# micahvista/VACmap

Measured on AMD Instinct MI355X. Metric: aligned Gbp/s (whole node) + reads/s, 15 kb ONT-shape reads vs hg38-size ref, 1/2/4/8 MI355X, higher is better.
Workload: dtype i16/i32 DP + f64 chains

## Files before the change

### include/vacmapx.h

```cpp
#ifndef VACMAPX_H
#define VACMAPX_H
#include <stdint.h>
#ifdef __cplusplus
extern "C" {
#endif

typedef enum vm_status {
    VM_OK = 0,
    VM_ERR_ARG = -1,
    VM_ERR_NO_DEVICE = -2,
    VM_ERR_NO_CTX = -3,
    VM_ERR_OOM = -4,
    VM_ERR_IO = -5,
    VM_ERR_HIP = -6,
    VM_ERR_UNSUPPORTED = -7,
    VM_READ_RAISED = -10,
    VM_READ_CAPACITY = -20,
    VM_READ_FASTPATH = -21,
    VM_READ_UNSUPPORTED = -22
} vm_status;

enum { VM_MODE_H = 0, VM_MODE_L = 1, VM_MODE_S = 2, VM_MODE_R = 3,
       VM_MODE_ASM = 4 };

// ... 45 lines not shown
int vm_index_blob_count(const vm_index*);
int vm_index_blob(const vm_index*, int i, void** dev_ptr, int64_t* bytes);
int vm_index_meta_size(const vm_index*, int64_t* bytes);
int vm_index_meta_get(const vm_index*, void* buf, int64_t bytes);
int vm_index_from_meta(vm_ctx*, const void* buf, int64_t bytes, vm_index** out);

int vm_sketch_batch(vm_ctx*, int k, int w, int64_t n, const char* seqs, const int64_t* offsets,
                    uint64_t** hash, int32_t** pos, int8_t** strand, int64_t** off);
int vm_map_batch(vm_ctx*, const vm_index*, int check_num, int mid_occ, int64_t n, const char* seqs,
                 const int64_t* offsets, int64_t** anchors, int64_t** anchor_off);
int vm_map(vm_ctx*, const vm_index*, const char* seq, int64_t len, int check_num, int mid_occ, int64_t** anchors, int64_t* n);

typedef struct vm_chains_out {
    int32_t* need_reverse;
    int32_t* mapq;
    double* score;
    int32_t* fast_used;
    int64_t* read_path_off;
    int64_t* path_off;
    int64_t* path_anchors;
    double* S; int64_t* P; int64_t* S_arg; int64_t* gmax; int64_t* opcount;
} vm_chains_out;
int vm_chain_global_batch(vm_ctx*, const vm_params*, int kmersize, int64_t n, const int64_t* anchors,
                          const int64_t* anchor_off, const int64_t* readlens, int want_raw, vm_chains_out* out);
void vm_chains_out_free(vm_chains_out*);

typedef struct vm_local_out {
    int32_t* status;
    int32_t* variant;
    double* score;
    int64_t* chain_off;
    int64_t* chain;
    int64_t* raw_off;
    int64_t* raw;
} vm_local_out;
int vm_local_chain_batch(vm_ctx*, const vm_index*, const vm_params*, int64_t n, const char* seqs, const int64_t* offsets,
                         const int64_t* read_path_off, const int64_t* path_off, const int64_t* path_anchors, vm_local_out* out);
void vm_local_out_free(vm_local_out*);

typedef struct vm_linked_out {
    int64_t gmax, n_hot, n_cold, opcount; double cold_max;
    double* S; int64_t* P; int64_t* S_arg_hot;
    int32_t carry_status, saved; int64_t n_carry; double* carry_S; int64_t* carry_P; int64_t* carry_rows; double carry_g_max_scores; int64_t carry_prereadloc;
} vm_linked_out;
int vm_chain_linked(vm_ctx*, int which, int kmersize, double skipcost, int maxdiff, int maxgap, int64_t n, const int64_t* rows, int64_t n_pre,
                    const double* pre_S, const int64_t* pre_P, double g_max_scores, int64_t g_max_index, int64_t prereadloc, vm_linked_out* out);
void vm_linked_out_free(vm_linked_out*);

typedef struct vm_score { int32_t match, mismatch, o1, e1, o2, e2; } vm_score;
int vm_k_cigar_batch(vm_ctx*, const vm_score*, int eqx, int64_t n, const char* t, const int64_t* t_off, const char* q,
                     const int64_t* q_off, char** cigars, int64_t** cigar_off, int32_t** scores);
int vm_k_cigar_batch_banded(vm_ctx*, const vm_score*, int eqx, int64_t n, const char* t, const int64_t* t_off, const char* q,
                            const int64_t* q_off, char** cigars, int64_t** cigar_off, int32_t** band_flag, int64_t* stats);
int vm_k_extend_batch(vm_ctx*, int match, int mismatch, int o, int e, int bw, int zdrop, int64_t n, const char* t,
                      const int64_t* t_off, const char* q, const int64_t* q_off, int32_t** t_e, int32_t** q_e, int32_t** score);
typedef struct vm_cigar_out { char* cigar; int32_t q_e, t_e, score; } vm_cigar_out;
int vm_k_cigar(vm_ctx*, const char* t, int64_t tl, const char* q, int64_t ql, const vm_score* sc, int bw, int zdrop,
               int eqx, vm_cigar_out* out);
int vm_edit_distance_batch(vm_ctx*, int64_t n, const char* q, const int64_t* q_off, const char* t, const int64_t* t_off,
                           int64_t** dist);
int64_t vm_edit_distance(vm_ctx*, const char* q, int64_t ql, const char* t, int64_t tl);
int vm_edit_distance_bound_batch(vm_ctx*, int tier, int64_t n, const char* q, const int64_t* q_off, const char* t, const int64_t* t_off,
                                 int64_t** bound);

typedef struct vm_record {
    int32_t read_idx;
    int32_t contig;
    int32_t strand;
    int32_t mapq;
    int64_t q_st, q_en;
    int64_t r_st, r_en;
    int64_t cigar_off, cigar_len;
} vm_record;

typedef struct vm_batch_stats {
    int64_t n_reads, read_bases, n_minimizers, n_hits, n_anchors, n_local_hits, n_local_anchors;
    int64_t n_segments, n_ed_problems, ed_cells, n_ext_problems, ext_cells, n_dp_problems, dp_cells;
    int64_t n_records, cigar_bytes, aligned_bases, n_unmapped, n_failed;
    int64_t dp_string_bytes;
    double ms_total;
    double ms_stage[16];
    double ms_gapfill_fill;
    double ms_gapfill_trace;
    int64_t n_gapfill_launches;
    int64_t n_ed_full;
    int64_t n_ed_tier2;
    int64_t n_ed_tier1;
    int64_t n_dp_redo;
    int64_t dp_redo_tb_bytes;
    double ms_local_seed;
    double ms_cluster;
    int64_t n_host_syncs;
    int64_t n_local_general;
    int64_t n_ext_retries;
    int64_t n_batch_retries;
    int64_t n_dp_redo_wide;
    int64_t n_dp_redo_full;
} vm_batch_stats;

int vm_align_batch(vm_ctx*, const vm_index*, const vm_params*, int64_t n_reads, const char* seqs, const int64_t* offsets,
                   vm_record** recs, int64_t* n_recs, char** cigar_blob, int32_t* status_per_read, vm_batch_stats* stats);
typedef struct vm_reads vm_reads;
int vm_reads_upload(vm_ctx*, int64_t n_reads, const char* seqs, const int64_t* offsets, vm_reads** out);
int vm_reads_reupload(vm_ctx*, vm_reads*, int64_t n_reads, const char* seqs, const int64_t* offsets);
void vm_reads_free(vm_reads*);
int vm_align_resident(vm_ctx*, const vm_index*, const vm_params*, const vm_reads*, vm_record** recs, int64_t* n_recs,
                      char** cigar_blob, int32_t* status_per_read, vm_batch_stats* stats);

int vm_align_asm(vm_ctx*, const vm_index*, const vm_params* p, const char* contig, int64_t len, int64_t split_len, int64_t batch_anchors, int64_t window,
                 vm_record** recs, int64_t* n_recs, char** cigar_blob, int32_t* status);

int vm_align_trace(vm_ctx*, const vm_index*, const vm_params*, int64_t n_reads, const char* seqs, const int64_t* offsets, int stage,
                   int64_t** rows, int64_t** row_off);

typedef struct vm_sam_opts {
    int32_t md, shortcs, cigar2cg, markunbalancetra, hardclip, fakecigar;
    const char* rg_id;
    int32_t asm_mode;
} vm_sam_opts;
int vm_sam_emit(const vm_index*, const vm_sam_opts*, int64_t n_reads, const char* names, const int64_t* name_off, const char* seqs, const int64_t* seq_off,
                const char* quals, const int64_t* qual_off, const char* comments, const int64_t* com_off, const vm_record* recs, int64_t n_recs,
                const char* cigar_blob, const int32_t* status, int nthreads, char** text, int64_t** text_off, int64_t* n_lines, int64_t* n_skipped);
int vm_sam_emit_device(vm_ctx*, const vm_index*, const vm_sam_opts*, int64_t n_reads, const char* names, const int64_t* name_off, const char* seqs,
                       const int64_t* seq_off, const char* quals, const int64_t* qual_off, const vm_record* recs, int64_t n_recs, const char* cigar_blob,
                       const int32_t* status, char** text, int64_t** text_off, int64_t* n_lines, int64_t* n_skipped);
int vm_sam_emit_device_times(vm_ctx*, double* seconds3);
int64_t vm_blob_gather(const char* blob, const int64_t* off, const int64_t* idx, int64_t n, char* out, int64_t* out_off);
int64_t vm_blob_write_parts_mmap(int fd, int64_t file_off, const char* const* blobs, const int64_t* const* offs, const int32_t* part, const int64_t* idx, int64_t n, int nthreads);
int64_t vm_blob_gather_parts(const char* const* blobs, const int64_t* const* offs, const int32_t* part, const int64_t* idx, int64_t n, char* out);
void* vm_pinned_alloc(int64_t bytes, int device);
void vm_pinned_free(void* p);
int64_t vm_blob_write_parts(int fd, const char* const* blobs, const int64_t* const* offs, const int32_t* part, const int64_t* idx, int64_t n);
typedef struct vm_fastx vm_fastx;
int vm_fastx_open(const char* path, vm_fastx** out);
int vm_fastx_open_range(const char* path, int64_t begin, int64_t end, vm_fastx** out);
void vm_fastx_close(vm_fastx*);
int64_t vm_fastx_read(vm_fastx*, int64_t max_reads, int64_t max_bases, char** names, int64_t** name_off, char** seqs, int64_t** seq_off, char** quals,
                      int64_t** qual_off, char** comments, int64_t** com_off);

typedef struct vm_bam_writer vm_bam_writer;
int vm_bam_writer_create(vm_ctx*, const char* sam_header, int64_t len, vm_bam_writer** out);
void vm_bam_writer_free(vm_bam_writer*);
int vm_bam_header(vm_bam_writer*, char** out, int64_t* n);
int vm_bam_encode(vm_bam_writer*, const char* sam, int64_t len, char** out, int64_t* n);
int vm_bam_compress_parts(vm_bam_writer*, const char* const* blobs, const int64_t* const* offs, const int32_t* part, const int64_t* idx, int64_t n,
                          char** out, int64_t* n_out);
int vm_bgzf_compress(vm_ctx*, const void* in, int64_t n, char** out, int64_t* n_out);

int vm_bgzf_decompress(vm_ctx*, const void* in, int64_t n, char** out, int64_t* n_out);
typedef struct vm_bam_reader vm_bam_reader;
// ... 27 lines not shown
```

### vacmap_amd/csrc/k_dp.hip

```cpp
#include "vmx_device.h"
#include "vmx_kernels.h"

__device__ __forceinline__ int vmx_tcode(uint8_t c) { return c < 4 ? (int)c : 6; }


__global__ void k_encode(const char* __restrict__ in, uint8_t* __restrict__ out, int64_t n) {
    int64_t i = (int64_t)blockIdx.x * blockDim.x + threadIdx.x;
    int64_t stride = (int64_t)gridDim.x * blockDim.x;
    for (; i < n; i += stride) out[i] = vmx_code((uint8_t)in[i]);
}

#define VMX_EXT_RING 512
__global__ void __launch_bounds__(64) k_extend(const uint8_t* __restrict__ tcodes, const int64_t* __restrict__ t_off,
                                               const uint8_t* __restrict__ qcodes, const int64_t* __restrict__ q_off, int n_prob,
                                               int match, int mismatch, int o, int e, int bw_in, int zdrop,
                                               int32_t* __restrict__ out_te, int32_t* __restrict__ out_qe, int32_t* __restrict__ out_sc, const int32_t* __restrict__ n_ptr) {
    if (n_ptr) n_prob = *n_ptr;
    __shared__ int sH[3][VMX_EXT_RING];
    __shared__ int sE[2][VMX_EXT_RING];
    __shared__ int sF[2][VMX_EXT_RING];
    const int lane = vmx_lane();
    const int RM = VMX_EXT_RING - 1;
    for (int p = blockIdx.x; p < n_prob; p += gridDim.x) {
        const uint8_t* T = tcodes + t_off[p];
// ... 390 lines not shown
                int dloX = 0, dloY = 0;
                const int gX = nsX > 0 ? vmx_ad_geom_nd(tlX0, qlX0, VMX_ADW_DPN * ns, &dloX) : 0, gY = nsY > 0 ? vmx_ad_geom_nd(tlY0, qlY0, VMX_ADW_DPN * ns, &dloY) : 0;
                const int tlX = gX > 0 ? tlX0 : 0, qlX = gX > 0 ? qlX0 : 0, tlY = gY > 0 ? tlY0 : 0, qlY = gY > 0 ? qlY0 : 0;
                int scX = 0, scY = 0;
#define VMX_ADW_RUN(NSV) vmx_gapfill_fill_ad<NSV, 64>(tcodes + prX.t_off, qcodes + prX.q_off, tlX, qlX, dloX, vmx_tb_ptr(tb_pool, redo_pool, prX.tb_off), tcodes + prY.t_off, qcodes + prY.q_off, \
                                                      tlY, qlY, dloY, vmx_tb_ptr(tb_pool, redo_pool, prY.tb_off), match, mismatch, o1, e1, o2, e2, lane, scX, scY)
                if (ns == 2) VMX_ADW_RUN(2); else if (ns == 3) VMX_ADW_RUN(3); else VMX_ADW_RUN(4);
#undef VMX_ADW_RUN
                keepX = gX > 0 && vmx_ad_proven(scX, tlX0, qlX0, gX, match, o1, e1, o2, e2);
                keepY = gY > 0 && vmx_ad_proven(scY, tlY0, qlY0, gY, match, o1, e1, o2, e2);
            }
            if (lane == 0) {
                if (keepX) out_score[pX] = VMX_PK_FLAG;
                if (keepY) out_score[pY] = VMX_PK_FLAG;
                const int kept = (int)keepX + (int)keepY, full = 1 + (int)(pY >= 0) - kept;
                if (kept) atomicAdd(redo_cnt + 6, kept);
                if (full) atomicAdd(redo_cnt + 7, full);
            }
            if (!keepX || (pY >= 0 && !keepY)) __syncthreads();
            if (!keepX) vmx_gapfill_fill_one<SCORE>(tcodes, qcodes, probs, pX, match, mismatch, o1, e1, o2, e2, tb_pool, bnd_pool, out_score, lane, VMX_PK_FLAG, redo_pool);
            if (pY >= 0 && !keepY) vmx_gapfill_fill_one<SCORE>(tcodes, qcodes, probs, pY, match, mismatch, o1, e1, o2, e2, tb_pool, bnd_pool, out_score, lane, VMX_PK_FLAG, redo_pool);
        }
    }
    while (true) {
        int q0;
        if (order) { int v = 0; if (lane == 0) v = atomicAdd(counter, 4); q0 = vmx_bcast0(v); }
        else { q0 = static_next; static_next += 4 * (int)gridDim.x; }
        if (q0 >= n_prob) break;
        const int qg = q0 + (lane >> 4);
        const int pg = qg < n_prob ? (order ? order[qg] : qg) : -1;
        bool x4 = false, skip = false;
        {
            vmx_dp_prob pr; pr.tl = 0; pr.ql = 0; pr.t_off = 0; pr.q_off = 0; pr.tb_off = 0; pr.bnd_off = 0;
            if (pg >= 0) pr = probs[pg];
            skip = redo_pass && pg >= 0 && VMX_REDO_PK(pr.tl, pr.ql);
            x4 = pg >= 0 && !skip && pr.tl > 0 && pr.ql > 0 && VMX_DP16X4_OK(pr.tl, pr.ql);
            if (!SCORE && x4 && (lane & 15) == 0) out_score[pg] = 0;
            if (__any(x4))
                vmx_gapfill_fill16x4<SCORE>(tcodes + pr.t_off, qcodes + pr.q_off, x4 ? pr.tl : 0, x4 ? pr.ql : 0, match, mismatch, o1, e1, o2, e2, vmx_tb_ptr(tb_pool, redo_pool, pr.tb_off),
                                            bnd_pool + pr.bnd_off, &out_score[pg < 0 ? 0 : pg], lane);
        }
        for (int gk = 0; gk < 4; ++gk) {
            const int p = vmx_readlane(pg, 16 * gk);
            if (p < 0 || vmx_readlane((int)(x4 || skip), 16 * gk)) continue;
            vmx_gapfill_fill_one<SCORE>(tcodes, qcodes, probs, p, match, mismatch, o1, e1, o2, e2, tb_pool, bnd_pool, out_score, lane, 0, redo_pool);
        }
    }
}

__device__ __forceinline__ void vmx_gapfill_ad_pass(const uint8_t* __restrict__ tcodes, const uint8_t* __restrict__ qcodes, vmx_dp_prob* __restrict__ probs, int n_prob,
                                                   int match, int mismatch, int o1, int e1, int o2, int e2, uint8_t* __restrict__ tb_pool, int32_t* __restrict__ bnd_pool,
                                                   int32_t* __restrict__ out_score, const int32_t* __restrict__ order, const int32_t* __restrict__ range, int32_t* __restrict__ counter,
                                                   int32_t* __restrict__ redo_list, int32_t* __restrict__ redo_cnt, int ad_pct, unsigned long long* __restrict__ redo_bytes,
                                                   unsigned long long redo_cap, int tb_by_ns) {
    const int lane = vmx_lane();
    const int pct = ad_pct & 0xffff, pct_min = (ad_pct >> 16) & 0xffff;
    const bool ad_ok = vmx_ad_scores_ok(match, mismatch, o1, e1, o2, e2);
    const int n_head = range[0] < n_prob ? range[0] : n_prob;
    bool head = n_head > 0;
    while (true) {
        int pX = -1, pY = -1;
        if (head) {
            int q; { int v = 0; if (lane == 0) v = atomicAdd(counter + 1, 1); q = vmx_bcast0(v); }
            if (q >= n_head) { head = false; continue; }
            if (lane < 16) pX = order[q];
        } else {
            int q0; { int v = 0; if (lane == 0) v = atomicAdd(counter, 8); q0 = n_head + vmx_bcast0(v); }
            if (q0 >= n_prob) break;
            const int qX = q0 + 2 * (lane >> 4), qY = qX + 1;
            if (qX < n_prob) pX = order[qX];
            if (qY < n_prob) pY = order[qY];
        }
        vmx_dp_prob prX, prY;
        prX.tl = 0; prX.ql = 0; prX.t_off = 0; prX.q_off = 0; prX.tb_off = 0; prY = prX;
        if (pX >= 0) prX = probs[pX];
        if (pY >= 0) prY = probs[pY];
        const bool x4X = pX >= 0 && prX.tl > 0 && prX.ql > 0 && VMX_DP16X4_OK(prX.tl, prX.ql), x4Y = pY >= 0 && prY.tl > 0 && prY.ql > 0 && VMX_DP16X4_OK(prY.tl, prY.ql);
        const int nsX = x4X && ad_ok ? vmx_ad_ns(prX.tl, prX.ql, match, o1, e1, o2, e2, pct, pct_min) : 0, nsY = x4Y && ad_ok ? vmx_ad_ns(prY.tl, prY.ql, match, o1, e1, o2, e2, pct, pct_min) : 0;
        const int ns = vmx_uniform_i32(vmx_wave_max_i32(nsX > nsY ? nsX : nsY));
        bool keepX = false, keepY = false, triedX = false, triedY = false;
        if (ns > 0) {
            int dloX = 0, dloY = 0;
            const bool fitX = !tb_by_ns || VMX_AD_W(nsX) == VMX_AD_W(ns), fitY = !tb_by_ns || VMX_AD_W(nsY) == VMX_AD_W(ns);
            const int gX = (nsX > 0 && fitX) ? vmx_ad_geom(prX.tl, prX.ql, ns, &dloX) : 0, gY = (nsY > 0 && fitY) ? vmx_ad_geom(prY.tl, prY.ql, ns, &dloY) : 0;
            const int tlX = gX > 0 ? prX.tl : 0, qlX = gX > 0 ? prX.ql : 0, tlY = gY > 0 ? prY.tl : 0, qlY = gY > 0 ? prY.ql : 0;
            int scX = 0, scY = 0;
#define VMX_AD_RUN(NSV) vmx_gapfill_fill_ad<NSV>(tcodes + prX.t_off, qcodes + prX.q_off, tlX, qlX, dloX, tb_pool + prX.tb_off, tcodes + prY.t_off, qcodes + prY.q_off, tlY, qlY, dloY, \
                                                 tb_pool + prY.tb_off, match, mismatch, o1, e1, o2, e2, lane, scX, scY)
            if (ns == 1) VMX_AD_RUN(1); else if (ns == 2) VMX_AD_RUN(2); else if (ns == 3) VMX_AD_RUN(3); else VMX_AD_RUN(4);
#undef VMX_AD_RUN
            triedX = gX > 0; triedY = gY > 0;
            keepX = gX > 0 && vmx_ad_proven(scX, prX.tl, prX.ql, gX, match, o1, e1, o2, e2);
            keepY = gY > 0 && vmx_ad_proven(scY, prY.tl, prY.ql, gY, match, o1, e1, o2, e2);
        }
        if ((lane & 15) == 0) {
            if (x4X) {
                out_score[pX] = keepX ? VMX_AD_FLAG + ns : 0;
                if (!keepX) {
                    if (triedX) atomicAdd(redo_cnt + 3, 1);
                    const unsigned long long need = (unsigned long long)VMX_REDO_TB_BYTES(prX.tl, prX.ql), at = atomicAdd(redo_bytes, need);
                    if (at + need > redo_cap) { probs[pX].tl = 0; probs[pX].ql = 0; probs[pX].tb_off = 0; }
                    else { probs[pX].tb_off = -(int64_t)at - 1; redo_list[atomicAdd(redo_cnt, 1)] = pX; }
                }
            }
            if (x4Y) {
                out_score[pY] = keepY ? VMX_AD_FLAG + ns : 0;
                if (!keepY) {
                    if (triedY) atomicAdd(redo_cnt + 3, 1);
                    const unsigned long long need = (unsigned long long)VMX_REDO_TB_BYTES(prY.tl, prY.ql), at = atomicAdd(redo_bytes, need);
                    if (at + need > redo_cap) { probs[pY].tl = 0; probs[pY].ql = 0; probs[pY].tb_off = 0; }
                    else { probs[pY].tb_off = -(int64_t)at - 1; redo_list[atomicAdd(redo_cnt, 1)] = pY; }
                }
            }
        }
        for (int gk = 0; gk < 8; ++gk) {
            const int p = vmx_readlane((gk & 1) ? pY : pX, 16 * (gk >> 1));
            if (p < 0 || vmx_readlane((int)((gk & 1) ? x4Y : x4X), 16 * (gk >> 1))) continue;
            vmx_gapfill_fill_one<false>(tcodes, qcodes, probs, p, match, mismatch, o1, e1, o2, e2, tb_pool, bnd_pool, out_score, lane);
        }
    }
}

__global__ void __launch_bounds__(64) k_gapfill_fill(const uint8_t* __restrict__ tcodes, const uint8_t* __restrict__ qcodes,
                                                     const vmx_dp_prob* __restrict__ probs, int n_prob, int match, int mismatch,
                                                     int o1, int e1, int o2, int e2, uint8_t* __restrict__ tb_pool,
                                                     int32_t* __restrict__ bnd_pool, int32_t* __restrict__ out_score,
                                                     const int32_t* __restrict__ order, int32_t* __restrict__ counter) {
    vmx_gapfill_fill_body<true>(tcodes, qcodes, probs, n_prob, match, mismatch, o1, e1, o2, e2, tb_pool, bnd_pool, out_score, order, counter);
}
__global__ void __launch_bounds__(64, 4) k_gapfill_fill_ns(const uint8_t* __restrict__ tcodes, const uint8_t* __restrict__ qcodes,
                                                        vmx_dp_prob* __restrict__ probs, int n_prob, int match, int mismatch,
                                                        int o1, int e1, int o2, int e2, uint8_t* __restrict__ tb_pool,
                                                        int32_t* __restrict__ bnd_pool, int32_t* __restrict__ out_score,
                                                        const int32_t* __restrict__ order, const int32_t* __restrict__ range, int32_t* __restrict__ counter,
                                                        int32_t* __restrict__ redo_list, int32_t* __restrict__ redo_cnt, int ad_pct,
                                                        unsigned long long* __restrict__ redo_bytes, const int32_t* __restrict__ n_ptr,
                                                        unsigned long long redo_cap, int tb_by_ns) {
    if (n_ptr) n_prob = *n_ptr;
    vmx_gapfill_ad_pass(tcodes, qcodes, probs, n_prob, match, mismatch, o1, e1, o2, e2, tb_pool, bnd_pool, out_score, order, range, counter, redo_list, redo_cnt, ad_pct, redo_bytes, redo_cap, tb_by_ns);
}
__global__ void __launch_bounds__(64) k_gapfill_redo(const uint8_t* __restrict__ tcodes, const uint8_t* __restrict__ qcodes, const vmx_dp_prob* __restrict__ probs,
                                                     int match, int mismatch, int o1, int e1, int o2, int e2, uint8_t* __restrict__ tb_pool,
                                                     int32_t* __restrict__ bnd_pool, int32_t* __restrict__ out_score, int32_t* __restrict__ redo_list,
                                                     int32_t* __restrict__ redo_cnt, uint8_t* __restrict__ redo_pool) {
    vmx_gapfill_fill_body<false, true>(tcodes, qcodes, probs, 0, match, mismatch, o1, e1, o2, e2, tb_pool, bnd_pool, out_score, nullptr, nullptr, redo_list, redo_cnt, redo_pool);
}

__global__ void k_gapfill_trace(const uint8_t* __restrict__ tcodes, const uint8_t* __restrict__ qcodes,
                                const vmx_dp_prob* __restrict__ probs, int n_prob, int eqx, const uint8_t* __restrict__ tb_pool,
                                uint32_t* __restrict__ run_pool, char* __restrict__ cig_pool, int32_t* __restrict__ cig_len,
                                const int32_t* __restrict__ band_flag, const uint8_t* __restrict__ redo_pool, int spread, int32_t* __restrict__ cig_q,
                                const int32_t* __restrict__ n_ptr) {
    VMX_SETPRIO(3);
    if (n_ptr) n_prob = *n_ptr;
    const int gt = (int)(blockIdx.x * blockDim.x + threadIdx.x);
    if (spread > 1 && gt % spread) return;
    int p = spread > 1 ? gt / spread : gt;
    if (p >= n_prob) return;
    const vmx_dp_prob pr = probs[p];
    const uint8_t* T = tcodes + pr.t_off;
    const uint8_t* Q = qcodes + pr.q_off;
    const int tl = pr.tl, ql = pr.ql;
    const uint8_t* tb = vmx_tb_ptr(tb_pool, redo_pool, pr.tb_off);
    uint32_t* runs = run_pool + pr.run_off;
    char* cig = cig_pool + pr.cig_off;
    bool x4 = tl > 0 && ql > 0 && VMX_DP16X4_OK(tl, ql);
    bool pk = !x4 && tl > 0 && ql > 0 && VMX_DP16_OK(tl, ql);
    const int flag = (x4 && band_flag != nullptr) ? band_flag[p] : 0;
    const int ns = flag > VMX_AD_FLAG ? flag - VMX_AD_FLAG : 0;
    if (flag == VMX_PK_FLAG) { x4 = false; pk = true; }
    int dlo = 0;
    if (ns) vmx_ad_geom(tl, ql, ns, &dlo);
    const int AW = ns ? VMX_AD_W(ns) : 4;
    const int W = x4 ? VMX_X4_W(ql) : ql + (pk ? 127 : 63);
    int nruns = 0; int cur_op = -1; uint32_t cur_len = 0;
#define VMX_EMIT(op)                                                                   \
    do {                                                                               \
        if ((op) == cur_op) ++cur_len;                                                 \
        else { if (cur_op >= 0) runs[nruns++] = (cur_len << 8) | (uint32_t)cur_op; cur_op = (op); cur_len = 1; } \
    } while (0)
    int i = tl, j = ql, state = 0;
    while (i > 0 && j > 0) {
        int b;
        if (ns && state == 0) {
            const int x = (j - i) - dlo, l = x / (2 * ns), k = (x - 2 * ns * l) >> 1;
            const uint8_t* cell = tb + VMX_AD_TB_OFF_W(0, l, AW) + k;
            const int s0 = i + j - 1;
            int m = i < j ? i : j; if (m > 8) m = 8;
            uint8_t bb[8], ta[8], qa[8];
#pragma unroll
            for (int u = 0; u < 8; ++u) if (u < m) { bb[u] = cell[VMX_AD_TB_OFF_W(s0 - 2 * u, 0, AW)]; if (eqx) { ta[u] = T[i - 1 - u]; qa[u] = Q[j - 1 - u]; } }
            int u = 0;
// ... 49 lines not shown
```

### vacmap_amd/csrc/vmx_align.hip

```cpp
#include "vmx_host.h"
#include "vmx_stage.h"
#include "vmx_select.h"
#include "vmx_ext_state.h"
#include "vmx_round.h"
#include <algorithm>
#include <cstdio>
#include <cstdlib>
#include <cstddef>
#include <cstring>
#include <string>

using namespace vmx;

__global__ void k_orient(const uint8_t* codes, const int64_t* roff, const double* gscore, int n_reads, uint8_t* ocodes);
__global__ void k_scan_i64(const int64_t* in, int64_t* out, int64_t n, int pow2_round);
__global__ void k_ext_phase(vmx_ext_args A, int phase);
__global__ void k_ed_anchor_bound(vmx_ext_args A, const int32_t* probread, const uint8_t* qpool, const int64_t* qoff, const uint8_t* tpool, const int64_t* toff,
                                  int64_t* ub_out);
__global__ void k_desc_lens(const vmx_pair_desc* desc, const int32_t* n_prob, int64_t* tl, int64_t* ql);
__global__ void k_gather(const vmx_pair_desc* desc, const int32_t* n_prob, const int32_t* prob_read, const uint8_t* ocodes, const int64_t* roff,
                         const uint8_t* ref, const int64_t* t_off, const int64_t* q_off, uint8_t* tpool, uint8_t* qpool, int64_t pool_cap, vmx_ext_read* er);
__global__ void k_prob_owner(const vmx_ext_read* er, int n_reads, int use_dp, int32_t* prob_read);
__global__ void k_dp_sizes(const vmx_pair_desc* desc, const int32_t* n_prob, int64_t* tb_sz, int64_t* bnd_sz, int64_t* run_sz, int64_t* cig_sz);
__global__ void k_dp_table(const vmx_pair_desc* desc, const int32_t* n_prob, const int64_t* t_off, const int64_t* q_off, const int64_t* tb_off,
// ... 90 lines not shown
    const bool rows_kernel = vmx_chain_rows_on() && rmode != 2;
    for (int64_t r = 0; r < n; ++r) {
        int64_t m = h_aoff[r + 1] - h_aoff[r]; const int64_t L = h_roff[r + 1] - h_roff[r];
        if (m <= 2) continue;
        if (prm->mode == VM_MODE_ASM && L >= 500000) { asm_long.push_back(r); continue; }
        if ((double)m / (double)L > 5.0) continue;
        int bk = NB; for (int q = 0; q < NB; ++q) if (m <= caps[q] && caps[q] <= gc_lds_max) { bk = q; break; }
        if (rows_kernel) bk = NB;
        lists[bk].push_back((int32_t)r);
    }
    {
        std::vector<int32_t> rl; int64_t rl_off[NB + 2];
        for (int q = 0; q <= NB; ++q) {
            std::stable_sort(lists[q].begin(), lists[q].end(), [&](int32_t a, int32_t b) { return h_aoff[a + 1] - h_aoff[a] > h_aoff[b + 1] - h_aoff[b]; });
            rl_off[q] = (int64_t)rl.size(); rl.insert(rl.end(), lists[q].begin(), lists[q].end());
        }
        VMX_TRY(vmx_push(c, B.rl, rl.data(), rl.size()));
        VMX_HIP(hipMemsetAsync(B.gmax.p, 0xff, 8 * (size_t)n, c->stream));
        { static const int64_t kUnsupported = -4; for (int64_t r : asm_long) VMX_HIP(hipMemcpyAsync(B.gmax.as<int64_t>() + r, &kUnsupported, 8, hipMemcpyHostToDevice, c->stream)); }
#ifndef VMX_EMU
        VMX_HIP(hipFuncSetAttribute((const void*)k_chain_global, hipFuncAttributeMaxDynamicSharedMemorySize, (int)((size_t)caps[NB - 1] * VMX_GC_BYTES_PER_ANCHOR + 64)));
#endif
        vmx_fork fk(c);
        for (int q = NB; q >= 0; --q) {
            int cnt = (int)lists[q].size(); if (!cnt) continue;
            int cap = q < NB ? caps[q] : 0; size_t shmem = (size_t)cap * VMX_GC_BYTES_PER_ANCHOR + 64;
            if (rows_kernel) {
                hipLaunchKernelGGL((vmx_chain_rows_win3() ? k_chain_global_rows_w3 : k_chain_global_rows), dim3((unsigned)((cnt + 3) / 4)), dim3(64), 0, fk.next(), B.sorted.as<vmx_anchor>(), B.aoff.as<int64_t>(),
                                   B.rl.as<int32_t>() + rl_off[q], cnt, c->tables, B.gap.as<double>(), prm->global_skipcost, prm->global_maxdiff, 1000, B.S.as<double>(),
                                   B.P.as<int32_t>(), B.SA.as<int32_t>(), B.cov.as<uint8_t>(), B.gmax.as<int64_t>(), B.opc.as<int64_t>(), rmode, B.fp.as<double>(), B.pp.as<double>(),
                                   vmx_chain_dbg());
                continue;
            }
            hipLaunchKernelGGL(k_chain_global, dim3((unsigned)cnt), dim3(64), shmem, fk.next(), B.sorted.as<vmx_anchor>(), B.aoff.as<int64_t>(),
                               B.rl.as<int32_t>() + rl_off[q], cnt, cap, c->tables, B.gap.as<double>(), prm->global_skipcost, prm->global_maxdiff, 1000, B.S.as<double>(),
                               B.P.as<int32_t>(), B.SA.as<int32_t>(), B.cov.as<uint8_t>(), B.gmax.as<int64_t>(), B.opc.as<int64_t>(), rmode, B.fp.as<double>(), B.pp.as<double>());
        }
        fk.join();
        vmx_chain_dbg_report(c->stream);
        VMX_TRY(B.si.reserve(4 * (size_t)(tot + 1))); VMX_TRY(B.tg.reserve(8 * (size_t)(tot + 1))); VMX_TRY(B.cntp.reserve(4 * (size_t)(total_bases + 50 * n + 64)));
        hipLaunchKernelGGL(k_chain_global_fast, dim3((unsigned)n), dim3(64), 0, c->stream, B.sorted.as<vmx_anchor>(), B.aoff.as<int64_t>(), (int)n, d_roff, c->tables,
                           B.gap.as<double>(), prm->global_skipcost, prm->global_maxdiff, 1000, B.S.as<double>(), B.P.as<int32_t>(), B.SA.as<int32_t>(), B.cov.as<uint8_t>(),
                           B.si.as<int32_t>(), B.tg.as<int64_t>(), B.cntp.as<int32_t>(), B.gmax.as<int64_t>(), d_ran, rmode, B.fp.as<double>(), B.pp.as<double>());
    }
    VMX_TRY(B.scr.reserve((size_t)stt + 64)); VMX_TRY(vmx_push(c, B.soff, soff.data(), (size_t)n + 1));
    VMX_TRY(B.res.reserve(16 * (size_t)(n + 2) + 64));
    double* d_gscore; int32_t* d_mapq; int32_t* d_np; vmx_res_ptrs(B, n, &d_gscore, &d_mapq, &d_np);
    VMX_TRY(B.plen.reserve(4 * (size_t)(tot + 1))); VMX_TRY(B.prow.reserve(sizeof(vmx_anchor) * (size_t)(tot + 1)));
    return vmx_launch_chain_select(c, n, h_aoff.data(), B.sellist, B.sorted.as<vmx_anchor>(), B.aoff.as<int64_t>(), B.lens.as<int64_t>(), B.S.as<double>(), B.P.as<int32_t>(), B.SA.as<int32_t>(),
                                   B.gmax.as<int64_t>(), B.flip.as<int32_t>(), prm->mode, B.scr.as<char>(), B.soff.as<int64_t>(), d_mapq, d_gscore, d_np, B.plen.as<int32_t>(), B.prow.as<vmx_anchor>());
}

void vmx_gapfill_chunk(vm_ctx* c, vmx_batch_bufs& B, const vm_score& sc, int ad_pct, int eqx, int p0, int64_t pn, const int32_t* n_ptr, int64_t tb_off0,
                       int32_t* ctl, int32_t* redo_list, int64_t redo_cap, hipEvent_t* ke) {
    int fill_waves = 16;
    if (const char* e = getenv("VMX_FILL_WAVES")) { const int v = atoi(e); if (v >= 1 && v <= 32) fill_waves = v; }
    static const int tr_spread = [] { const char* e = getenv("VMX_TRACE_SPREAD"); const int v = e ? atoi(e) : 1; return v >= 1 && v <= 64 ? v : 1; }();
    int32_t* d_range = ctl; int32_t* d_cnt = ctl + 4; int32_t* d_redo_cnt = ctl + 12;
    unsigned long long* d_redo_bytes = (unsigned long long*)(ctl + 16); int32_t* scratch = ctl + 32;
    uint8_t* tb_base = B.tb.as<uint8_t>() - tb_off0;
    vmx_dp_prob* probs = B.dptab.as<vmx_dp_prob>() + p0; int32_t* score = B.dpscore.as<int32_t>() + p0;
    const unsigned Gs = (unsigned)std::max<int64_t>(1, std::min<int64_t>((pn + 1023) / 1024, (int64_t)c->num_cu * 2));
    hipLaunchKernelGGL(k_size_hist, dim3(Gs), dim3(256), 0, c->stream, B.dpsz[0].as<int64_t>() + p0, n_ptr, (int64_t)((1LL << 42) - 1), scratch);
    hipLaunchKernelGGL(k_size_scatter, dim3(Gs), dim3(256), 0, c->stream, B.dpsz[0].as<int64_t>() + p0, n_ptr, (const int32_t*)scratch, scratch + 257, B.order.as<int32_t>(), d_range, d_cnt);
    if (ke) (void)hipEventRecord(ke[0], c->stream);
    {
        vmx_lowprio lp(c);
        hipLaunchKernelGGL(k_gapfill_fill_ns, dim3((unsigned)std::max<int64_t>(1, std::min<int64_t>(pn, (int64_t)c->num_cu * fill_waves))), dim3(64), 0, lp.stream(), B.tpool.as<uint8_t>(), B.qpool.as<uint8_t>(),
                           probs, (int)pn, sc.match, sc.mismatch, sc.o1, sc.e1, sc.o2, sc.e2, tb_base, B.bnd.as<int32_t>(), score, B.order.as<int32_t>(), d_range, d_cnt,
                           redo_list, d_redo_cnt, ad_pct, d_redo_bytes, n_ptr, (unsigned long long)redo_cap, 1);
        lp.join();
    }
    hipLaunchKernelGGL(k_gapfill_redo, dim3((unsigned)std::max<int64_t>(1, std::min<int64_t>(pn, (int64_t)c->num_cu * 4))), dim3(64), 0, c->stream, B.tpool.as<uint8_t>(), B.qpool.as<uint8_t>(),
                       probs, sc.match, sc.mismatch, sc.o1, sc.e1, sc.o2, sc.e2, tb_base, B.bnd.as<int32_t>(), score, redo_list, d_redo_cnt, B.tbredo.as<uint8_t>());
    if (ke) (void)hipEventRecord(ke[1], c->stream);
    hipLaunchKernelGGL(k_gapfill_trace, dim3((unsigned)std::max<int64_t>(1, (pn * tr_spread + 63) / 64)), dim3(64), 0, c->stream, B.tpool.as<uint8_t>(), B.qpool.as<uint8_t>(), probs, (int)pn, eqx,
                       tb_base, B.run.as<uint32_t>(), B.cig.as<char>(), B.ciglen.as<int32_t>() + p0, score, B.tbredo.as<uint8_t>(), tr_spread, B.cigq.as<int32_t>() + p0, n_ptr);
    if (ke) (void)hipEventRecord(ke[2], c->stream);
}

#define LAUNCH1D(kernel, n, ...) hipLaunchKernelGGL(kernel, dim3((unsigned)std::max<int64_t>(1, std::min<int64_t>(((n) + 255) / 256, 4096))), dim3(256), 0, c->stream, __VA_ARGS__)

__global__ void k_ext_geometry(const int32_t* la_cnt, const int64_t* roff, int n, int mul, int tmask, long long tdiv, long long capA, long long capS, long long capB, int64_t* coff3,
                               int64_t* soff2, int64_t* bloboff, int64_t* tot);
__global__ void k_scan_part_dev(const int64_t* in, int64_t* part, const int32_t* n_ptr);
__global__ void k_scan_apply_dev(const int64_t* in, int64_t* out, const int64_t* part_off, const int32_t* n_ptr);
__global__ void k_scan_part(const int64_t* in, int64_t* part, int64_t n, int64_t chunk);
__global__ void k_scan_apply(const int64_t* in, int64_t* out, const int64_t* part_off, int64_t n, int64_t chunk);

static int dev_scan(vm_ctx* c, vmx_batch_bufs& B, const int64_t* in, int64_t* out, int64_t n) {
    if (n <= 16384) { hipLaunchKernelGGL(k_scan_i64, dim3(1), dim3(256), 0, c->stream, in, out, n, 0); return 0; }
    int64_t chunk = (n + 511) / 512; const int64_t nb = (n + chunk - 1) / chunk;
    VMX_TRY(B.scanpart.reserve(8 * (size_t)(nb + 2))); VMX_TRY(B.scanoff.reserve(8 * (size_t)(nb + 2)));
    hipLaunchKernelGGL(k_scan_part, dim3((unsigned)nb), dim3(256), 0, c->stream, in, B.scanpart.as<int64_t>(), n, chunk);
    hipLaunchKernelGGL(k_scan_i64, dim3(1), dim3(256), 0, c->stream, B.scanpart.as<int64_t>(), B.scanoff.as<int64_t>(), nb, 0);
    hipLaunchKernelGGL(k_scan_apply, dim3((unsigned)nb), dim3(256), 0, c->stream, in, out, B.scanoff.as<int64_t>(), n, chunk);
    return 0;
}

static int dev_scan_dev(vm_ctx* c, vmx_batch_bufs& B, const int64_t* in, int64_t* out, const int32_t* n_ptr) {
    const int nb = 512;
    VMX_TRY(B.scanpart.reserve(8 * (size_t)(nb + 2))); VMX_TRY(B.scanoff.reserve(8 * (size_t)(nb + 2)));
    hipLaunchKernelGGL(k_scan_part_dev, dim3(nb), dim3(256), 0, c->stream, in, B.scanpart.as<int64_t>(), n_ptr);
    hipLaunchKernelGGL(k_scan_i64, dim3(1), dim3(256), 0, c->stream, B.scanpart.as<int64_t>(), B.scanoff.as<int64_t>(), (int64_t)nb, 0);
    hipLaunchKernelGGL(k_scan_apply_dev, dim3(nb), dim3(256), 0, c->stream, in, out, B.scanoff.as<int64_t>(), n_ptr);
    return 0;
}

static const vm_score gf_score = {2, -4, 4, 2, 24, 1};

static int ext_gather_round(vm_ctx* c, vmx_batch_bufs& B, const vm_index_view& ix, int64_t n, const uint8_t* d_ocodes, const int64_t* d_roff, int cur, int redo_only,
                            int64_t round_cap, int64_t pool_cap, int stat_slot, bool dp, int64_t tb_limit, const int64_t* caps = nullptr, int64_t* plan_out = nullptr, int ad_pct = 0) {
    (void)n; (void)redo_only; (void)round_cap;
    if (!B.roundpart.p) { VMX_TRY(B.roundpart.reserve(8 * (size_t)VMX_ROUND_PART_WORDS)); VMX_HIP(hipMemsetAsync(B.roundpart.p, 0, 8 * (size_t)VMX_ROUND_PART_WORDS, c->stream)); }
    vmx_round_args R; memset(&R, 0, sizeof R);
    R.desc = B.desc[cur].as<vmx_pair_desc>(); R.n_prob = c->rc_cur;
    R.off[0] = B.toff.as<int64_t>(); R.off[1] = B.qoff.as<int64_t>();
    R.part = B.roundpart.as<int64_t>(); R.stat_out = B.statblk.as<int32_t>() + stat_slot; R.epoch = ++c->round_epoch;
    if (dp) {
        for (int i = 0; i < 4; ++i) R.off[2 + i] = B.dpoff[i].as<int64_t>();
        R.tb_size = B.dpsz[0].as<int64_t>(); R.probs = B.dptab.as<vmx_dp_prob>(); R.plan_out = plan_out; R.tb_limit = tb_limit;
        if (caps) for (int i = 0; i < 4; ++i) R.cap[i] = caps[i];
        R.ad_on = 1; R.ad_match = gf_score.match; R.ad_o1 = gf_score.o1; R.ad_e1 = gf_score.e1; R.ad_o2 = gf_score.o2; R.ad_e2 = gf_score.e2; R.ad_pct = ad_pct;
// ... 237 lines not shown
    A.ocodes = B.ocodes.as<uint8_t>(); A.roff = d_roff; A.ref = ix.codes; A.coff = ix.coff;
    A.chain = L.chain.as<vmx_anchor>(); A.chain_len = L.chain_len.as<int32_t>(); A.la_off = L.la_off.as<int64_t>(); A.lstatus = L.status.as<int32_t>();
    A.gscore = d_gscore; A.mapq = d_mapq; A.er = B.er.as<vmx_ext_read>(); A.coff3 = B.coff3.as<int64_t>(); A.soff = B.soff2.as<int64_t>();
    A.segA = B.segA.as<vmx_anchor>(); A.st = B.st.as<int32_t>(); A.en = B.en.as<int32_t>(); A.segA_snap = B.segA_s.as<vmx_anchor>(); A.st_snap = B.st_s.as<int32_t>(); A.en_snap = B.en_s.as<int32_t>();
    A.seg_prob = B.segprob.as<int32_t>(); A.dup = B.dup.as<int32_t>(); A.round_count = B.rcount.as<int32_t>(); A.round_cap = round_cap; A.overflow = B.oflow.as<int32_t>(); A.prob_read = B.probread.as<int32_t>();
    A.ed_out = B.edout.as<int64_t>(); A.ext_te = B.ext3.as<int32_t>(); A.ext_qe = B.ext3.as<int32_t>() + round_cap;
    A.rec = B.rec.as<vm_record>(); A.rec_blob = B.blob.as<char>(); A.blob_off = B.bloboff.as<int64_t>(); A.rec_coff = B.reccoff.as<int64_t>(); A.rec_clen = B.recclen.as<int32_t>();
    A.dup_d = B.dupd.as<double>();
    const unsigned gridR = (unsigned)((n + 63) / 64);
    static const int ext_env = [] { const char* e = getenv("VMX_EXT_SPREAD"); const int v = e ? atoi(e) : 0; return v >= 1 && v <= 64 ? v : 0; }();
    static const int rec_env = [] { const char* e = getenv("VMX_REC_SPREAD"); const int v = e ? atoi(e) : 0; return v >= 1 && v <= 64 ? v : 0; }();
    const int ext_spread = ext_env ? ext_env : (c->inflight >= 2 ? 1 : 16), rec_spread = rec_env ? rec_env : (c->inflight >= 2 ? 1 : 4);
    const unsigned gridX = (unsigned)((n * ext_spread + 63) / 64), gridXR = (unsigned)((n * rec_spread + 63) / 64);
    static const bool ext_wave = [] { const char* e = getenv("VMX_EXT_WAVE"); return !(e && atoi(e) == 0); }();
    int cur = 0;
    auto phase = [&](int ph) { A.desc = B.desc[cur].as<vmx_pair_desc>(); A.desc_prev = B.desc[cur ^ 1].as<vmx_pair_desc>();
                               c->rc_cur = B.rcount.as<int32_t>() + (c->rc_next++ & 63); A.round_count = c->rc_cur;
                               const bool wv = ext_wave && (ph == 0 || ph == 3 || ph == 5);
                               A.spread = wv ? 64 : ext_spread; hipLaunchKernelGGL(k_ext_phase, dim3(wv ? (unsigned)n : gridX), dim3(64), 0, c->stream, A, ph);
                               if (trace && trace->stage == ph && !A.redo_only && trace->off.empty()) {
                                   std::vector<vmx_ext_read> er((size_t)n); std::vector<vmx_anchor> sa((size_t)cA + 1); std::vector<int32_t> st_((size_t)cS + 1), en_((size_t)cS + 1);
                                   (void)hipMemcpyAsync(er.data(), B.er.p, sizeof(vmx_ext_read) * (size_t)n, hipMemcpyDeviceToHost, c->stream);
                                   (void)hipMemcpyAsync(sa.data(), B.segA.p, sizeof(vmx_anchor) * (size_t)cA, hipMemcpyDeviceToHost, c->stream);
                                   (void)hipMemcpyAsync(st_.data(), B.st.p, 4 * (size_t)cS, hipMemcpyDeviceToHost, c->stream);
                                   (void)hipMemcpyAsync(en_.data(), B.en.p, 4 * (size_t)cS, hipMemcpyDeviceToHost, c->stream);
                                   (void)vmx_stream_sync(c);
                                   trace->off.assign(1, 0);
                                   for (int64_t r = 0; r < n; ++r) {
                                       if (er[(size_t)r].active && er[(size_t)r].status == 0)
                                           for (int sg = 0; sg < er[(size_t)r].nseg; ++sg)
                                               for (int t = st_[(size_t)(soff2[r] + sg)]; t < en_[(size_t)(soff2[r] + sg)]; ++t) {
                                                   const vmx_anchor& a = sa[(size_t)(coff3[r] + t)];
                                                   const int64_t row[5] = {sg, a.q, a.r, a.s, a.l}; trace->rows.insert(trace->rows.end(), row, row + 5);
                                               }
                                       trace->off.push_back((int64_t)trace->rows.size() / 5);
                                   }
                               } };
    int ext_rounds = 0;
    auto ext_round = [&](int redo_only) -> int {
        int rc = ext_gather_round(c, B, ix, n, B.ocodes.as<uint8_t>(), d_roff, cur, redo_only, round_cap, pool_cap, 1 + ext_rounds++, false, 0);
        if (rc < 0) return rc;
        hipLaunchKernelGGL(k_extend, dim3((unsigned)((int64_t)c->num_cu * 16)), dim3(64), 0, c->stream, B.tpool.as<uint8_t>(), B.toff.as<int64_t>(), B.qpool.as<uint8_t>(),
                           B.qoff.as<int64_t>(), 0, 2, -4, 4, 4, 100, 50, B.ext3.as<int32_t>(), B.ext3.as<int32_t>() + round_cap, B.ext3.as<int32_t>() + 2 * round_cap, c->rc_cur);
        cur ^= 1;
        return 0;
    };
    std::vector<int64_t> dp_tot(5, 0);
    static std::mutex ad_m; static struct { int pct = 0, floor = 20, hold = 0; } ad_tab[16][8];
    auto& adr = ad_tab[c->device & 15][prm->mode & 7];
    int ad_cur; { std::lock_guard<std::mutex> g(ad_m); if (adr.pct == 0) adr.pct = vmx_ad_pct_env(prm->mode) & 0xffff; ad_cur = adr.pct; }
    const bool ad_pinned = getenv("VMX_AD_PCT") != nullptr || getenv("VMX_AD_PCT_MIN") != nullptr;
    const int ad_pct = ad_pinned ? vmx_ad_pct_env(prm->mode) : (ad_cur | (std::max(20, ad_cur - 25) << 16));
    static const int64_t tb_chunk = [] { const char* e = getenv("VMX_TB_CHUNK_GB"); const double v = e ? atof(e) : 0.0; return v > 0.5 ? (int64_t)(v * (double)(1 << 30)) : (int64_t)VMX_TB_CHUNK; }();
    int gf_chunks[2] = {0, 0}; int64_t gf_redo_cap = 0;
    auto gf_chunk = [&](int pass, int q, int p0, int64_t pn, const int32_t* n_ptr, int64_t tb_off0) {
        int32_t* ctl = B.gfctl.as<int32_t>() + (size_t)(pass * (VMX_MAX_CHUNKS + 1) + q) * VMX_GF_SLOT;
        hipEvent_t* ke = q < 8 ? c->gev + (pass ? 24 : 0) + 3 * q : nullptr;
        vmx_gapfill_chunk(c, B, gf_score, ad_pct, prm->eqx, p0, pn, n_ptr, tb_off0, ctl, B.order.as<int32_t>() + round_cap + 32, gf_redo_cap, ke);
        if (ke) c->n_gev[pass] = q + 1;
        gf_chunks[pass] = q + 1;
    };
    auto gapfill = [&](int redo_only) -> int {
        for (int i = 0; i < 4; ++i) { VMX_TRY(B.dpsz[i].reserve(8 * (size_t)(round_cap + 2))); VMX_TRY(B.dpoff[i].reserve(8 * (size_t)(round_cap + 2))); }
        VMX_TRY(B.dptab.reserve(sizeof(vmx_dp_prob) * (size_t)(round_cap + 1))); VMX_TRY(B.ciglen.reserve(4 * (size_t)(round_cap + 1))); VMX_TRY(B.cigq.reserve(4 * (size_t)(round_cap + 1))); VMX_TRY(B.dpscore.reserve(4 * (size_t)(round_cap + 1)));
        VMX_TRY(B.order.reserve(4 * (size_t)(2 * round_cap + 64)));
        if (!redo_only) {
            gf_redo_cap = std::max<int64_t>((int64_t)((double)c->redo_need_max * 1.3), std::min<int64_t>((int64_t)512 << 20, std::max<int64_t>(tb_chunk / 8, 1 << 20)));
            if (const char* e = getenv("VMX_TEST_REDO_POOL_BYTES")) { const long long v = atoll(e); if (v > 0 && c->redo_need_max == 0) gf_redo_cap = v; }
            VMX_TRY(B.tbredo.reserve((size_t)gf_redo_cap + 64));
            gf_redo_cap = (int64_t)B.tbredo.cap - 64;
        }
        c->n_gev[redo_only ? 1 : 0] = 0;
        {
            int rcg = ext_gather_round(c, B, ix, n, B.ocodes.as<uint8_t>(), d_roff, cur, redo_only, round_cap, pool_cap, 6 + redo_only, true, tb_chunk, nullptr, B.statblk.as<int64_t>() + 64 + (redo_only ? 64 : 0), ad_pct);
            if (rcg < 0) return rcg;
            int64_t plan[8 + 2 * (VMX_MAX_CHUNKS + 1)];
            VMX_TRY(vmx_fetch(c, plan, B.statblk.as<int64_t>() + 64 + (redo_only ? 64 : 0), sizeof(plan) / 8));
            VMX_HIP(vmx_stream_sync(c));
            const int cnt = (int)plan[0];
            int64_t totals[4] = {plan[1], plan[2], plan[3], plan[4]};
            if (plan[7] < 0) { set_error("gap fill: more traceback chunks than VMX_MAX_CHUNKS"); return VM_ERR_OOM; }
            st.n_dp_problems += cnt; st.dp_cells += totals[0]; st.dp_string_bytes += plan[5] + plan[6];
            std::vector<int32_t> cuts; std::vector<int64_t> h_tboff_at;
            for (int q = 0; q <= (int)plan[7]; ++q) { cuts.push_back((int32_t)plan[8 + q]); h_tboff_at.push_back(plan[8 + VMX_MAX_CHUNKS + 1 + q]); }
            if (cuts.size() < 2) { cuts.assign(2, 0); h_tboff_at.assign(2, 0); }
            int64_t tbmax = 0;
            for (size_t q = 0; q + 1 < cuts.size(); ++q) tbmax = std::max(tbmax, h_tboff_at[q + 1] - h_tboff_at[q]);
            VMX_TRY(B.tb.reserve((size_t)tbmax + 64)); VMX_TRY(B.bnd.reserve(4 * (size_t)(totals[1] + 4))); VMX_TRY(B.run.reserve(4 * (size_t)(totals[2] + 4))); VMX_TRY(B.cig.reserve((size_t)totals[3] + 16));
            if (cnt) {
                std::vector<int32_t> csz; for (size_t q = 0; q + 1 < cuts.size(); ++q) csz.push_back(cuts[q + 1] - cuts[q]);
                VMX_TRY(vmx_push(c, B.chunkn, csz.data(), csz.size()));
                for (size_t q = 0; q + 1 < cuts.size(); ++q) gf_chunk(redo_only, (int)q, cuts[q], cuts[q + 1] - cuts[q], B.chunkn.as<int32_t>() + q, h_tboff_at[q]);
            }
        }
        A.redo_only = redo_only;
        A.spread = rec_spread;
        hipLaunchKernelGGL(k_ext_records, dim3((unsigned)n), dim3(64), 0, c->stream, A, B.dptab.as<vmx_dp_prob>(), B.cig.as<char>(), B.ciglen.as<int32_t>(), B.cigq.as<int32_t>());
        cur ^= 1;
        return 0;
    };
    phase(0);
    {
        int rc0 = ext_gather_round(c, B, ix, n, B.ocodes.as<uint8_t>(), d_roff, cur, 0, round_cap, pool_cap, 0, false, 0);
        if (rc0 < 0) return rc0;
        const int64_t cnt = round_cap;
        {
            VMX_TRY(B.order.reserve(4 * (size_t)(2 * round_cap + 64))); VMX_TRY(B.qrange.reserve(128)); VMX_TRY(B.szh.reserve(4 * 520));
            int32_t* d_range = B.qrange.as<int32_t>(); int32_t* d_cnt = d_range + 4; int32_t* d_nfull = d_range + 8;
            VMX_TRY(B.dpsz[0].reserve(8 * (size_t)(round_cap + 2))); VMX_TRY(B.dpsz[1].reserve(8 * (size_t)(round_cap + 2)));
            int32_t* d_n2 = d_range + 9; int32_t* d_n1 = d_range + 10;
            (void)hipMemsetAsync(d_nfull, 0, 12, c->stream);
            hipLaunchKernelGGL(k_ed_anchor_bound, dim3((unsigned)std::min<int64_t>(cnt, (int64_t)c->num_cu * 16)), dim3(64), 0, c->stream, A, B.probread.as<int32_t>(),
                               B.qpool.as<uint8_t>(), B.qoff.as<int64_t>(), B.tpool.as<uint8_t>(), B.toff.as<int64_t>(), B.dpsz[1].as<int64_t>());
            static const bool always_all = getenv("VMX_FORCE_EXACT") != nullptr;
            const bool all_tiers = c->force_exact || always_all;
            hipLaunchKernelGGL(k_ed_flag, dim3((unsigned)std::min<int64_t>((cnt + 255) / 256, 1024)), dim3(256), 0, c->stream, B.dpsz[1].as<int64_t>(), B.qoff.as<int64_t>(), B.toff.as<int64_t>(),
                               c->rc_cur, prm->maxdivergence, B.dpsz[0].as<int64_t>(), B.edout.as<int64_t>(), d_n1, 1, B.probread.as<int32_t>(), all_tiers ? (vmx_ext_read*)nullptr : B.er.as<vmx_ext_read>());
            if (all_tiers) {
// ... 26 lines not shown
    phase(5); VMX_TRY(gapfill(0));
    VMX_HIP(hipEventRecord(ev[nev++], c->stream));
    int64_t test_side_every = 0; if (const char* e = getenv("VMX_TEST_SIDE_EVERY")) test_side_every = atoll(e);
    static const bool always_pass1 = getenv("VMX_FORCE_PASS1") != nullptr;
    const bool do_pass1 = c->run_pass1 || always_pass1;
    if (do_pass1) {
        A.redo_only = 1;
        phase(3); phase(4); phase(5); VMX_TRY(gapfill(1));
        A.redo_only = 0;
    }
    VMX_HIP(hipEventRecord(ev[nev++], c->stream));

    VMX_TRY(B.dpsz[0].reserve(8 * (size_t)(n + 2))); VMX_TRY(B.dpsz[1].reserve(8 * (size_t)(n + 2))); VMX_TRY(B.dpoff[0].reserve(8 * (size_t)(n + 2))); VMX_TRY(B.dpoff[1].reserve(8 * (size_t)(n + 2)));
    hipLaunchKernelGGL(k_res_sizes, dim3(gridR), dim3(64), 0, c->stream, B.er.as<vmx_ext_read>(), B.rec.as<vm_record>(), B.soff2.as<int64_t>(), (int)n, B.dpsz[0].as<int64_t>(), B.dpsz[1].as<int64_t>());
    hipLaunchKernelGGL(k_scan_i64, dim3(1), dim3(256), 0, c->stream, B.dpsz[0].as<int64_t>(), B.dpoff[0].as<int64_t>(), n, 0);
    hipLaunchKernelGGL(k_scan_i64, dim3(1), dim3(256), 0, c->stream, B.dpsz[1].as<int64_t>(), B.dpoff[1].as<int64_t>(), n, 0);
    int64_t nr = 0, nb = 0; int32_t oflow = 0;
    int32_t n_full = 0, n_t2 = 0, n_t1 = 0;
    int64_t fin[14]; int64_t hstat[8];
    hipLaunchKernelGGL(k_final_scalars, dim3(1), dim3(1), 0, c->stream, B.dpoff[0].as<int64_t>() + n, B.dpoff[1].as<int64_t>() + n, B.oflow.as<int32_t>(), B.qrange.as<int32_t>() + 8,
                       B.statblk.as<int32_t>(), B.statblk.as<int64_t>() + 32);
    VMX_TRY(B.totals.reserve(sizeof(vm_record) * (size_t)(cS + 1))); VMX_TRY(B.dupd.reserve((size_t)cB + 64));
    hipLaunchKernelGGL(k_res_pack, dim3((unsigned)std::min<int64_t>(n, (int64_t)c->num_cu * 8)), dim3(64), 0, c->stream, B.er.as<vmx_ext_read>(), B.rec.as<vm_record>(), B.blob.as<char>(),
                       B.soff2.as<int64_t>(), B.bloboff.as<int64_t>(), (int)n, B.dpoff[0].as<int64_t>(), B.dpoff[1].as<int64_t>(), B.totals.as<vm_record>(), B.dupd.as<char>());
    int64_t g_nr = std::min<int64_t>(cS, (int64_t)(c->res_rec_per_read * 2.0 * (double)n) + 256), g_nb = std::min<int64_t>(cB, (int64_t)(c->res_blob_per_base * 1.5 * (double)total_bases) + 65536);
    if (c->res_rec_per_read <= 0.0) { g_nr = 0; g_nb = 0; }
    std::vector<vmx_ext_read> er((size_t)n);
    std::vector<int64_t> h_gmax((size_t)n);
    *recs = (vm_record*)malloc(sizeof(vm_record) * (size_t)std::max<int64_t>(g_nr, 1)); *cigar_blob = (char*)malloc((size_t)std::max<int64_t>(g_nb, 1));
    struct OutGuard { vm_record** r; char** b; bool keep = false; ~OutGuard() { if (!keep) { free(*r); free(*b); *r = nullptr; *b = nullptr; } } } out_guard{recs, cigar_blob};
    if (!*recs || !*cigar_blob) { set_error("out of host memory"); return VM_ERR_OOM; }
    VMX_TRY(vmx_fetch(c, fin, B.statblk.as<int64_t>() + 32, 14));
    int64_t geo[8] = {0, 0, 0, 0, 0, 0, 0, 0};
    if (fast_local) VMX_TRY(vmx_fetch(c, geo, B.geotot.p, 6));
    std::vector<int32_t> h_ctl(gfctl_bytes / 4);
    VMX_TRY(vmx_fetch(c, h_ctl.data(), B.gfctl.p, h_ctl.size()));
    VMX_TRY(vmx_fetch(c, er.data(), B.er.p, (size_t)n)); VMX_TRY(vmx_fetch(c, h_gmax.data(), B.gmax.p, (size_t)n));
    VMX_TRY(vmx_fetch(c, *recs, B.totals.p, (size_t)g_nr)); VMX_TRY(vmx_fetch(c, *cigar_blob, B.dupd.p, (size_t)g_nb));
    VMX_HIP(hipEventRecord(ev[nev++], c->stream));
    VMX_HIP(vmx_stream_sync(c));
    VMX_HIP(hipGetLastError());
    nr = fin[0]; nb = fin[1]; oflow = (int32_t)fin[2]; n_full = (int32_t)fin[3]; n_t2 = (int32_t)fin[4]; n_t1 = (int32_t)fin[5];
    if (fast_local) {
        st.n_local_anchors = geo[4];
        if (geo[5] > 0 || geo[3] + 16 > c->geo_cap[3]) c->geo_valid = false;
        if (geo[5] && getenv("VMX_DBG_POOLS")) fprintf(stderr, "[pools] extend stage: %lld read(s) did not fit the history-sized pools (run again alone)\n", (long long)geo[5]);
    }
    {
        bool again = false; int64_t need_max = 0, ad_failed = 0;
        for (int pass = 0; pass < 2; ++pass)
            for (int q = 0; q < gf_chunks[pass]; ++q) {
                const int32_t* ctl = h_ctl.data() + (size_t)(pass * (VMX_MAX_CHUNKS + 1) + q) * VMX_GF_SLOT;
                unsigned long long rb = 0; memcpy(&rb, ctl + 16, 8);
                st.n_dp_redo += ctl[12]; st.n_dp_redo_wide += ctl[18]; st.n_dp_redo_full += ctl[19]; st.dp_redo_tb_bytes += (int64_t)rb; st.dp_cells += (int64_t)rb; ad_failed += ctl[15];
                need_max = std::max<int64_t>(need_max, (int64_t)rb);
            }
        c->redo_need_max = std::max<long long>(c->redo_need_max, need_max);
        if (need_max > gf_redo_cap) { again = true; if (getenv("VMX_DBG_POOLS")) fprintf(stderr, "[pools] gap fill: a chunk's second launch needs %.3f GB of traceback space, the pool held %.3f: running the batch again\n", need_max / 1e9, gf_redo_cap / 1e9); }
        if (again) return VMX_RETRY_BATCH;
        if (!ad_pinned && !c->force_exact && st.n_dp_problems >= 2000) {
            const double f = (double)ad_failed / (double)st.n_dp_problems;
            std::lock_guard<std::mutex> g(ad_m);
            if (ad_cur == adr.pct) {
                if (f > 0.03 && adr.pct < 100) { adr.pct = std::min(100, adr.pct + 10); adr.floor = adr.pct; adr.hold = 256; }
                else if (adr.hold > 0) { if (--adr.hold == 0) adr.floor = 20; }
                else if (f < 0.025 && adr.pct > adr.floor) adr.pct = std::max(adr.floor, adr.pct - (f < 0.01 ? 20 : 10));
            }
        }
    }
    for (int i = 0; i < 8; ++i) hstat[i] = fin[6 + i];
    st.n_segments = hstat[0]; st.n_ed_problems = hstat[0]; st.n_ext_problems = (int64_t)hstat[1] + hstat[2] + hstat[3] + hstat[4];
    st.n_ed_full = n_full; st.n_ed_tier2 = n_t2; st.n_ed_tier1 = n_t1;
    if (oflow) { set_error("extend stage: a per-batch work pool overflowed"); return VM_ERR_OOM; }
    if (nr > g_nr || nb > g_nb) {
        if (nr > g_nr) { vm_record* p2 = (vm_record*)realloc(*recs, sizeof(vm_record) * (size_t)nr); if (!p2) { set_error("out of host memory"); return VM_ERR_OOM; } *recs = p2;
                         VMX_TRY(vmx_fetch(c, *recs + g_nr, B.totals.as<vm_record>() + g_nr, (size_t)(nr - g_nr))); }
        if (nb > g_nb) { char* p2 = (char*)realloc(*cigar_blob, (size_t)nb); if (!p2) { set_error("out of host memory"); return VM_ERR_OOM; } *cigar_blob = p2;
                         VMX_TRY(vmx_fetch(c, *cigar_blob + g_nb, B.dupd.as<char>() + g_nb, (size_t)(nb - g_nb))); }
        VMX_HIP(vmx_stream_sync(c));
    }
    if (n > 0 && total_bases > 0) { c->res_rec_per_read = std::max(c->res_rec_per_read, (double)nr / (double)n); c->res_blob_per_base = std::max(c->res_blob_per_base, (double)nb / (double)total_bases); }
    for (int64_t r = 0; r < n; ++r) {
        int stt2 = er[r].status == VMX_EXT_CAPACITY_DEV ? VMX_EXT_SHORT_INTERNAL : (er[r].status == VMX_EXT_NEED_EXACT_DEV ? VMX_EXT_EXACT_INTERNAL : er[r].status);
        if (fast_local && (er[r].status == VM_READ_CAPACITY_DEV || er[r].status == VM_READ_BANDFALL_DEV)) stt2 = VMX_EXT_EXACT_INTERNAL;
        if (stt2 == 0 && !do_pass1 && er[r].active && er[r].redo == 1 && er[r].pass == 1) stt2 = VMX_EXT_EXACT_INTERNAL;
        if (stt2 == 0 && test_side_every > 0 && !c->force_exact && r % test_side_every == 0) stt2 = VMX_EXT_EXACT_INTERNAL;
        if (h_gmax[r] == -2 && (h_aoff[r + 1] - h_aoff[r]) > 2) stt2 = VM_READ_RAISED;
        if (h_gmax[r] == -4) stt2 = VM_READ_UNSUPPORTED;
        if (!asm_override.empty() && asm_override[(size_t)r] != 0) stt2 = asm_override[(size_t)r];
        if (rmode == 1 && (h_aoff[r + 1] - h_aoff[r]) <= 2) stt2 = VM_READ_RAISED;
        if (status_per_read) status_per_read[r] = stt2;
        if (stt2 != 0) { st.n_failed++; continue; }
        if (er[r].nrec == 0) st.n_unmapped++;
    }
    for (int64_t i = 0; i < nr; ++i) { st.aligned_bases += (*recs)[i].q_en - (*recs)[i].q_st; st.cigar_bytes += (*recs)[i].cigar_len; }
    *n_recs = nr; st.n_records = nr;
    float ms = 0;
    hipEventElapsedTime(&ms, ev[0], ev[nev - 1]); st.ms_total = ms;
    for (int i = 1; i < nev && i < 16; ++i) { hipEventElapsedTime(&ms, ev[i - 1], ev[i]); st.ms_stage[i - 1] = ms; }
    if ((c->kev_set & 1) && hipEventElapsedTime(&ms, c->kev[0], c->kev[1]) == hipSuccess) st.ms_local_seed = ms;
    if ((c->kev_set & 2) && hipEventElapsedTime(&ms, c->kev[2], c->kev[3]) == hipSuccess) st.ms_cluster = ms;
    st.n_host_syncs = c->n_syncs; st.n_local_general = c->n_bandfall;
    st.ms_stage[14] = (float)((c->sync_wait_ns + download_wait_ns()) * 1e-6);
    st.ms_stage[15] = (float)((std::chrono::duration_cast<std::chrono::nanoseconds>(std::chrono::steady_clock::now().time_since_epoch()).count() - c->call_t0_ns) * 1e-6);
    for (int pass = 0; pass < 2; ++pass)
        for (int q = 0; q < c->n_gev[pass]; ++q) {
            hipEvent_t* ke = c->gev + 24 * pass + 3 * q;
            if (hipEventElapsedTime(&ms, ke[0], ke[1]) == hipSuccess) st.ms_gapfill_fill += ms;
            if (hipEventElapsedTime(&ms, ke[1], ke[2]) == hipSuccess) st.ms_gapfill_trace += ms;
            st.n_gapfill_launches++;
        }
    if (stats) *stats = st;
    if (getenv("VMX_DBG_POOLS")) {
        const DevBuf* bb = (const DevBuf*)&B; size_t tot = 0;
        for (size_t i = 0; i < sizeof(B) / sizeof(DevBuf); ++i) { tot += bb[i].cap; if (bb[i].cap > ((size_t)128 << 20)) fprintf(stderr, "[pools] batch[%zu] %.2f GB\n", i, bb[i].cap / 1e9); }
        fprintf(stderr, "[pools] batch bufs total %.2f GB\n", tot / 1e9);
        const DevBuf* lb = (const DevBuf*)&L; size_t lt = 0; const size_t nl = (size_t)((const char*)&L.la_pool_rows - (const char*)&L) / sizeof(DevBuf);
        for (size_t i = 0; i < nl; ++i) { lt += lb[i].cap; if (lb[i].cap > ((size_t)128 << 20)) fprintf(stderr, "[pools] local[%zu] %.2f GB\n", i, lb[i].cap / 1e9); }
        fprintf(stderr, "[pools] local bufs total %.2f GB\n", lt / 1e9);
        fprintf(stderr, "[pools] process so far: %lld first allocations, %lld re-allocations, %.3f s in hipFree + hipMalloc\n", (long long)vmx::devbuf_stats().first.load(),
                (long long)vmx::devbuf_stats().grows.load(), vmx::devbuf_stats().ns.load() * 1e-9);
    }
    if (stats) *stats = st;
    out_guard.keep = true;
    return VM_OK;
}

template <class RunOne>
static int align_in_sub_batches(int64_t n, const int64_t* offsets, int64_t max_bases, RunOne run_one, vm_record** recs, int64_t* n_recs, char** cigar_blob, vm_batch_stats* stats) {
    if (n <= VMX_MAX_BATCH_READS && offsets[n] - offsets[0] <= max_bases) {
        const int rc = run_one(0, n, recs, n_recs, cigar_blob, stats);
        if (rc != VM_ERR_OOM || n <= 1) return rc;
        free(*recs); free(*cigar_blob);
    }
    *recs = nullptr; *n_recs = 0; *cigar_blob = nullptr;
    std::vector<vm_record> all; std::string blob;
    vm_batch_stats tot; memset(&tot, 0, sizeof tot);
    std::vector<std::pair<int64_t, int64_t>> work;
    for (int64_t a = 0; a < n;) {
        int64_t b = a + 1;
        while (b < n && b - a < VMX_MAX_BATCH_READS && offsets[b + 1] - offsets[a] <= max_bases) ++b;
        work.emplace_back(a, b); a = b;
    }
    for (size_t wi = 0; wi < work.size(); ++wi) {
        const int64_t a = work[wi].first, b = work[wi].second;
        vm_record* r = nullptr; int64_t nr = 0; char* cb = nullptr; vm_batch_stats st;
        const int rc = run_one(a, b, &r, &nr, &cb, &st);
        if (rc == VM_ERR_OOM && b - a > 1) {
            free(r); free(cb);
            vmx::devbuf_retired().flush();
            const int64_t mid = a + (b - a) / 2;
            work[wi] = std::make_pair(a, mid); work.insert(work.begin() + (std::ptrdiff_t)wi + 1, std::make_pair(mid, b));
            --wi; continue;
        }
        if (rc < 0) { free(r); free(cb); return rc; }
        int64_t bl = 0; for (int64_t i = 0; i < nr; ++i) bl = std::max(bl, r[i].cigar_off + r[i].cigar_len);
        for (int64_t i = 0; i < nr; ++i) { vm_record x = r[i]; x.read_idx += (int32_t)a; x.cigar_off += (int64_t)blob.size(); all.push_back(x); }
        blob.append(cb, (size_t)bl); blob.push_back('\0');
        free(r); free(cb);
        {
            int64_t* d = (int64_t*)&tot; const int64_t* s2 = (const int64_t*)&st;
            for (size_t i = 0; i < offsetof(vm_batch_stats, ms_total) / 8; ++i) d[i] += s2[i];
            tot.ms_total += st.ms_total; for (int i = 0; i < 16; ++i) tot.ms_stage[i] += st.ms_stage[i];
            tot.ms_gapfill_fill += st.ms_gapfill_fill; tot.ms_gapfill_trace += st.ms_gapfill_trace; tot.n_gapfill_launches += st.n_gapfill_launches;
            tot.n_ed_full += st.n_ed_full; tot.n_ed_tier2 += st.n_ed_tier2; tot.n_ed_tier1 += st.n_ed_tier1;
            tot.n_dp_redo += st.n_dp_redo; tot.n_dp_redo_wide += st.n_dp_redo_wide; tot.n_dp_redo_full += st.n_dp_redo_full; tot.dp_redo_tb_bytes += st.dp_redo_tb_bytes; tot.ms_local_seed += st.ms_local_seed; tot.ms_cluster += st.ms_cluster; tot.n_host_syncs += st.n_host_syncs; tot.n_local_general += st.n_local_general; tot.n_ext_retries += st.n_ext_retries; tot.n_batch_retries += st.n_batch_retries;
        }
    }
    *recs = (vm_record*)malloc(sizeof(vm_record) * std::max<size_t>(all.size(), 1)); *cigar_blob = (char*)malloc(std::max<size_t>(blob.size(), 1));
    if (!*recs || !*cigar_blob) { free(*recs); free(*cigar_blob); *recs = nullptr; *cigar_blob = nullptr; set_error("out of host memory"); return VM_ERR_OOM; }
    memcpy(*recs, all.data(), sizeof(vm_record) * all.size()); memcpy(*cigar_blob, blob.data(), blob.size());
    *n_recs = (int64_t)all.size();
    if (stats) *stats = tot;
    return VM_OK;
}
static int64_t vmx_pass_bases() {
    static const int64_t v = [] { const char* e = getenv("VMX_MAX_BATCH_BASES"); const long long x = e ? atoll(e) : 0; return x > 0 ? (int64_t)x : (int64_t)VMX_MAX_BATCH_BASES; }();
    return v;
}

extern "C" {

int vm_reads_upload(vm_ctx* c, int64_t n, const char* seqs, const int64_t* offsets, vm_reads** out) {
    *out = nullptr;
    if (!c) { set_error("no context"); return VM_ERR_NO_CTX; }
    VMX_HIP(hipSetDevice(c->device));
    vm_reads* R = new vm_reads(); R->ctx = c; R->n = n; R->h_off.assign(offsets, offsets + n + 1);
    const int64_t tot = offsets[n];
    int rc = 0;
    if ((rc = upload(R->raw, seqs, (size_t)tot, c->stream)) < 0 || (rc = R->codes.reserve((size_t)tot + 64)) < 0 || (rc = upload(R->off, offsets, (size_t)n + 1, c->stream)) < 0) { delete R; return rc; }
    if (tot) LAUNCH1D(k_encode, tot, R->raw.as<char>(), R->codes.as<uint8_t>(), tot);
    VMX_HIP(vmx_stream_sync(c));
    R->raw.release();
    *out = R;
    return VM_OK;
}
int vm_reads_reupload(vm_ctx* c, vm_reads* R, int64_t n, const char* seqs, const int64_t* offsets) {
    if (!c || !R) { set_error("no context / reads object"); return VM_ERR_NO_CTX; }
    VMX_HIP(hipSetDevice(c->device));
    R->n = n; R->h_off.assign(offsets, offsets + n + 1);
    const int64_t tot = offsets[n];
    VMX_TRY(upload(R->raw, seqs, (size_t)tot, c->stream)); VMX_TRY(R->codes.reserve((size_t)tot + 64)); VMX_TRY(upload(R->off, offsets, (size_t)n + 1, c->stream));
    if (tot) LAUNCH1D(k_encode, tot, R->raw.as<char>(), R->codes.as<uint8_t>(), tot);
    VMX_HIP(vmx_stream_sync(c));
    return VM_OK;
}
void vm_reads_free(vm_reads* R) { if (!R) return; R->raw.release(); R->codes.release(); R->off.release(); delete R; }

int vm_align_resident(vm_ctx* c, const vm_index* mi, const vm_params* prm, const vm_reads* R, vm_record** recs, int64_t* n_recs, char** cigar_blob,
                      int32_t* status_per_read, vm_batch_stats* stats) {
    if (!c) { set_error("no context"); return VM_ERR_NO_CTX; }
    VMX_HIP(hipSetDevice(c->device));
    if (R->n <= VMX_MAX_BATCH_READS && R->h_off[(size_t)R->n] <= vmx_pass_bases())
        return align_device(c, mi, prm, R->n, R->codes.as<uint8_t>(), R->off.as<int64_t>(), R->h_off, recs, n_recs, cigar_blob, status_per_read, stats);
    vmx_batch_bufs& B = *vmx_ctx_batch_bufs(c);
    auto run_one = [&](int64_t a, int64_t b, vm_record** r, int64_t* nr, char** cb, vm_batch_stats* st) -> int {
        std::vector<int64_t> h((size_t)(b - a) + 1);
        for (int64_t i = a; i <= b; ++i) h[(size_t)(i - a)] = R->h_off[(size_t)i] - R->h_off[(size_t)a];
        VMX_TRY(vmx_push(c, B.off, h.data(), h.size()));
// ... 56 lines not shown
```

### vacmap_amd/csrc/vmx_capi.hip

```cpp
#include "vmx_host.h"
#include <time.h>
#include "vmx_select.h"
#include "vmx_stage.h"
#include "vmx_round.h"
#include <algorithm>
#include <cmath>
#include <cstdlib>
#include <cstring>
#include <numeric>

namespace vmx {
static thread_local std::string g_err;
void set_error(const std::string& s) { g_err = s; }
int hip_fail(hipError_t e, const char* what, const char* file, int line) {
    g_err = std::string("HIP error: ") + hipGetErrorString(e) + " at " + what + " (" + file + ":" + std::to_string(line) + ")";
    return e == hipErrorOutOfMemory ? VM_ERR_OOM : VM_ERR_HIP;
}
}
using namespace vmx;

void vmx_ctx_free_local_bufs(vm_ctx* c);
void vmx_ctx_free_batch_bufs(vm_ctx* c);
void vmx_ctx_free_sam_bufs(vm_ctx* c);

// ... 177 lines not shown
static unsigned long long* g_chain_dbg = nullptr;
static std::mutex g_chain_dbg_m;
static int chain_dbg_enable() {
    std::lock_guard<std::mutex> g(g_chain_dbg_m);
    if (g_chain_dbg) return 0;
    unsigned long long* q = nullptr;
    if (hipMalloc((void**)&q, 64) != hipSuccess) { (void)hipGetLastError(); return -1; }
    (void)hipMemset(q, 0, 64);
    g_chain_dbg = q;
    return 0;
}
unsigned long long* vmx_chain_dbg() {
    static const bool env = [] { if (getenv("VMX_DBG_CHAIN")) (void)chain_dbg_enable(); return true; }(); (void)env;
    return g_chain_dbg;
}
void vmx_chain_dbg_report(hipStream_t st) {
    static const bool print = getenv("VMX_DBG_CHAIN") != nullptr;
    unsigned long long* p = vmx_chain_dbg(); if (!p || !print) return;
    unsigned long long h[8]; (void)hipStreamSynchronize(st); (void)hipMemcpy(h, p, 64, hipMemcpyDeviceToHost);
    fprintf(stderr, "[chain rows] global: anchors %llu scans past the window %llu insertions through HBM %llu opcount %llu | local: %llu %llu %llu %llu\n", h[0], h[1], h[2], h[3], h[4], h[5], h[6], h[7]);
}
extern "C" {
int vm_debug_chain_counters(int enable, unsigned long long* out8) {
    if (enable > 0 && chain_dbg_enable() < 0) { vmx::set_error("vm_debug_chain_counters: no device memory"); return VM_ERR_OOM; }
    unsigned long long* p = g_chain_dbg;
    if (out8) { memset(out8, 0, 64); if (p) { VMX_HIP(hipDeviceSynchronize()); VMX_HIP(hipMemcpy(out8, p, 64, hipMemcpyDeviceToHost)); } }
    if (enable < 0 && p) { VMX_HIP(hipDeviceSynchronize()); VMX_HIP(hipMemset(p, 0, 64)); }
    return VM_OK;
}

int vm_device_count(void) {
    int n = 0;
    if (hipGetDeviceCount(&n) != hipSuccess) return 0;
    return n;
}

int vm_ctx_create(int device_id, vm_ctx** out) {
    *out = nullptr;
    int n = 0;
    if (hipGetDeviceCount(&n) != hipSuccess || n <= 0) { set_error("no HIP device: libvacmapx has no CPU fallback"); return VM_ERR_NO_DEVICE; }
    if (device_id < 0 || device_id >= n) { set_error("bad device id"); return VM_ERR_ARG; }
    VMX_HIP(hipSetDevice(device_id));
    vm_ctx* c = new vm_ctx();
    c->device = device_id;
    hipDeviceProp_t prop;
    if (hipGetDeviceProperties(&prop, device_id) == hipSuccess && prop.multiProcessorCount > 0) c->num_cu = prop.multiProcessorCount;
    int prio_least = 0, prio_greatest = 0;
    const bool prio = vmx_stream_prio_on() && hipDeviceGetStreamPriorityRange(&prio_least, &prio_greatest) == hipSuccess && prio_least != prio_greatest;
    if ((prio ? hipStreamCreateWithPriority(&c->stream, hipStreamDefault, prio_greatest) : hipStreamCreate(&c->stream)) != hipSuccess) { delete c; set_error("hipStreamCreate failed"); return VM_ERR_HIP; }
    if (prio && hipStreamCreateWithPriority(&c->low, hipStreamDefault, prio_least) == hipSuccess) { (void)hipEventCreateWithFlags(&c->low_ev[0], hipEventDisableTiming); (void)hipEventCreateWithFlags(&c->low_ev[1], hipEventDisableTiming); }
    else c->low = nullptr;
    for (int i = 0; i < 24; ++i) (void)hipEventCreate(&c->ev[i]);
    for (int i = 0; i < 48; ++i) (void)hipEventCreate(&c->gev[i]);
    for (int i = 0; i < 4; ++i) (void)hipEventCreate(&c->kev[i]);
    for (int i = 0; i < 4; ++i) { if (prio) (void)hipStreamCreateWithPriority(&c->aux[i], hipStreamDefault, prio_greatest); else (void)hipStreamCreate(&c->aux[i]); (void)hipEventCreate(&c->join_ev[i]); }
    (void)hipEventCreate(&c->fork_ev);
    (void)mailbox_create(c);
    const HostTables& T = host_tables();
    size_t o_extra = 0, o_rh = o_extra + T.extra.size() * 4, o_rr = o_rh + 400, o_lr = o_rr + 400;
    size_t o_l2c = (o_lr + 400 + 15) & ~(size_t)15, o_l2i = o_l2c + T.log2cache.size() * 8, tot = o_l2i + T.log2int.size() * 8;
    std::vector<char> blob(tot);
    memcpy(&blob[o_extra], T.extra.data(), T.extra.size() * 4);
    memcpy(&blob[o_rh], T.readgap_h.data(), 400); memcpy(&blob[o_rr], T.readgap_r.data(), 400); memcpy(&blob[o_lr], T.large_readgap.data(), 400);
    memcpy(&blob[o_l2c], T.log2cache.data(), T.log2cache.size() * 8); memcpy(&blob[o_l2i], T.log2int.data(), T.log2int.size() * 8);
    if (c->tab_buf.reserve(tot) < 0) { delete c; return VM_ERR_OOM; }
    if (hipMemcpy(c->tab_buf.p, blob.data(), tot, hipMemcpyHostToDevice) != hipSuccess) { delete c; set_error("table upload failed"); return VM_ERR_HIP; }
    char* base = (char*)c->tab_buf.p;
    c->tables.extra = (const float*)(base + o_extra); c->tables.extra_n = (int)T.extra.size();
    c->tables.readgap_h = (const float*)(base + o_rh); c->tables.readgap_r = (const float*)(base + o_rr);
    c->tables.large_readgap = (const float*)(base + o_lr);
    c->tables.log2cache = (const double*)(base + o_l2c); c->tables.log2cache_n = (int)T.log2cache.size();
    c->tables.log2int = (const double*)(base + o_l2i);
    {
        int an = 0; const int lim = std::min<int>(20000, (int)T.extra.size() - 1);
        for (; an < lim; ++an) {
            const double dg = (double)an; const double a = dg * 0.01;
            const float v = (float)((a < 10.0 ? a : 10.0) + dg * 0.001);
            if (memcmp(&v, &T.extra[an], 4) != 0) break;
        }
        c->tables.extra_arith_n = an;
        if (T.extra.back() != 36.0f) { delete c; set_error("cost table `extra` does not end at 36.0"); return VM_ERR_UNSUPPORTED; }
    }
    *out = c;
    return VM_OK;
}

#ifdef VMX_CF_TICKS
extern "C" void vmx_cf_ticks_dump();
#endif
void vm_ctx_destroy(vm_ctx* c) {
    if (!c) return;
    (void)hipSetDevice(c->device);
    (void)hipStreamSynchronize(c->stream);
#ifdef VMX_CF_TICKS
    vmx_cf_ticks_dump();
#endif
    for (int i = 0; i < VMX_NBUF; ++i) c->b[i].release();
    vmx_ctx_free_local_bufs(c);
    vmx_ctx_free_batch_bufs(c);
    vmx_ctx_free_sam_bufs(c);
    c->tab_buf.release();
    vmx::devbuf_retired().flush();
    for (int i = 0; i < 24; ++i) (void)hipEventDestroy(c->ev[i]);
    for (int i = 0; i < 48; ++i) (void)hipEventDestroy(c->gev[i]);
    for (int i = 0; i < 4; ++i) (void)hipEventDestroy(c->kev[i]);
    for (int i = 0; i < 4; ++i) { (void)hipStreamSynchronize(c->aux[i]); (void)hipStreamDestroy(c->aux[i]); (void)hipEventDestroy(c->join_ev[i]); }
    (void)hipEventDestroy(c->fork_ev);
    if (c->sync_ev) (void)hipEventDestroy(c->sync_ev);
    if (c->low) { (void)hipStreamSynchronize(c->low); (void)hipStreamDestroy(c->low); (void)hipEventDestroy(c->low_ev[0]); (void)hipEventDestroy(c->low_ev[1]); }
    (void)hipStreamDestroy(c->stream);
    mailbox_destroy(c);
    delete c;
}

int vm_ctx_set_inflight(vm_ctx* c, int n_contexts) {
    if (!c) { set_error("no context"); return VM_ERR_NO_CTX; }
    if (n_contexts < 1) { set_error("n_contexts must be >= 1"); return VM_ERR_ARG; }
    c->inflight = n_contexts;
    return VM_OK;
}

int vm_ctx_mem_info(vm_ctx* c, int64_t* free_bytes, int64_t* total_bytes) {
    if (!c) { set_error("no context"); return VM_ERR_NO_CTX; }
    size_t f = 0, t = 0;
#ifndef VMX_EMU
    VMX_HIP(hipSetDevice(c->device));
    VMX_HIP(hipMemGetInfo(&f, &t));
#else
    f = (size_t)1 << 34; t = (size_t)1 << 34;
#endif
    *free_bytes = (int64_t)f; *total_bytes = (int64_t)t;
    return VM_OK;
}

int vm_ctx_set_blocking_sync(vm_ctx* c, int on) {
    if (!c) { set_error("no context"); return VM_ERR_NO_CTX; }
    if (on && !c->mb.h) { VMX_HIP(hipSetDevice(c->device)); (void)mailbox_create(c); }
    c->mb.on = on != 0 && c->mb.h != nullptr;
    return VM_OK;
}

int64_t vm_table(vm_ctx* c, int which, void** data) {
    if (!c) return VM_ERR_NO_CTX;
    const vmx_tables& t = c->tables;
    const void* src; size_t n, es;
    switch (which) {
        case 0: src = t.extra; n = t.extra_n; es = 4; break;
        case 1: src = t.readgap_h; n = 100; es = 4; break;
        case 2: src = t.readgap_r; n = 100; es = 4; break;
        case 3: src = t.large_readgap; n = 100; es = 4; break;
        case 4: src = t.log2cache; n = t.log2cache_n; es = 8; break;
        case 5: src = t.log2int; n = 1025; es = 8; break;
        default: return VM_ERR_ARG;
    }
    *data = malloc(n * es);
    VMX_HIP(hipMemcpy(*data, src, n * es, hipMemcpyDeviceToHost));
    return (int64_t)n;
// ... 100 lines not shown
    VMX_HIP(hipStreamSynchronize(c->stream));
    VMX_HIP(hipGetLastError());
    return VM_OK;
}

static void cigar_strings(int64_t n, const vmx_dp_prob* probs, const char* pool, const int32_t* len, char** cigars, int64_t** cigar_off) {
    *cigar_off = host_alloc<int64_t>((size_t)n + 1);
    int64_t tot = 0;
    for (int64_t i = 0; i < n; ++i) { (*cigar_off)[i] = tot; tot += len[i] + 1; }
    (*cigar_off)[n] = tot;
    *cigars = host_alloc<char>((size_t)tot + 1);
    for (int64_t i = 0; i < n; ++i) { memcpy(*cigars + (*cigar_off)[i], pool + probs[i].cig_off, (size_t)len[i]); (*cigars)[(*cigar_off)[i] + len[i]] = 0; }
}

int vm_k_cigar_batch(vm_ctx* c, const vm_score* sc, int eqx, int64_t n, const char* t, const int64_t* t_off, const char* q,
                     const int64_t* q_off, char** cigars, int64_t** cigar_off, int32_t** scores) {
    if (!c) { set_error("no context"); return VM_ERR_NO_CTX; }
    if (n > 0x7fffffff) { set_error("too many problems"); return VM_ERR_ARG; }
    VMX_HIP(hipSetDevice(c->device));
    VMX_TRY(upload_encode(c, t, t_off, n, c->b[0], c->b[1], c->b[2]));
    VMX_TRY(upload_encode(c, q, q_off, n, c->b[3], c->b[4], c->b[5]));
    std::vector<vmx_dp_prob> probs((size_t)n);
    int64_t tb = 0, bnd = 0, run = 0, cig = 0;
    for (int64_t i = 0; i < n; ++i) {
        vmx_dp_prob& p = probs[i];
        p.t_off = t_off[i]; p.q_off = q_off[i]; p.tl = (int32_t)(t_off[i + 1] - t_off[i]); p.ql = (int32_t)(q_off[i + 1] - q_off[i]);
        p.tb_off = tb; p.bnd_off = bnd; p.run_off = run; p.cig_off = cig;
        tb += VMX_TB_BYTES((int64_t)p.tl, (int64_t)p.ql);
        bnd += 3 * (int64_t)(p.ql + 1); run += (int64_t)p.tl + p.ql + 2; cig += 2 * ((int64_t)p.tl + p.ql) + 16;
    }
    VMX_TRY(upload(c->b[6], probs.data(), (size_t)n, c->stream));
    VMX_TRY(c->b[7].reserve((size_t)tb + 64)); VMX_TRY(c->b[8].reserve(sizeof(int32_t) * (size_t)(bnd + 4)));
    VMX_TRY(c->b[9].reserve(sizeof(uint32_t) * (size_t)(run + 4))); VMX_TRY(c->b[10].reserve((size_t)cig + 16));
    VMX_TRY(c->b[11].reserve(sizeof(int32_t) * 2 * (size_t)(n + 1)));
    int32_t* d_score = c->b[11].as<int32_t>(); int32_t* d_len = d_score + n;
    if (n) {
        hipLaunchKernelGGL(k_gapfill_fill, dim3(grid_for(c, n, 16)), dim3(64), 0, c->stream, c->b[1].as<uint8_t>(), c->b[4].as<uint8_t>(),
                           c->b[6].as<vmx_dp_prob>(), (int)n, sc->match, sc->mismatch, sc->o1, sc->e1, sc->o2, sc->e2, c->b[7].as<uint8_t>(),
                           c->b[8].as<int32_t>(), d_score, (const int32_t*)nullptr, (int32_t*)nullptr);
        hipLaunchKernelGGL(k_gapfill_trace, dim3((unsigned)((n + 63) / 64)), dim3(64), 0, c->stream, c->b[1].as<uint8_t>(), c->b[4].as<uint8_t>(),
                           c->b[6].as<vmx_dp_prob>(), (int)n, eqx, c->b[7].as<uint8_t>(), c->b[9].as<uint32_t>(), c->b[10].as<char>(), d_len, (const int32_t*)nullptr, (const uint8_t*)nullptr, 1, (int32_t*)nullptr);
    }
    std::vector<char> hc((size_t)cig + 16); std::vector<int32_t> hl((size_t)n);
    *scores = host_alloc<int32_t>((size_t)n);
    VMX_TRY(download(hc.data(), c->b[10].p, (size_t)cig, c->stream));
    VMX_TRY(download(hl.data(), d_len, (size_t)n, c->stream));
    VMX_TRY(download(*scores, d_score, (size_t)n, c->stream));
    VMX_HIP(hipStreamSynchronize(c->stream));
    VMX_HIP(hipGetLastError());
    cigar_strings(n, probs.data(), hc.data(), hl.data(), cigars, cigar_off);
    return VM_OK;
}

int vm_k_cigar_batch_banded(vm_ctx* c, const vm_score* sc, int eqx, int64_t n, const char* t, const int64_t* t_off, const char* q,
                            const int64_t* q_off, char** cigars, int64_t** cigar_off, int32_t** band_flag, int64_t* stats) {
    if (!c) { set_error("no context"); return VM_ERR_NO_CTX; }
    if (n > 0x7fffffff) { set_error("too many problems"); return VM_ERR_ARG; }
    VMX_HIP(hipSetDevice(c->device));
    vmx_fetch_scope fetch_scope(c);
    vmx_batch_bufs& B = *vmx_ctx_batch_bufs(c);
    VMX_TRY(upload_encode(c, t, t_off, n, c->b[0], B.tpool, c->b[2]));
    VMX_TRY(upload_encode(c, q, q_off, n, c->b[3], B.qpool, c->b[5]));
    const int ad_pct = vmx_ad_pct_env();
    vmx_round_args R; memset(&R, 0, sizeof R);
    R.ad_on = 1; R.ad_match = sc->match; R.ad_o1 = sc->o1; R.ad_e1 = sc->e1; R.ad_o2 = sc->o2; R.ad_e2 = sc->e2; R.ad_pct = ad_pct;
    std::vector<vmx_dp_prob> probs((size_t)n);
    std::vector<int64_t> keys((size_t)n);
    int64_t tb = 0, bnd = 0, run = 0, cig = 0, redo = 0;
    for (int64_t i = 0; i < n; ++i) {
        vmx_dp_prob& p = probs[i];
        p.t_off = t_off[i]; p.q_off = q_off[i]; p.tl = (int32_t)(t_off[i + 1] - t_off[i]); p.ql = (int32_t)(q_off[i + 1] - q_off[i]);
        p.tb_off = tb; p.bnd_off = bnd; p.run_off = run; p.cig_off = cig;
        tb += vmx_round_tb_bytes(R, p.tl, p.ql); keys[i] = vmx_round_key(R, p.tl, p.ql);
        if (p.tl > 0 && p.ql > 0 && VMX_DP16X4_OK(p.tl, p.ql)) redo += VMX_REDO_TB_BYTES((int64_t)p.tl, (int64_t)p.ql);
        bnd += 3 * (int64_t)(p.ql + 1); run += (int64_t)p.tl + p.ql + 2; cig += 2 * ((int64_t)p.tl + p.ql) + 16;
    }
    const int32_t nn = (int32_t)n;
    VMX_TRY(upload(B.dptab, probs.data(), (size_t)n, c->stream)); VMX_TRY(upload(B.dpsz[0], keys.data(), (size_t)n, c->stream)); VMX_TRY(upload(B.chunkn, &nn, 1, c->stream));
    VMX_TRY(B.tb.reserve((size_t)tb + 64)); VMX_TRY(B.tbredo.reserve((size_t)redo + 64)); VMX_TRY(B.bnd.reserve(sizeof(int32_t) * (size_t)(bnd + 4)));
    VMX_TRY(B.run.reserve(sizeof(uint32_t) * (size_t)(run + 4))); VMX_TRY(B.cig.reserve((size_t)cig + 16));
    VMX_TRY(B.ciglen.reserve(4 * (size_t)(n + 1))); VMX_TRY(B.cigq.reserve(4 * (size_t)(n + 1))); VMX_TRY(B.dpscore.reserve(4 * (size_t)(n + 1)));
    VMX_TRY(B.order.reserve(4 * (size_t)(2 * n + 64)));
    VMX_TRY(B.gfctl.reserve(4 * VMX_GF_SLOT)); VMX_HIP(hipMemsetAsync(B.gfctl.p, 0, 4 * VMX_GF_SLOT, c->stream));
    if (n) vmx_gapfill_chunk(c, B, *sc, ad_pct, eqx, 0, n, B.chunkn.as<int32_t>(), 0, B.gfctl.as<int32_t>(), B.order.as<int32_t>() + n + 32, redo, nullptr);
    std::vector<char> hc((size_t)cig + 16); std::vector<int32_t> hl((size_t)n), flag((size_t)n), ctl(32);
    VMX_TRY(download(hc.data(), B.cig.p, (size_t)cig, c->stream));
    VMX_TRY(download(hl.data(), B.ciglen.p, (size_t)n, c->stream));
    VMX_TRY(download(flag.data(), B.dpscore.p, (size_t)n, c->stream));
    VMX_TRY(download(ctl.data(), B.gfctl.p, ctl.size(), c->stream));
    VMX_HIP(vmx_stream_sync(c));
    VMX_HIP(hipGetLastError());
    int64_t nb = 0, eligible = 0, small = 0;
    for (int64_t i = 0; i < n; ++i) {
        const bool sm = probs[i].tl > 0 && probs[i].ql > 0 && VMX_DP16X4_OK(probs[i].tl, probs[i].ql);
        if (!sm) flag[i] = 0;
        small += sm; nb += sm && flag[i] > VMX_AD_FLAG;
        eligible += sm && vmx_ad_ns(probs[i].tl, probs[i].ql, sc->match, sc->o1, sc->e1, sc->o2, sc->e2, ad_pct & 0xffff, (ad_pct >> 16) & 0xffff) > 0;
    }
    if (stats) { stats[0] = eligible; stats[1] = nb; stats[2] = ctl[12]; stats[3] = n - small; stats[4] = ctl[18]; stats[5] = ctl[19]; }
    if (band_flag) { *band_flag = host_alloc<int32_t>((size_t)n); memcpy(*band_flag, flag.data(), sizeof(int32_t) * (size_t)n); }
    cigar_strings(n, probs.data(), hc.data(), hl.data(), cigars, cigar_off);
    return VM_OK;
}

int vm_k_cigar(vm_ctx* c, const char* t, int64_t tl, const char* q, int64_t ql, const vm_score* sc, int bw, int zdrop, int eqx, vm_cigar_out* out) {
    memset(out, 0, sizeof(*out));
    int64_t to[2] = {0, tl}, qo[2] = {0, ql};
    if (zdrop < 0) {
        char* cg = nullptr; int64_t* co = nullptr; int32_t* s = nullptr;
        int rc = vm_k_cigar_batch(c, sc, eqx, 1, t, to, q, qo, &cg, &co, &s);
        if (rc < 0) return rc;
        out->cigar = cg; out->q_e = (int32_t)ql; out->t_e = (int32_t)tl; out->score = s[0];
        free(co); free(s);
        return VM_OK;
    }
    if (sc->o1 != sc->o2 || sc->e1 != sc->e2) { set_error("vm_k_cigar: z-drop extension needs identical gap pieces (the reference calls it with 4,4,4,4)"); return VM_ERR_UNSUPPORTED; }
    int32_t *te = nullptr, *qe = nullptr, *s = nullptr;
    int rc = vm_k_extend_batch(c, sc->match, sc->mismatch, sc->o1, sc->e1, bw, zdrop, 1, t, to, q, qo, &te, &qe, &s);
    if (rc < 0) return rc;
    out->cigar = (char*)calloc(1, 1); out->t_e = te[0]; out->q_e = qe[0]; out->score = s[0];
    free(te); free(qe); free(s);
    return VM_OK;
}

void vm_chains_out_free(vm_chains_out* o) {
    free(o->need_reverse); free(o->mapq); free(o->score); free(o->fast_used); free(o->read_path_off); free(o->path_off);
    free(o->path_anchors); free(o->S); free(o->P); free(o->S_arg); free(o->gmax); free(o->opcount);
    memset(o, 0, sizeof(*o));
}

int vm_chain_global_batch(vm_ctx* c, const vm_params* prm, int kmersize, int64_t n, const int64_t* anchors, const int64_t* aoff,
                          const int64_t* readlens, int want_raw, vm_chains_out* out) {
    memset(out, 0, sizeof(*out));
    if (!c) { set_error("no context"); return VM_ERR_NO_CTX; }
    if (prm->global_maxdiff > 62) { set_error("global_maxdiff > 62 unsupported"); return VM_ERR_UNSUPPORTED; }
    const int64_t tot = aoff[n];
    if (const int64_t bad = vmx_rows_misfit(anchors, tot); bad >= 0) {
        char msg[192]; snprintf(msg, sizeof msg, "vm_chain_global_batch: anchor row %lld does not fit the device row (l in 0 ... 65535, q and q + l in int32, s in int16)", (long long)bad);
        set_error(msg); return VM_ERR_UNSUPPORTED;
    }
    VMX_HIP(hipSetDevice(c->device));
    vmx_fetch_scope fetch_scope(c);
    vmx_batch_bufs& B = *vmx_ctx_batch_bufs(c);
    const std::vector<int64_t> h_aoff(aoff, aoff + n + 1);
    std::vector<int64_t> h_roff((size_t)n + 1, 0);
    for (int64_t r = 0; r < n; ++r) h_roff[(size_t)r + 1] = h_roff[(size_t)r] + readlens[r];
    VMX_TRY(upload(B.rows, anchors, (size_t)tot * 4, c->stream)); VMX_TRY(upload(B.aoff, aoff, (size_t)n + 1, c->stream));
    VMX_TRY(upload(B.lens, readlens, (size_t)n, c->stream)); VMX_TRY(upload(B.off, h_roff.data(), (size_t)n + 1, c->stream));
    DevBuf& d_ran = c->b[0];
    VMX_TRY(d_ran.reserve(4 * (size_t)(n + 1))); VMX_HIP(hipMemsetAsync(d_ran.p, 0, 4 * (size_t)n, c->stream));
    const int rmode = prm->mode == VM_MODE_R ? 1 : (prm->mode == VM_MODE_ASM ? 2 : 0);
    double* d_score = nullptr; int32_t* d_mapq = nullptr; int32_t* d_np = nullptr;
    if (n) {
        VMX_TRY(vmx_global_stage(c, B, prm, kmersize, n, B.off.as<int64_t>(), h_roff, h_aoff, rmode, d_ran.as<int32_t>()));
        vmx_res_ptrs(B, n, &d_score, &d_mapq, &d_np);
    }
// ... 43 lines not shown
```

### vacmap_amd/csrc/vmx_host.h

```cpp
#ifndef VMX_HOST_H
#define VMX_HOST_H
#include "vmx_device.h"
#include "vmx_kernels.h"
#include "../../include/vacmapx.h"
#include <algorithm>
#include <map>
#include <cstring>
#include <string>
#include <vector>
#include <chrono>
#include <atomic>
#include <mutex>
#include <execinfo.h>

namespace vmx {

void set_error(const std::string& s);
int hip_fail(hipError_t e, const char* what, const char* file, int line);

#define VMX_HIP(expr)                                                              \
    do {                                                                           \
        hipError_t _e = (expr);                                                    \
        if (_e != hipSuccess) return vmx::hip_fail(_e, #expr, __FILE__, __LINE__);  \
    } while (0)
// ... 49 lines not shown
    std::mutex m; std::map<std::pair<std::string, int>, std::pair<long long, long long>> by_line; bool on = getenv("VMX_DBG_COPIES") != nullptr;
    void add(const char* file, int line, size_t bytes) { if (!on) return; std::lock_guard<std::mutex> g(m); const char* b = strrchr(file, '/'); auto& e = by_line[std::make_pair(std::string(b ? b + 1 : file), line)]; e.first++; e.second += (long long)bytes; }
    ~CopyCensus() { if (!on) return; for (auto& kv : by_line) fprintf(stderr, "[copies] %s:%d (%s): %lld copies, %lld bytes\n", kv.first.first.c_str(), kv.first.second < 0 ? -kv.first.second : kv.first.second, kv.first.second < 0 ? "download" : "upload", kv.second.first, kv.second.second); }
};
inline CopyCensus& copy_census() { static CopyCensus c; return c; }
inline long long& download_wait_ns() { static thread_local long long v = 0; return v; }
template <class T> int upload(DevBuf& b, const T* host, size_t n, hipStream_t st, int line = __builtin_LINE(), const char* file = __builtin_FILE()) {
    VMX_TRY(b.reserve(sizeof(T) * (n ? n : 1)));
    if (n) { VMX_HIP(hipMemcpyAsync(b.p, host, sizeof(T) * n, hipMemcpyHostToDevice, st)); copy_census().add(file, line, sizeof(T) * n); }
    return 0;
}
template <class T> int download(T* host, const void* dev, size_t n, hipStream_t st, int line = __builtin_LINE(), const char* file = __builtin_FILE()) {
    if (n) {
        const auto t0 = std::chrono::steady_clock::now();
        VMX_HIP(hipMemcpyAsync(host, dev, sizeof(T) * n, hipMemcpyDeviceToHost, st)); copy_census().add(file, -line, sizeof(T) * n);
        download_wait_ns() += std::chrono::duration_cast<std::chrono::nanoseconds>(std::chrono::steady_clock::now() - t0).count();
    }
    return 0;
}

}

struct vmx_mailbox {
    char* h = nullptr; char* d = nullptr;
    size_t up_off = 0, up_cap = 0, up_used = 0;
    size_t dn_off = 0, dn_cap = 0, dn_used = 0;
    char* big = nullptr; size_t big_cap = 0, big_used = 0;
    unsigned long long seq = 0;
    struct Pending { void* dst; const char* src; size_t bytes; const void* dev; };
    std::vector<Pending> pend;
    char* big_d = nullptr;
    unsigned long long* done_ctr = nullptr;
    bool on = false;
    long long poll_ns = 40000;
};
__global__ void k_signal(unsigned long long* word, unsigned long long v);
#define VMX_EXPORT_MAX 12
struct vmx_export_args { const char* src[VMX_EXPORT_MAX]; char* dst[VMX_EXPORT_MAX]; unsigned long long bytes[VMX_EXPORT_MAX]; int n; unsigned long long* word; unsigned long long seq; unsigned long long* done; };
__global__ void k_export(vmx_export_args A);

enum { VMX_NBUF = 64 };
struct vm_ctx {
    int device = 0;
    hipStream_t stream = nullptr;
    vmx_tables tables{};
    vmx::DevBuf tab_buf;
    vmx::DevBuf b[VMX_NBUF];
    int num_cu = 256;
    int inflight = 1;
    hipEvent_t sync_ev = nullptr;
    vmx_mailbox mb;
    hipEvent_t ev[24];
    hipEvent_t gev[48];
    int n_gev[2] = {0, 0};
    hipEvent_t kev[4] = {nullptr, nullptr, nullptr, nullptr};
    int kev_set = 0;
    int64_t n_bandfall = 0;
    int ext_mul = 1;
    long long redo_need_max = 0;
    long long geo_cap[4] = {0, 0, 0, 0}; bool geo_valid = false;
    bool run_pass1 = false;
    int32_t* rc_cur = nullptr; int rc_next = 0;
    bool force_exact = false;
    long long round_epoch = 0;
    int64_t n_syncs = 0;
    int64_t sync_wait_ns = 0, call_t0_ns = 0;
    double res_rec_per_read = 0.0, res_blob_per_base = 0.0;
    hipStream_t aux[4] = {nullptr, nullptr, nullptr, nullptr};
    hipEvent_t fork_ev = nullptr, join_ev[4] = {nullptr, nullptr, nullptr, nullptr};
    hipStream_t low = nullptr;
    hipEvent_t low_ev[2] = {nullptr, nullptr};
    int64_t last_n_minimizers = 0;
    struct vmx_local_bufs* lbufs = nullptr;
    struct vmx_extend_bufs* ebufs = nullptr;
    struct vmx_batch_bufs* bbufs = nullptr;
    struct vmx_sam_bufs* sbufs = nullptr;
};

static inline bool vmx_stream_prio_on() { static const bool on = [] { const char* e = getenv("VMX_STREAM_PRIO"); return e && atoi(e) != 0; }(); return on; }
struct vmx_lowprio {
    vm_ctx* c; bool on;
    explicit vmx_lowprio(vm_ctx* ctx) : c(ctx), on(ctx->low != nullptr) { if (on) { (void)hipEventRecord(c->low_ev[0], c->stream); (void)hipStreamWaitEvent(c->low, c->low_ev[0], 0); } }
    hipStream_t stream() const { return on ? c->low : c->stream; }
    void join() { if (on) { (void)hipEventRecord(c->low_ev[1], c->low); (void)hipStreamWaitEvent(c->stream, c->low_ev[1], 0); on = false; } }
};

int vmx_mailbox_wait(vm_ctx* c);
static inline hipError_t vmx_stream_sync(vm_ctx* c) {
    ++c->n_syncs;
    const auto t0 = std::chrono::steady_clock::now();
    hipError_t e = hipSuccess;
    if (c->mb.on) { if (vmx_mailbox_wait(c) < 0) e = hipErrorUnknown; }
    else e = hipStreamSynchronize(c->stream);
    c->sync_wait_ns += std::chrono::duration_cast<std::chrono::nanoseconds>(std::chrono::steady_clock::now() - t0).count();
    return e;
}
struct vmx_import_args { const char* src[4]; char* dst[4]; unsigned long long bytes[4]; int n; };
__global__ void k_import(vmx_import_args A);
struct vmx_push_piece { void* dev; const void* host; size_t bytes; };
static inline int vmx_push_pieces(vm_ctx* c, const vmx_push_piece* pc, int np) {
    vmx_mailbox& m = c->mb;
    static const bool by_copy = getenv("VMX_PUSH_COPIES") != nullptr;
    size_t at = (m.up_used + 63) & ~(size_t)63, need = 0;
    for (int i = 0; i < np; ++i) need += (pc[i].bytes + 63) & ~(size_t)63;
    if (!m.on || at + need > m.up_cap) { for (int i = 0; i < np; ++i) if (pc[i].bytes) VMX_HIP(hipMemcpyAsync(pc[i].dev, pc[i].host, pc[i].bytes, hipMemcpyHostToDevice, c->stream)); return 0; }
    vmx_import_args A; memset(&A, 0, sizeof A);
// ... 39 lines not shown
    vm_ctx* c;
    explicit vmx_fetch_scope(vm_ctx* ctx) : c(ctx) { drop(); }
    ~vmx_fetch_scope() { drop(); }
    void drop() { c->mb.pend.clear(); c->mb.dn_used = 0; c->mb.big_used = 0; }
};

struct vmx_fork {
    vm_ctx* c; int used = 0;
    explicit vmx_fork(vm_ctx* ctx) : c(ctx) { (void)hipEventRecord(c->fork_ev, c->stream); }
    hipStream_t next() {
        hipStream_t s = c->aux[used & 3];
        if (used < 4) (void)hipStreamWaitEvent(s, c->fork_ev, 0);
        ++used;
        return s;
    }
    void join() {
        const int n = used < 4 ? used : 4;
        for (int i = 0; i < n; ++i) { (void)hipEventRecord(c->join_ev[i], c->aux[i]); (void)hipStreamWaitEvent(c->stream, c->join_ev[i], 0); }
        used = 0;
    }
};

__global__ void k_encode(const char* in, uint8_t* out, int64_t n);
__global__ void k_edit_distance(const uint8_t* qcodes, const int64_t* q_off, const uint8_t* tcodes, const int64_t* t_off,
                                int8_t* carry_pool, const int32_t* order, const int32_t* range, int32_t* counters, int which, int64_t* out,
                                int64_t carry_stride, int32_t* oflow);
__global__ void k_size_order(const int64_t* size, const int32_t* n_ptr, int64_t thresh, int32_t* order, int32_t* range, int32_t* counters);
__global__ void k_size_hist(const int64_t* size, const int32_t* n_ptr, int64_t thresh, int32_t* ghist);
__global__ void k_size_scatter(const int64_t* size, const int32_t* n_ptr, const int32_t* ghist, int32_t* gcur, int32_t* order, int32_t* range, int32_t* counters);
static inline void vmx_size_order_wide(vm_ctx* c, const int64_t* size, const int32_t* n_ptr, int64_t n_upper, int64_t thresh, int32_t* order, int32_t* range, int32_t* counters,
                                       int32_t* scratch) {
    static const bool one_wg = getenv("VMX_SIZE_ORDER_ONE") != nullptr;
    if (one_wg) { hipLaunchKernelGGL(k_size_order, dim3(1), dim3(1024), 0, c->stream, size, n_ptr, thresh, order, range, counters); return; }
    (void)hipMemsetAsync(scratch, 0, 4 * 513, c->stream);
    const unsigned G = (unsigned)std::max<int64_t>(1, std::min<int64_t>((n_upper + 1023) / 1024, (int64_t)c->num_cu * 2));
    hipLaunchKernelGGL(k_size_hist, dim3(G), dim3(256), 0, c->stream, size, n_ptr, thresh, scratch);
    hipLaunchKernelGGL(k_size_scatter, dim3(G), dim3(256), 0, c->stream, size, n_ptr, (const int32_t*)scratch, scratch + 257, order, range, counters);
}
__global__ void k_ed_banded(const uint8_t* qcodes, const int64_t* q_off, const uint8_t* tcodes, const int64_t* t_off, const int32_t* order,
                            const int32_t* range, int32_t* counter, int64_t* ub_out);
struct vmx_ext_args;
__global__ void k_ed_banded4(const uint8_t* qcodes, const int64_t* q_off, const uint8_t* tcodes, const int64_t* t_off, const int32_t* order,
                             const int32_t* range, int32_t* counter, int64_t* ub_out);
__global__ void k_ed_flag(const int64_t* ub, const int64_t* q_off, const int64_t* t_off, const int32_t* n_ptr, double maxdiv, int64_t* sizes,
                          int64_t* ed_out, int32_t* n_flagged, int first, const int32_t* prob_read, struct vmx_ext_read* er);
__global__ void k_extend(const uint8_t* tcodes, const int64_t* t_off, const uint8_t* qcodes, const int64_t* q_off, int n_prob,
                         int match, int mismatch, int o, int e, int bw_in, int zdrop, int32_t* out_te, int32_t* out_qe, int32_t* out_sc, const int32_t* n_ptr);
__global__ void k_gapfill_fill(const uint8_t* tcodes, const uint8_t* qcodes, const vmx_dp_prob* probs, int n_prob, int match,
                               int mismatch, int o1, int e1, int o2, int e2, uint8_t* tb_pool, int32_t* bnd_pool, int32_t* out_score,
                               const int32_t* order, int32_t* counter);
__global__ void k_gapfill_fill_ns(const uint8_t* tcodes, const uint8_t* qcodes, vmx_dp_prob* probs, int n_prob, int match,
                                  int mismatch, int o1, int e1, int o2, int e2, uint8_t* tb_pool, int32_t* bnd_pool, int32_t* out_score,
                                  const int32_t* order, const int32_t* range, int32_t* counter, int32_t* redo_list, int32_t* redo_cnt, int ad_pct,
                                  unsigned long long* redo_bytes, const int32_t* n_ptr = nullptr, unsigned long long redo_cap = ~0ULL, int tb_by_ns = 0);
__global__ void k_gapfill_redo(const uint8_t* tcodes, const uint8_t* qcodes, const vmx_dp_prob* probs, int match, int mismatch, int o1, int e1, int o2, int e2,
                               uint8_t* tb_pool, int32_t* bnd_pool, int32_t* out_score, int32_t* redo_list, int32_t* redo_cnt, uint8_t* redo_pool);
static inline int vmx_ad_pct_env(int mode = 0) {
    int pct = mode == 1 ? 40 : 90, pmin = mode == 1 ? 40 : VMX_AD_PCT_MIN_DEFAULT;
    if (const char* e = getenv("VMX_AD_PCT")) { const int v = atoi(e); if (v >= 0 && v <= 60000) pct = v; }
    if (const char* e = getenv("VMX_AD_PCT_MIN")) { const int v = atoi(e); if (v >= 0 && v <= 60000) pmin = v; }
    return pct | (pmin << 16);
}
__global__ void k_gapfill_trace(const uint8_t* tcodes, const uint8_t* qcodes, const vmx_dp_prob* probs, int n_prob, int eqx,
                                const uint8_t* tb_pool, uint32_t* run_pool, char* cig_pool, int32_t* cig_len, const int32_t* band_flag, const uint8_t* redo_pool, int spread, int32_t* cig_q, const int32_t* n_ptr = nullptr);
__global__ void k_flip_sort(const int64_t* rows, const int64_t* aoff, const int64_t* readlens, int n_reads, uint64_t* key_pool,
                            const int64_t* key_off, vmx_anchor* sorted, int32_t* need_reverse);
__global__ void k_chain_global(const vmx_anchor* anchors, const int64_t* aoff, const int32_t* rlist, int nlist, int lds_cap,
                               vmx_tables tab, const double* gapcost_list, double oskipcost, int omaxdiff, int maxgap,
                               double* S_out, int32_t* P_out, int32_t* SA_out, uint8_t* cov_pool, int64_t* gmax_out, int64_t* opcount_out, int rmode,
                               double* FP_pool, double* PP_pool);
static inline int64_t vmx_rows_misfit(const int64_t* rows, int64_t n) {
    for (int64_t i = 0; i < n; ++i) {
        const int64_t q = rows[4 * i], s = rows[4 * i + 2], l = rows[4 * i + 3];
        if (l < 0 || l > 65535 || q < INT32_MIN || q > INT32_MAX || q + l > INT32_MAX || s < INT16_MIN || s > INT16_MAX) return i;
    }
    return -1;
}
__global__ void k_chain_global_rows(const vmx_anchor* anchors, const int64_t* aoff, const int32_t* rlist, int nlist, vmx_tables tab, const double* gapcost_list,
                                    double oskipcost, int omaxdiff, int maxgap, double* S_out, int32_t* P_out, int32_t* SA_out, uint8_t* cov_pool,
                                    int64_t* gmax_out, int64_t* opcount_out, int rmode, double* FP_pool, double* PP_pool, unsigned long long* dbg);
__global__ void k_chain_global_rows_w3(const vmx_anchor* anchors, const int64_t* aoff, const int32_t* rlist, int nlist, vmx_tables tab, const double* gapcost_list,
                                       double oskipcost, int omaxdiff, int maxgap, double* S_out, int32_t* P_out, int32_t* SA_out, uint8_t* cov_pool,
                                       int64_t* gmax_out, int64_t* opcount_out, int rmode, double* FP_pool, double* PP_pool, unsigned long long* dbg);
static inline bool vmx_chain_rows_win3() { const char* e = getenv("VMX_RW_WIN"); return e && atoi(e) == 3; }
unsigned long long* vmx_chain_dbg();
void vmx_chain_dbg_report(hipStream_t st);
static inline bool vmx_chain_rows_on() { static const bool on = [] { const char* e = getenv("VMX_CHAIN_ROWS"); return !e || atoi(e) != 0; }(); return on; }
__global__ void k_chain_global_fast(const vmx_anchor* anchors, const int64_t* aoff, int n_reads, const int64_t* roff, vmx_tables tab,
                                    const double* gapcost_list, double oskipcost, int omaxdiff, int maxgap, double* S_out, int32_t* P_out, int32_t* SA_out,
                                    uint8_t* cov_pool, int32_t* si_pool, int64_t* t_pool, int32_t* cnt_pool, int64_t* gmax_out, int32_t* ran, int rmode,
                                    double* FP_pool, double* PP_pool);
__global__ void k_chain_select(const vmx_anchor* anchors, const int64_t* aoff, const int64_t* readlens, const int32_t* rlist, int nlist, int lds_cap,
                               const double* S, const int32_t* P, const int32_t* SA, const int64_t* gmax, const int32_t* need_reverse, int mode,
                               char* scratch, const int64_t* scratch_off, int32_t* out_mapq, double* out_score, int32_t* out_npaths,
                               int32_t* out_path_len, vmx_anchor* out_path_anchors);

#endif
```

### vacmap_amd/csrc/vmx_kernels.h

```cpp
#ifndef VMX_KERNELS_H
#define VMX_KERNELS_H
#include <stdint.h>

struct vmx_dp_prob {
    int64_t t_off, q_off;
    int32_t tl, ql;
    int64_t tb_off;
    int64_t bnd_off;
    int64_t run_off;
    int64_t cig_off;
};

struct vmx_anchor {
    int32_t q;
    int16_t l;
    int16_t s;
    int64_t r;
};

struct vmx_slot { uint64_t key; uint32_t start; uint32_t count; };

struct vmx_tables {
    const float* extra; int32_t extra_n;
    const float* readgap_h; const float* readgap_r; const float* large_readgap;
// ... 86 lines not shown
#define VMX_SORT_LDS 4096
#ifdef VMX_EMU
#define VMX_SORT_LDS_BIG 8192
#else
#define VMX_SORT_LDS_BIG 16384
#endif
#define VM_READ_FASTPATH_DEV (-21)
#ifdef VMX_EMU
#define VMX_DP16_MAX 420
#else
#define VMX_DP16_MAX 6000
#endif
#define VMX_DP16_OK(tl, ql) ((tl) + (ql) <= VMX_DP16_MAX)
#ifdef VMX_EMU
#define VMX_DP16X4_MAX 160
#else
#define VMX_DP16X4_MAX 1024
#endif
#define VMX_DP16X4_OK(tl, ql) ((tl) + (ql) <= VMX_DP16X4_MAX)
#define VMX_X4_W(ql) ((((ql) + 31) + 15) & ~15)
#define VMX_AD_NS_MAX 4
__host__ __device__ static inline int vmx_ad_geom_nd(int tl, int ql, int nd, int* dlo_out) {
    const int dl = ql - tl, lo = dl < 0 ? dl : 0, hi = dl > 0 ? dl : 0;
    const int slack = nd - (hi - lo + 1);
    if (slack < 0) return 0;
    int mb = slack / 2, dlo = lo - mb;
    if (dlo & 1) {
        if (mb + 1 <= slack) { ++mb; --dlo; }
        else if (mb >= 1) { --mb; ++dlo; }
        else return 0;
    }
    *dlo_out = dlo;
    const int ma = slack - mb;
    return (mb < ma ? mb : ma) + 1;
}
__host__ __device__ static inline int vmx_ad_geom(int tl, int ql, int ns, int* dlo_out) { return vmx_ad_geom_nd(tl, ql, 32 * ns, dlo_out); }
__host__ __device__ static inline long long vmx_ad_margin(int g, int match, int o1, int e1, int o2, int e2) {
    const long long c1 = o1 + (long long)g * e1, c2 = o2 + (long long)g * e2;
    return (long long)match * g + 2 * (c1 < c2 ? c1 : c2);
}
__host__ __device__ static inline int vmx_ad_ns_nd(int tl, int ql, int match, int o1, int e1, int o2, int e2, int pct, int pct_min, int dpn, int ns_lo, int ns_hi) {
    if (tl <= 0 || ql <= 0) return 0;
    const int mn = tl < ql ? tl : ql;
    int dlo, g = 0;
    for (int ns = ns_lo; ns <= ns_hi; ++ns) {
        g = vmx_ad_geom_nd(tl, ql, dpn * ns, &dlo);
        if (g >= 1 && (g > mn || vmx_ad_margin(g, match, o1, e1, o2, e2) * 100 >= (long long)pct * mn)) return ns;
    }
    return (g >= 1 && vmx_ad_margin(g, match, o1, e1, o2, e2) * 100 >= (long long)pct_min * mn) ? ns_hi : 0;
}
__host__ __device__ static inline int vmx_ad_ns(int tl, int ql, int match, int o1, int e1, int o2, int e2, int pct, int pct_min) {
    return vmx_ad_ns_nd(tl, ql, match, o1, e1, o2, e2, pct, pct_min, 32, 1, VMX_AD_NS_MAX);
}
#define VMX_AD_PCT_DEFAULT 100
#define VMX_AD_PCT_MIN_DEFAULT 65
#ifdef VMX_EMU
#define VMX_ADW_DPN 36
#else
#define VMX_ADW_DPN 128
#endif
#define VMX_ADW_NS_MIN 2
#define VMX_ADW_PCT 100
#define VMX_ADW_PCT_MIN 65
#define VMX_AD_FLAG 16
#define VMX_PK_FLAG 1
#ifdef VMX_EMU
#define VMX_REDO_PK(tl, ql) ((tl) > 0 && (ql) > 0 && VMX_DP16X4_OK(tl, ql) && (tl) + (ql) >= 120)
#else
#ifndef VMX_REDO_PK_MIN
#define VMX_REDO_PK_MIN 384
#endif
#define VMX_REDO_PK(tl, ql) ((tl) > 0 && (ql) > 0 && VMX_DP16X4_OK(tl, ql) && (tl) + (ql) >= VMX_REDO_PK_MIN)
#endif
#define VMX_PK_TB_BYTES(tl, ql) ((int64_t)(((tl) + 127) / 128) * ((ql) + 127) * 128)
#ifndef VMX_AD_AB
#define VMX_AD_AB 4
#endif
static_assert(VMX_AD_AB == 1 || 64 / VMX_AD_AB <= 16, "a 64-byte line of the anti-diagonal traceback holds at most the 16 lanes of a row per anti-diagonal (1-byte slots): AB = 1, 4 or 8");
#define VMX_AD_TB_OFF(s, l) ((((size_t)(s) & ~(size_t)(VMX_AD_AB - 1)) << 6) + ((size_t)(s) & (VMX_AD_AB - 1)) * (64 / VMX_AD_AB) + ((size_t)(l) / (16 / VMX_AD_AB)) * 64 + ((size_t)(l) % (16 / VMX_AD_AB)) * 4)
#define VMX_AD_TB_BYTES(tl, ql) ((int64_t)(((tl) + (ql) + VMX_AD_AB - 1) & ~(VMX_AD_AB - 1)) * 64)
#define VMX_AD_W(ns) ((ns) <= 0 ? 0 : ((ns) == 1 ? 1 : ((ns) == 2 ? 2 : 4)))
#define VMX_AD_TB_OFF_W(s, l, W) (((size_t)(s) / VMX_AD_AB) * (size_t)(VMX_AD_AB * 16 * (W)) + ((size_t)(l) / (64 / (VMX_AD_AB * (W)))) * 64 + ((size_t)(s) % VMX_AD_AB) * (64 / VMX_AD_AB) + ((size_t)(l) % (64 / (VMX_AD_AB * (W)))) * (W))
#define VMX_AD_TB_BYTES_W(tl, ql, W) ((int64_t)(((tl) + (ql) + VMX_AD_AB - 1) & ~(VMX_AD_AB - 1)) * 16 * (W))
#define VMX_X4_TB_BYTES(tl, ql) ((int64_t)(((tl) + 31) / 32) * VMX_X4_W(ql) * 32)
#define VMX_TB_BYTES(tl, ql) (((tl) > 0 && (ql) > 0) ? (VMX_DP16X4_OK(tl, ql) ? VMX_X4_TB_BYTES(tl, ql) : \
                              VMX_DP16_OK(tl, ql) ? VMX_PK_TB_BYTES(tl, ql) : (int64_t)(((tl) + 63) / 64) * ((ql) + 63) * 64) : 0)
#define VMX_TB_BYTES_NS(tl, ql) (((tl) > 0 && (ql) > 0 && VMX_DP16X4_OK(tl, ql)) ? VMX_AD_TB_BYTES(tl, ql) : VMX_TB_BYTES(tl, ql))
#define VMX_REDO_TB_BYTES(tl, ql) (VMX_REDO_PK(tl, ql) ? VMX_PK_TB_BYTES(tl, ql) : VMX_X4_TB_BYTES(tl, ql))
__device__ __forceinline__ uint8_t* vmx_tb_ptr(const uint8_t* tb_pool, const uint8_t* redo_pool, int64_t off) {
    const unsigned long long base = off >= 0 ? (unsigned long long)tb_pool : (unsigned long long)redo_pool;
    return (uint8_t*)(base + (unsigned long long)(off >= 0 ? off : -off - 1));
}
#define VMX_HEAD_THRESH (((int64_t)1 << 18) - 1)
#define VMX_TB_CHUNK ((int64_t)4 << 30)
#ifdef VMX_EMU
#define VMX_MAX_BATCH_BASES 20000
#define VMX_MAX_BATCH_READS 6
#else
#define VMX_MAX_BATCH_BASES ((int64_t)160 << 20)
#define VMX_MAX_BATCH_READS 16384
#endif
#define VMX_LA_SLOT(len) ((len) / 2 + 4096)
#define VMX_SELECT_LDS 3072
#define VMX_LC_LDS_MAX_DEFAULT 13056
#define VMX_GC_LDS_MAX_DEFAULT 13056
#define VMX_CHAIN_LDS_MAX_SHARED 512
// ... 5 lines not shown
```

### vacmap_amd/csrc/vmx_stage.h

```cpp
#ifndef VMX_STAGE_H
#define VMX_STAGE_H
#include "vmx_host.h"

struct vm_index_view {
    const uint8_t* codes; const int64_t* coff; int nseq; int64_t total_len;
    const uint64_t* pos; const vmx_slot* table; int table_bits; int k, w, mid_occ;
};
void vmx_index_view(const vm_index* mi, vm_index_view* v);

struct vmx_preset { const vmx_anchor* chain_desc; int64_t len; };

struct vmx_local_bufs {
    vmx::DevBuf sq, dst, rorder, pc2, stg, si, tg, cntp, fp, pp, prep_ws;
    vmx::DevBuf guide_rows, guide_len, ng_used, ng_total, cnt, cur, tpos, hkey, hkey2, dbg, hval, hq, goff, pcnt, gkey, gq, gr, epoch;
    vmx::DevBuf la_rows, la_ekey, la_sorted, la_off, la_cnt, status, gap, rlist, S, P, SA, chain, chain_len, score, variant;
    int64_t la_pool_rows = 0;
    std::vector<int64_t> h_la_off;
    std::vector<int32_t> h_la_cnt;
    void release() {
        vmx::DevBuf* all[] = {&prep_ws, &sq, &dst, &rorder, &pc2, &stg, &si, &tg, &cntp, &fp, &pp, &dbg, &epoch, &hkey2, &guide_rows, &guide_len, &ng_used, &ng_total, &cnt, &cur, &tpos, &hkey, &hval, &hq, &goff, &pcnt, &gkey, &gq, &gr,
                              &la_rows, &la_ekey, &la_sorted, &la_off, &la_cnt, &status, &gap, &rlist, &S, &P, &SA, &chain, &chain_len, &score, &variant};
        for (auto* b : all) b->release();
    }
};
vmx_local_bufs* vmx_ctx_local_bufs(vm_ctx* c);

struct vmx_batch_bufs {
    vmx::DevBuf seed[13];
    vmx::DevBuf nanc64, aoff, rows, lens, keys, koff, sorted, flip, S, P, SA, cov, gmax, opc, rl, gap, scr, soff, res, plen, prow, ocodes;
    vmx::DevBuf er, coff3, soff2, segA, st, en, segA_s, st_s, en_s, segprob, dup, desc[2], rcount, oflow, probread, tl, ql, toff, qoff, tpool, qpool;
    vmx::DevBuf edout, carry, ext3, dpsz[4], dpoff[4], dptab, tb, tbredo, bnd, run, cig, ciglen, dpscore, rec, blob, bloboff, reccoff, recclen, dupd, totals;
    vmx::DevBuf raw, codes, off, order, qrange, scanpart, scanoff, si, tg, cntp, fp, pp, chunkn, sellist, cigq, statblk, szh, side_codes, side_off, roundpart, gfctl, geotot;
    void release() { vmx::DevBuf* p = (vmx::DevBuf*)this; for (size_t i = 0; i < sizeof(*this) / sizeof(vmx::DevBuf); ++i) p[i].release(); }
};
vmx_batch_bufs* vmx_ctx_batch_bufs(vm_ctx* c);

int vmx_global_stage(vm_ctx* c, vmx_batch_bufs& B, const vm_params* prm, int k, int64_t n, const int64_t* d_roff, const std::vector<int64_t>& h_roff,
                     const std::vector<int64_t>& h_aoff, int rmode, int32_t* d_ran);
static inline void vmx_res_ptrs(vmx_batch_bufs& B, int64_t n, double** score, int32_t** mapq, int32_t** np) {
    *score = B.res.as<double>(); *mapq = (int32_t*)(*score + n + 1); *np = *mapq + n + 1;
}

#define VMX_GF_SLOT (32 + 544)
void vmx_gapfill_chunk(vm_ctx* c, vmx_batch_bufs& B, const vm_score& sc, int ad_pct, int eqx, int p0, int64_t pn, const int32_t* n_ptr, int64_t tb_off0,
                       int32_t* ctl, int32_t* redo_list, int64_t redo_cap, hipEvent_t* ke);

extern "C" int vmx_seed_stage(vm_ctx* c, const vm_index* mi, int check_num, int mid_occ, int64_t n, const uint8_t* d_codes, const int64_t* d_roff, int64_t total_bases,
                   vmx::DevBuf* B, std::vector<int64_t>& h_koff, std::vector<int64_t>& h_nhits, vmx::DevBuf* arena = nullptr, int64_t** rows_out = nullptr);
int vmx_local_stage(vm_ctx* c, const vm_index_view& ix, const vm_params* prm, int64_t n, const uint8_t* d_ocodes, const int64_t* d_roff,
                    const std::vector<int64_t>& h_roff, const vmx_anchor* d_path_rows, const int32_t* d_path_len, const int32_t* d_npaths,
                    const int64_t* d_aoff, const std::vector<int64_t>& h_aoff, const double* d_gscore, vmx_local_bufs& L, bool fast = false);
int vmx_launch_chain_select(vm_ctx* c, int64_t n, const int64_t* h_aoff, vmx::DevBuf& d_list, const vmx_anchor* sorted, const int64_t* d_aoff, const int64_t* d_lens,
                            const double* S, const int32_t* P, const int32_t* SA, const int64_t* gmax, const int32_t* flip, int mode, char* scr, const int64_t* soff,
                            int32_t* d_mapq, double* d_score, int32_t* d_np, int32_t* plen, vmx_anchor* prow);
#endif
```

### vacmap_amd/lib.py

```python
import ctypes as C
import os
import numpy as np

_HERE = os.path.dirname(os.path.abspath(__file__))
DEFAULT_SO = os.environ.get('VACMAPX_LIB') or os.path.join(_HERE, 'libvacmapx.so')

VM_ERR_NO_DEVICE = -2
MODES = {'H': 0, 'L': 1, 'S': 2, 'R': 3, 'asm': 4}


class VmxError(RuntimeError):
    def __init__(self, code, msg):
        super().__init__('vacmapx error %d: %s' % (code, msg))
        self.code = code


class Params(C.Structure):
    _fields_ = [('mode', C.c_int32), ('check_num', C.c_int32), ('mid_occ', C.c_int32), ('global_maxdiff', C.c_int32),
                ('local_maxdiff', C.c_int32), ('local_kmersize', C.c_int32), ('eqx', C.c_int32), ('hardclip', C.c_int32),
                ('nodiscard', C.c_int32), ('reserved', C.c_int32), ('global_skipcost', C.c_double),
                ('local_skipcost', C.c_double), ('maxdivergence', C.c_double)]


class Score(C.Structure):
    _fields_ = [('match', C.c_int32), ('mismatch', C.c_int32), ('o1', C.c_int32), ('e1', C.c_int32), ('o2', C.c_int32), ('e2', C.c_int32)]


class CigarOut(C.Structure):
    _fields_ = [('cigar', C.c_void_p), ('q_e', C.c_int32), ('t_e', C.c_int32), ('score', C.c_int32)]


class ChainsOut(C.Structure):
    _fields_ = [('need_reverse', C.POINTER(C.c_int32)), ('mapq', C.POINTER(C.c_int32)), ('score', C.POINTER(C.c_double)),
                ('fast_used', C.POINTER(C.c_int32)), ('read_path_off', C.POINTER(C.c_int64)), ('path_off', C.POINTER(C.c_int64)),
                ('path_anchors', C.POINTER(C.c_int64)), ('S', C.POINTER(C.c_double)), ('P', C.POINTER(C.c_int64)),
                ('S_arg', C.POINTER(C.c_int64)), ('gmax', C.POINTER(C.c_int64)), ('opcount', C.POINTER(C.c_int64))]


class LinkedOut(C.Structure):
    _fields_ = [('gmax', C.c_int64), ('n_hot', C.c_int64), ('n_cold', C.c_int64), ('opcount', C.c_int64), ('cold_max', C.c_double),
                ('S', C.POINTER(C.c_double)), ('P', C.POINTER(C.c_int64)), ('S_arg_hot', C.POINTER(C.c_int64)),
                ('carry_status', C.c_int32), ('saved', C.c_int32), ('n_carry', C.c_int64), ('carry_S', C.POINTER(C.c_double)),
                ('carry_P', C.POINTER(C.c_int64)), ('carry_rows', C.POINTER(C.c_int64)), ('carry_g_max_scores', C.c_double), ('carry_prereadloc', C.c_int64)]


class LocalOut(C.Structure):
    _fields_ = [('status', C.POINTER(C.c_int32)), ('variant', C.POINTER(C.c_int32)), ('score', C.POINTER(C.c_double)),
                ('chain_off', C.POINTER(C.c_int64)), ('chain', C.POINTER(C.c_int64)), ('raw_off', C.POINTER(C.c_int64)),
                ('raw', C.POINTER(C.c_int64))]


class Record(C.Structure):
    _fields_ = [('read_idx', C.c_int32), ('contig', C.c_int32), ('strand', C.c_int32), ('mapq', C.c_int32),
                ('q_st', C.c_int64), ('q_en', C.c_int64), ('r_st', C.c_int64), ('r_en', C.c_int64),
                ('cigar_off', C.c_int64), ('cigar_len', C.c_int64)]


class SamOpts(C.Structure):
    _fields_ = [('md', C.c_int32), ('shortcs', C.c_int32), ('cigar2cg', C.c_int32), ('markunbalancetra', C.c_int32), ('hardclip', C.c_int32),
                ('fakecigar', C.c_int32), ('rg_id', C.c_char_p), ('asm_mode', C.c_int32)]


class BatchStats(C.Structure):
    _fields_ = [(n, C.c_int64) for n in ('n_reads', 'read_bases', 'n_minimizers', 'n_hits', 'n_anchors', 'n_local_hits', 'n_local_anchors',
                                          'n_segments', 'n_ed_problems', 'ed_cells', 'n_ext_problems', 'ext_cells', 'n_dp_problems',
                                          'dp_cells', 'n_records', 'cigar_bytes', 'aligned_bases', 'n_unmapped', 'n_failed',
                                          'dp_string_bytes')] + \
               [('ms_total', C.c_double), ('ms_stage', C.c_double * 16), ('ms_gapfill_fill', C.c_double), ('ms_gapfill_trace', C.c_double),
                ('n_gapfill_launches', C.c_int64), ('n_ed_full', C.c_int64), ('n_ed_tier2', C.c_int64), ('n_ed_tier1', C.c_int64),
                ('n_dp_redo', C.c_int64), ('dp_redo_tb_bytes', C.c_int64), ('ms_local_seed', C.c_double), ('ms_cluster', C.c_double), ('n_host_syncs', C.c_int64), ('n_local_general', C.c_int64), ('n_ext_retries', C.c_int64), ('n_batch_retries', C.c_int64),
                ('n_dp_redo_wide', C.c_int64), ('n_dp_redo_full', C.c_int64)]


def _b(s):
    return s if isinstance(s, (bytes, bytearray)) else s.encode()


def _cat(seqs):
    bs = [_b(s) for s in seqs]
    off = np.zeros(len(bs) + 1, np.int64)
    if bs:
        off[1:] = np.cumsum([len(b) for b in bs])
    return b''.join(bs), off


def _seq_ptrs(seqs):
    keep, ptrs, lens = [], [], []
    for x in seqs:
        if isinstance(x, np.ndarray):
            a = np.ascontiguousarray(x, dtype=np.uint8)
            keep.append(a); ptrs.append(a.ctypes.data); lens.append(a.size)
        else:
            b = C.create_string_buffer(_b(x), len(x)) if len(x) else C.create_string_buffer(1)
            keep.append(b); ptrs.append(C.addressof(b)); lens.append(len(x))
    n = len(ptrs)
    arr = (C.c_void_p * max(n, 1))(*ptrs)
    return keep, C.cast(arr, C.POINTER(C.c_char_p)), (C.c_int64 * max(n, 1))(*lens)


class VmxLib:

    def __init__(self, path=None):
        path = path or DEFAULT_SO
        try:
            if os.environ.get('VACMAPX_SKIP_TORCH') == '1' and 'torch' not in __import__('sys').modules:
                raise ImportError('single-GPU command line: no torch, the library brings the system HIP runtime (saves ~1.5 s of start-up)')
            import torch
        except ImportError:
            pass
        if not os.path.exists(path):
            raise FileNotFoundError('%s not built: run `python -m vacmap_amd.build` (hipcc, gfx950). No fallback exists.' % path)
        L = self.L = C.CDLL(path)
        vp, i32, i64, dbl, cp, P = C.c_void_p, C.c_int32, C.c_int64, C.c_double, C.c_char_p, C.POINTER
        L.vm_last_error.restype = cp
        L.vm_version.restype = cp
        L.vm_free.argtypes = [vp]
        L.vm_params_default.argtypes = [P(Params), C.c_int]
        L.vm_ctx_create.argtypes = [C.c_int, P(vp)]
        L.vm_ctx_destroy.argtypes = [vp]
        L.vm_ctx_set_inflight.argtypes = [vp, C.c_int]
        L.vm_ctx_set_blocking_sync.argtypes = [vp, C.c_int]
        L.vm_debug_chain_counters.argtypes = [C.c_int, C.POINTER(C.c_ulonglong)]
        L.vm_ctx_mem_info.argtypes = [vp, P(i64), P(i64)]
        L.vm_table.argtypes = [vp, C.c_int, P(vp)]; L.vm_table.restype = i64
        L.vm_edit_distance_batch.argtypes = [vp, i64, cp, vp, cp, vp, P(P(i64))]
        L.vm_edit_distance_bound_batch.argtypes = [vp, C.c_int, i64, cp, vp, cp, vp, P(P(i64))]
        L.vm_edit_distance.argtypes = [vp, cp, i64, cp, i64]; L.vm_edit_distance.restype = i64
        L.vm_k_extend_batch.argtypes = [vp] + [C.c_int] * 6 + [i64, cp, vp, cp, vp, P(P(i32)), P(P(i32)), P(P(i32))]
        L.vm_k_cigar_batch.argtypes = [vp, P(Score), C.c_int, i64, cp, vp, cp, vp, P(vp), P(P(i64)), P(P(i32))]
        L.vm_k_cigar.argtypes = [vp, cp, i64, cp, i64, P(Score), C.c_int, C.c_int, C.c_int, P(CigarOut)]
        L.vm_k_cigar_batch_banded.argtypes = [vp, P(Score), C.c_int, i64, cp, vp, cp, vp, P(vp), P(P(i64)), P(P(i32)), vp]
        L.vm_chain_global_batch.argtypes = [vp, P(Params), C.c_int, i64, vp, vp, vp, C.c_int, P(ChainsOut)]
        L.vm_chain_linked.argtypes = [vp, C.c_int, C.c_int, C.c_double, C.c_int, C.c_int, i64, vp, i64, vp, vp, C.c_double, i64, i64, P(LinkedOut)]
        L.vm_linked_out_free.argtypes = [P(LinkedOut)]
        L.vm_align_asm.argtypes = [vp, vp, P(Params), C.c_char_p, i64, i64, i64, i64, P(P(Record)), P(i64), P(vp), P(C.c_int32)]
        L.vm_chains_out_free.argtypes = [P(ChainsOut)]
        L.vm_index_build_fasta.argtypes = [vp, cp, C.c_int, C.c_int, P(vp)]
        L.vm_index_build_mem.argtypes = [vp, C.c_int, P(cp), P(cp), P(i64), C.c_int, C.c_int, P(vp)]
        L.vm_index_save.argtypes = [vp, cp]; L.vm_index_load.argtypes = [vp, cp, P(vp)]
        L.vm_index_save_mmi.argtypes = [vp, cp, C.c_int]; L.vm_index_load_mmi.argtypes = [vp, cp, P(vp)]
        L.vm_index_free.argtypes = [vp]
        for f in ('vm_index_k', 'vm_index_w', 'vm_index_nseq', 'vm_index_mid_occ', 'vm_index_blob_count'):
            getattr(L, f).argtypes = [vp]
        L.vm_index_n_minimizers.argtypes = [vp]; L.vm_index_n_minimizers.restype = i64
        L.vm_index_n_distinct.argtypes = [vp]; L.vm_index_n_distinct.restype = i64
        L.vm_index_seq_info.argtypes = [vp, C.c_int, P(cp), P(i64), P(i64)]
        L.vm_index_seq.argtypes = [vp, C.c_int, i64, i64, vp]; L.vm_index_seq.restype = i64
        L.vm_index_minimizers.argtypes = [vp, P(P(C.c_uint64)), P(P(C.c_uint64)), P(i64)]
        L.vm_index_blob.argtypes = [vp, C.c_int, P(vp), P(i64)]
        L.vm_index_meta_size.argtypes = [vp, P(i64)]; L.vm_index_meta_get.argtypes = [vp, vp, i64]
        L.vm_index_from_meta.argtypes = [vp, vp, i64, P(vp)]
        L.vm_sketch_batch.argtypes = [vp, C.c_int, C.c_int, i64, cp, vp, P(P(C.c_uint64)), P(P(i32)), P(P(C.c_int8)), P(P(i64))]
        L.vm_map_batch.argtypes = [vp, vp, C.c_int, C.c_int, i64, cp, vp, P(P(i64)), P(P(i64))]
        L.vm_map.argtypes = [vp, vp, cp, i64, C.c_int, C.c_int, P(P(i64)), P(i64)]
        L.vm_local_chain_batch.argtypes = [vp, vp, P(Params), i64, cp, vp, vp, vp, vp, P(LocalOut)]
        L.vm_local_out_free.argtypes = [P(LocalOut)]
        L.vm_align_batch.argtypes = [vp, vp, P(Params), i64, cp, vp, P(P(Record)), P(i64), P(vp), vp, P(BatchStats)]
        L.vm_align_trace.argtypes = [vp, vp, P(Params), i64, cp, vp, C.c_int, P(P(i64)), P(P(i64))]
        L.vm_sam_emit.argtypes = [vp, P(SamOpts), i64, vp, vp, vp, vp, vp, vp, vp, vp, vp, i64, vp, vp, C.c_int, P(vp), P(P(i64)), P(i64), P(i64)]
        L.vm_sam_emit_device.argtypes = [vp, vp, P(SamOpts), i64, vp, vp, vp, vp, vp, vp, vp, i64, vp, vp, P(vp), P(P(i64)), P(i64), P(i64)]
        L.vm_sam_emit_device_times.argtypes = [vp, P(dbl)]
        L.vm_blob_gather.argtypes = [vp, vp, vp, i64, vp, vp]; L.vm_blob_gather.restype = i64
        L.vm_blob_write_parts.argtypes = [C.c_int, vp, vp, vp, vp, i64]; L.vm_blob_write_parts.restype = i64
        L.vm_pinned_alloc.argtypes = [i64, C.c_int]; L.vm_pinned_alloc.restype = vp
        L.vm_pinned_free.argtypes = [vp]; L.vm_pinned_free.restype = None
        L.vm_blob_gather_parts.argtypes = [vp, vp, vp, vp, i64, vp]; L.vm_blob_gather_parts.restype = i64
        L.vm_blob_write_parts_mmap.argtypes = [C.c_int, i64, vp, vp, vp, vp, i64, C.c_int]; L.vm_blob_write_parts_mmap.restype = i64
        L.vm_fastx_open.argtypes = [cp, P(vp)]; L.vm_fastx_close.argtypes = [vp]; L.vm_fastx_open_range.argtypes = [cp, i64, i64, P(vp)]
        L.vm_fastx_read.argtypes = [vp, i64, i64] + [P(vp), P(P(i64))] * 4; L.vm_fastx_read.restype = i64
        L.vm_reads_upload.argtypes = [vp, i64, cp, vp, P(vp)]
        L.vm_reads_free.argtypes = [vp]
        L.vm_reads_reupload.argtypes = [vp, vp, i64, vp, vp]
        L.vm_align_resident.argtypes = [vp, vp, P(Params), vp, P(P(Record)), P(i64), P(vp), vp, P(BatchStats)]
        L.vm_bam_writer_create.argtypes = [vp, cp, i64, P(vp)]
        L.vm_bam_writer_free.argtypes = [vp]; L.vm_bam_writer_free.restype = None
        L.vm_bam_header.argtypes = [vp, P(vp), P(i64)]
        L.vm_bam_encode.argtypes = [vp, cp, i64, P(vp), P(i64)]
        L.vm_bam_compress_parts.argtypes = [vp, vp, vp, vp, vp, i64, P(vp), P(i64)]
        L.vm_bam_sorter_create.argtypes = [vp, i64, P(vp)]
        L.vm_bam_sorter_free.argtypes = [vp]; L.vm_bam_sorter_free.restype = None
        L.vm_bam_sorter_add_parts.argtypes = [vp, vp, vp, vp, vp, i64, P(vp), P(i64)]
        L.vm_bam_sorter_plan.argtypes = [vp, vp, i64, i64, P(i64)]
        L.vm_bam_sorter_chunk.argtypes = [vp, i64, P(vp), P(i64)]
        L.vm_bam_sorter_index.argtypes = [vp, P(vp), P(i64)]
# ... 67 lines not shown
        except Exception:
            pass

    def _take(self, ptr, n, dtype):
        a = np.ctypeslib.as_array(ptr, shape=(max(int(n), 1),))[:int(n)].astype(dtype, copy=True)
        self.lib.L.vm_free(ptr)
        return a

    def table(self, which):
        p = C.c_void_p()
        n = self.lib.check(self.lib.L.vm_table(self.h, which, C.byref(p)))
        ty = C.c_float if which < 4 else C.c_double
        a = np.ctypeslib.as_array(C.cast(p, C.POINTER(ty)), shape=(n,)).copy()
        self.lib.L.vm_free(p)
        return a

    def edit_distance_batch(self, queries, targets):
        q, qo = _cat(queries); t, to = _cat(targets)
        out = C.POINTER(C.c_int64)()
        self.lib.check(self.lib.L.vm_edit_distance_batch(self.h, len(queries), q, qo.ctypes.data, t, to.ctypes.data, C.byref(out)))
        return self._take(out, len(queries), np.int64)

    def edit_distance_bound_batch(self, queries, targets, tier=2):
        q, qo = _cat(queries); t, to = _cat(targets)
        out = C.POINTER(C.c_int64)()
        self.lib.check(self.lib.L.vm_edit_distance_bound_batch(self.h, tier, len(queries), q, qo.ctypes.data, t, to.ctypes.data, C.byref(out)))
        return self._take(out, len(queries), np.int64)

    def edit_distance(self, q, t):
        q, t = _b(q), _b(t)
        return self.lib.check(self.lib.L.vm_edit_distance(self.h, q, len(q), t, len(t)))

    def k_extend_batch(self, targets, queries, match=2, mismatch=-4, o=4, e=4, bw=100, zdrop=50):
        t, to = _cat(targets); q, qo = _cat(queries)
        te = C.POINTER(C.c_int32)(); qe = C.POINTER(C.c_int32)(); sc = C.POINTER(C.c_int32)()
        n = len(targets)
        self.lib.check(self.lib.L.vm_k_extend_batch(self.h, match, mismatch, o, e, bw, zdrop, n, t, to.ctypes.data, q, qo.ctypes.data,
                                                    C.byref(te), C.byref(qe), C.byref(sc)))
        return self._take(sc, n, np.int32), self._take(te, n, np.int32), self._take(qe, n, np.int32)

    def k_cigar_batch(self, targets, queries, match=2, mismatch=-4, o1=4, e1=2, o2=24, e2=1, eqx=False):
        t, to = _cat(targets); q, qo = _cat(queries)
        n = len(targets)
        sc = Score(match, mismatch, o1, e1, o2, e2)
        cg = C.c_void_p(); co = C.POINTER(C.c_int64)(); ss = C.POINTER(C.c_int32)()
        self.lib.check(self.lib.L.vm_k_cigar_batch(self.h, C.byref(sc), int(eqx), n, t, to.ctypes.data, q, qo.ctypes.data,
                                                   C.byref(cg), C.byref(co), C.byref(ss)))
        off = self._take(co, n + 1, np.int64)
        blob = C.string_at(cg.value, int(off[-1])) if off[-1] else b''
        self.lib.L.vm_free(cg)
        cigars = [blob[off[i]:off[i + 1] - 1].decode() for i in range(n)]
        return cigars, self._take(ss, n, np.int32)

    def k_cigar_batch_banded(self, targets, queries, match=2, mismatch=-4, o1=4, e1=2, o2=24, e2=1, eqx=False):
        t, to = _cat(targets); q, qo = _cat(queries)
        n = len(targets)
        sc = Score(match, mismatch, o1, e1, o2, e2)
        cg = C.c_void_p(); co = C.POINTER(C.c_int64)(); fl = C.POINTER(C.c_int32)(); st = (C.c_int64 * 6)()
        self.lib.check(self.lib.L.vm_k_cigar_batch_banded(self.h, C.byref(sc), int(eqx), n, t, to.ctypes.data, q, qo.ctypes.data,
                                                          C.byref(cg), C.byref(co), C.byref(fl), st))
        off = self._take(co, n + 1, np.int64)
        blob = C.string_at(cg.value, int(off[-1])) if off[-1] else b''
        self.lib.L.vm_free(cg)
        cigars = [blob[off[i]:off[i + 1] - 1].decode() for i in range(n)]
        return cigars, self._take(fl, n, np.int32), {'eligible': st[0], 'proven': st[1], 'redo': st[2], 'not_eligible': st[3],
                                                          'redo_wide': st[4], 'redo_full': st[5]}

    def k_cigar(self, target, query, match=2, mismatch=-4, gap_open_1=4, gap_extend_1=2, gap_open_2=24, gap_extend_2=1,
                bw=-1, zdropvalue=-1, eqx=False):
        t, q = _b(target), _b(query)
        sc = Score(match, mismatch, gap_open_1, gap_extend_1, gap_open_2, gap_extend_2)
        out = CigarOut()
        self.lib.check(self.lib.L.vm_k_cigar(self.h, t, len(t), q, len(q), C.byref(sc), bw, zdropvalue, int(eqx), C.byref(out)))
        cg = C.string_at(out.cigar).decode() if out.cigar else ''
        self.lib.L.vm_free(out.cigar)
        return cg, 0, out.q_e, out.t_e, 0, 0

    def chain_global_batch(self, prm, kmersize, anchors_list, readlens, want_raw=False):
        n = len(anchors_list)
        aoff = np.zeros(n + 1, np.int64)
        for i, a in enumerate(anchors_list):
            aoff[i + 1] = aoff[i] + len(a)
        rows = np.ascontiguousarray(np.concatenate([np.asarray(a, dtype=np.int64).reshape(-1, 4) for a in anchors_list]) if n else np.zeros((0, 4), np.int64))
        rl = np.ascontiguousarray(readlens, dtype=np.int64)
        out = ChainsOut()
        self.lib.check(self.lib.L.vm_chain_global_batch(self.h, C.byref(prm), kmersize, n, rows.ctypes.data, aoff.ctypes.data, rl.ctypes.data,
                                                        int(want_raw), C.byref(out)))
        res = []
        rpo = np.ctypeslib.as_array(out.read_path_off, shape=(n + 1,)).copy()
        npaths = int(rpo[-1])
        po = np.ctypeslib.as_array(out.path_off, shape=(npaths + 1,)).copy()
        nrows = int(po[-1])
        pa = np.ctypeslib.as_array(out.path_anchors, shape=(max(nrows, 1), 4))[:nrows].copy()
        tot = int(aoff[-1])
        for r in range(n):
            d = {'need_reverse': bool(out.need_reverse[r]), 'mapq': int(out.mapq[r]), 'score': float(out.score[r]),
                 'fast_used': bool(out.fast_used[r]), 'gmax': int(out.gmax[r]), 'opcount': int(out.opcount[r]),
                 'paths': [pa[po[p]:po[p + 1]] for p in range(rpo[r], rpo[r + 1])]}
            if want_raw:
                a, b = int(aoff[r]), int(aoff[r + 1])
                d['S'] = np.ctypeslib.as_array(out.S, shape=(max(tot, 1),))[a:b].copy()
                d['P'] = np.ctypeslib.as_array(out.P, shape=(max(tot, 1),))[a:b].copy()
                d['S_arg'] = np.ctypeslib.as_array(out.S_arg, shape=(max(tot, 1),))[a:b].copy()
            res.append(d)
        self.lib.L.vm_chains_out_free(C.byref(out))
        return res

    def sketch_batch(self, k, w, seqs):
        s, off = _cat(seqs)
        n = len(seqs)
        h = C.POINTER(C.c_uint64)(); p = C.POINTER(C.c_int32)(); z = C.POINTER(C.c_int8)(); oo = C.POINTER(C.c_int64)()
        self.lib.check(self.lib.L.vm_sketch_batch(self.h, k, w, n, s, off.ctypes.data, C.byref(h), C.byref(p), C.byref(z), C.byref(oo)))
        o = self._take(oo, n + 1, np.int64)
        m = int(o[-1])
        H = self._take(h, m, np.uint64); Pp = self._take(p, m, np.int32); Z = self._take(z, m, np.int8)
        return [(H[o[i]:o[i + 1]], Pp[o[i]:o[i + 1]], Z[o[i]:o[i + 1]]) for i in range(n)]

    def map(self, index, seq, check_num=100, mid_occ=-1):
        sq = _b(seq)
# ... 622 lines not shown
```

Baseline: 3.515.

## Certify narrower anti-diagonal DP band widths using bit-parallel edit-distance bound

Adds a per-problem pre-pass kernel that computes an edit-distance upper bound with a Myers bit-vector scan and derives a certified band width for the gap-fill anti-diagonal DP. When that width is no wider than the heuristic rule, the fill kernel uses it, and the size key used for bucketing is recomputed to match. The aim is to shrink DP bands and avoid failed band attempts followed by full redo. The cost is an extra kernel launch per chunk plus scanning every sequence pair, and the path is on by default behind an env switch.

```diff
diff --git a/include/vacmapx.h b/include/vacmapx.h
--- a/include/vacmapx.h
+++ b/include/vacmapx.h
@@ -121,6 +121,11 @@
                      const int64_t* q_off, char** cigars, int64_t** cigar_off, int32_t** scores);
 int vm_k_cigar_batch_banded(vm_ctx*, const vm_score*, int eqx, int64_t n, const char* t, const int64_t* t_off, const char* q,
                             const int64_t* q_off, char** cigars, int64_t** cigar_off, int32_t** band_flag, int64_t* stats);
+int vm_k_cigar_batch_banded_cert(vm_ctx*, const vm_score*, int eqx, int64_t n, const char* t, const int64_t* t_off, const char* q,
+                                 const int64_t* q_off, char** cigars, int64_t** cigar_off, int32_t** band_flag, int64_t* stats);
+void vm_ad_cert(const vm_score* sc, int tl, int ql, int64_t ed_ub, int64_t* out);
+int64_t vm_ad_width_key(int ns, int tl, int ql);
+int64_t vm_ad_ed_ub(const uint8_t* tcodes, int tl, const uint8_t* qcodes, int ql);
 int vm_k_extend_batch(vm_ctx*, int match, int mismatch, int o, int e, int bw, int zdrop, int64_t n, const char* t,
                       const int64_t* t_off, const char* q, const int64_t* q_off, int32_t** t_e, int32_t** q_e, int32_t** score);
 typedef struct vm_cigar_out { char* cigar; int32_t q_e, t_e, score; } vm_cigar_out;
@@ -165,6 +170,10 @@
     int64_t n_batch_retries;
     int64_t n_dp_redo_wide;
     int64_t n_dp_redo_full;
+    int64_t n_dp_cert;
+    int64_t n_dp_cert_narrower;
+    int64_t n_dp_cert_unproven;
+    double ms_gapfill_width;
 } vm_batch_stats;
 
 int vm_align_batch(vm_ctx*, const vm_index*, const vm_params*, int64_t n_reads, const char* seqs, const int64_t* offsets,
diff --git a/vacmap_amd/csrc/k_dp.hip b/vacmap_amd/csrc/k_dp.hip
--- a/vacmap_amd/csrc/k_dp.hip
+++ b/vacmap_amd/csrc/k_dp.hip
@@ -466,7 +466,7 @@
                                                    int match, int mismatch, int o1, int e1, int o2, int e2, uint8_t* __restrict__ tb_pool, int32_t* __restrict__ bnd_pool,
                                                    int32_t* __restrict__ out_score, const int32_t* __restrict__ order, const int32_t* __restrict__ range, int32_t* __restrict__ counter,
                                                    int32_t* __restrict__ redo_list, int32_t* __restrict__ redo_cnt, int ad_pct, unsigned long long* __restrict__ redo_bytes,
-                                                   unsigned long long redo_cap, int tb_by_ns) {
+                                                   unsigned long long redo_cap, int tb_by_ns, const uint8_t* __restrict__ adw) {
     const int lane = vmx_lane();
     const int pct = ad_pct & 0xffff, pct_min = (ad_pct >> 16) & 0xffff;
     const bool ad_ok = vmx_ad_scores_ok(match, mismatch, o1, e1, o2, e2);
@@ -490,12 +490,15 @@
         if (pX >= 0) prX = probs[pX];
         if (pY >= 0) prY = probs[pY];
         const bool x4X = pX >= 0 && prX.tl > 0 && prX.ql > 0 && VMX_DP16X4_OK(prX.tl, prX.ql), x4Y = pY >= 0 && prY.tl > 0 && prY.ql > 0 && VMX_DP16X4_OK(prY.tl, prY.ql);
-        const int nsX = x4X && ad_ok ? vmx_ad_ns(prX.tl, prX.ql, match, o1, e1, o2, e2, pct, pct_min) : 0, nsY = x4Y && ad_ok ? vmx_ad_ns(prY.tl, prY.ql, match, o1, e1, o2, e2, pct, pct_min) : 0;
+        const int bX = adw && x4X ? (int)adw[pX] : 0, bY = adw && x4Y ? (int)adw[pY] : 0;
+        const int nsX = !(x4X && ad_ok) ? 0 : (adw ? VMX_ADW_NS(bX) : vmx_ad_ns(prX.tl, prX.ql, match, o1, e1, o2, e2, pct, pct_min));
+        const int nsY = !(x4Y && ad_ok) ? 0 : (adw ? VMX_ADW_NS(bY) : vmx_ad_ns(prY.tl, prY.ql, match, o1, e1, o2, e2, pct, pct_min));
         const int ns = vmx_uniform_i32(vmx_wave_max_i32(nsX > nsY ? nsX : nsY));
         bool keepX = false, keepY = false, triedX = false, triedY = false;
         if (ns > 0) {
             int dloX = 0, dloY = 0;
-            const bool fitX = !tb_by_ns || VMX_AD_W(nsX) == VMX_AD_W(ns), fitY = !tb_by_ns || VMX_AD_W(nsY) == VMX_AD_W(ns);
+            const int szX = adw ? VMX_ADW_SIZED(bX) : VMX_AD_W(nsX), szY = adw ? VMX_ADW_SIZED(bY) : VMX_AD_W(nsY);
+            const bool fitX = !tb_by_ns || VMX_AD_W(ns) <= szX, fitY = !tb_by_ns || VMX_AD_W(ns) <= szY;
             const int gX = (nsX > 0 && fitX) ? vmx_ad_geom(prX.tl, prX.ql, ns, &dloX) : 0, gY = (nsY > 0 && fitY) ? vmx_ad_geom(prY.tl, prY.ql, ns, &dloY) : 0;
             const int tlX = gX > 0 ? prX.tl : 0, qlX = gX > 0 ? prX.ql : 0, tlY = gY > 0 ? prY.tl : 0, qlY = gY > 0 ? prY.ql : 0;
             int scX = 0, scY = 0;
@@ -512,6 +515,7 @@
                 out_score[pX] = keepX ? VMX_AD_FLAG + ns : 0;
                 if (!keepX) {
                     if (triedX) atomicAdd(redo_cnt + 3, 1);
+                    if (triedX && (bX & VMX_ADW_CERT)) atomicAdd(redo_cnt + 10, 1);
                     const unsigned long long need = (unsigned long long)VMX_REDO_TB_BYTES(prX.tl, prX.ql), at = atomicAdd(redo_bytes, need);
                     if (at + need > redo_cap) { probs[pX].tl = 0; probs[pX].ql = 0; probs[pX].tb_off = 0; }
                     else { probs[pX].tb_off = -(int64_t)at - 1; redo_list[atomicAdd(redo_cnt, 1)] = pX; }
@@ -521,6 +525,7 @@
                 out_score[pY] = keepY ? VMX_AD_FLAG + ns : 0;
                 if (!keepY) {
                     if (triedY) atomicAdd(redo_cnt + 3, 1);
+                    if (triedY && (bY & VMX_ADW_CERT)) atomicAdd(redo_cnt + 10, 1);
                     const unsigned long long need = (unsigned long long)VMX_REDO_TB_BYTES(prY.tl, prY.ql), at = atomicAdd(redo_bytes, need);
                     if (at + need > redo_cap) { probs[pY].tl = 0; probs[pY].ql = 0; probs[pY].tb_off = 0; }
                     else { probs[pY].tb_off = -(int64_t)at - 1; redo_list[atomicAdd(redo_cnt, 1)] = pY; }
@@ -549,9 +554,30 @@
                                                         const int32_t* __restrict__ order, const int32_t* __restrict__ range, int32_t* __restrict__ counter,
                                                         int32_t* __restrict__ redo_list, int32_t* __restrict__ redo_cnt, int ad_pct,
                                                         unsigned long long* __restrict__ redo_bytes, const int32_t* __restrict__ n_ptr,
-                                                        unsigned long long redo_cap, int tb_by_ns) {
+                                                        unsigned long long redo_cap, int tb_by_ns, const uint8_t* __restrict__ adw) {
     if (n_ptr) n_prob = *n_ptr;
-    vmx_gapfill_ad_pass(tcodes, qcodes, probs, n_prob, match, mismatch, o1, e1, o2, e2, tb_pool, bnd_pool, out_score, order, range, counter, redo_list, redo_cnt, ad_pct, redo_bytes, redo_cap, tb_by_ns);
+    vmx_gapfill_ad_pass(tcodes, qcodes, probs, n_prob, match, mismatch, o1, e1, o2, e2, tb_pool, bnd_pool, out_score, order, range, counter, redo_list, redo_cnt, ad_pct, redo_bytes, redo_cap, tb_by_ns, adw);
+}
+__global__ void __launch_bounds__(256) k_gapfill_width(const uint8_t* __restrict__ tcodes, const uint8_t* __restrict__ qcodes, const vmx_dp_prob* __restrict__ probs, int n_prob,
+                                                       const int32_t* __restrict__ n_ptr, int match, int mismatch, int o1, int e1, int o2, int e2, int ad_pct,
+                                                       uint8_t* __restrict__ adw, int64_t* __restrict__ key, int32_t* __restrict__ cnt) {
+    if (n_ptr) n_prob = *n_ptr;
+    const int pct = ad_pct & 0xffff, pct_min = (ad_pct >> 16) & 0xffff;
+    const bool ad_ok = vmx_ad_scores_ok(match, mismatch, o1, e1, o2, e2);
+    for (int p = (int)(blockIdx.x * blockDim.x + threadIdx.x); p < n_prob; p += (int)(gridDim.x * blockDim.x)) {
+        const vmx_dp_prob pr = probs[p];
+        if (!(ad_ok && pr.tl > 0 && pr.ql > 0 && VMX_DP16X4_OK(pr.tl, pr.ql))) { adw[p] = 0; continue; }
+        const int rule = vmx_ad_ns(pr.tl, pr.ql, match, o1, e1, o2, e2, pct, pct_min);
+        int ns = rule, cert = 0;
+        if (rule >= 2) {
+            const int nc = vmx_ad_ns_cert(pr.tl, pr.ql, vmx_ad_ed_ub(tcodes + pr.t_off, pr.tl, qcodes + pr.q_off, pr.ql), match, mismatch, o1, e1, o2, e2);
+            if (nc > 0 && VMX_AD_W(nc) <= VMX_AD_W(rule)) { ns = nc; cert = VMX_ADW_CERT; }
+        }
+        adw[p] = (uint8_t)(ns | cert | (VMX_AD_W(rule) << 5));
+        key[p] = vmx_ad_width_key(ns, pr.tl, pr.ql);
+        if (cert) atomicAdd(cnt, 1);
+        if (cert && ns < rule) atomicAdd(cnt + 1, 1);
+    }
 }
 __global__ void __launch_bounds__(64) k_gapfill_redo(const uint8_t* __restrict__ tcodes, const uint8_t* __restrict__ qcodes, const vmx_dp_prob* __restrict__ probs,
                                                      int match, int mismatch, int o1, int e1, int o2, int e2, uint8_t* __restrict__ tb_pool,
diff --git a/vacmap_amd/csrc/vmx_align.hip b/vacmap_amd/csrc/vmx_align.hip
--- a/vacmap_amd/csrc/vmx_align.hip
+++ b/vacmap_amd/csrc/vmx_align.hip
@@ -166,7 +166,7 @@
 }
 
 void vmx_gapfill_chunk(vm_ctx* c, vmx_batch_bufs& B, const vm_score& sc, int ad_pct, int eqx, int p0, int64_t pn, const int32_t* n_ptr, int64_t tb_off0,
-                       int32_t* ctl, int32_t* redo_list, int64_t redo_cap, hipEvent_t* ke) {
+                       int32_t* ctl, int32_t* redo_list, int64_t redo_cap, hipEvent_t* ke, hipEvent_t* we, bool cert) {
     int fill_waves = 16;
     if (const char* e = getenv("VMX_FILL_WAVES")) { const int v = atoi(e); if (v >= 1 && v <= 32) fill_waves = v; }
     static const int tr_spread = [] { const char* e = getenv("VMX_TRACE_SPREAD"); const int v = e ? atoi(e) : 1; return v >= 1 && v <= 64 ? v : 1; }();
@@ -175,6 +175,12 @@
     uint8_t* tb_base = B.tb.as<uint8_t>() - tb_off0;
     vmx_dp_prob* probs = B.dptab.as<vmx_dp_prob>() + p0; int32_t* score = B.dpscore.as<int32_t>() + p0;
     const unsigned Gs = (unsigned)std::max<int64_t>(1, std::min<int64_t>((pn + 1023) / 1024, (int64_t)c->num_cu * 2));
+    uint8_t* adw = cert ? B.adw.as<uint8_t>() + p0 : nullptr;
+    if (we) (void)hipEventRecord(we[0], c->stream);
+    if (cert)
+        hipLaunchKernelGGL(k_gapfill_width, dim3((unsigned)std::max<int64_t>(1, std::min<int64_t>((pn + 255) / 256, (int64_t)c->num_cu * 8))), dim3(256), 0, c->stream, B.tpool.as<uint8_t>(), B.qpool.as<uint8_t>(),
+                           (const vmx_dp_prob*)probs, (int)pn, n_ptr, sc.match, sc.mismatch, sc.o1, sc.e1, sc.o2, sc.e2, ad_pct, adw, B.dpsz[0].as<int64_t>() + p0, ctl + 20);
+    if (we) (void)hipEventRecord(we[1], c->stream);
     hipLaunchKernelGGL(k_size_hist, dim3(Gs), dim3(256), 0, c->stream, B.dpsz[0].as<int64_t>() + p0, n_ptr, (int64_t)((1LL << 42) - 1), scratch);
     hipLaunchKernelGGL(k_size_scatter, dim3(Gs), dim3(256), 0, c->stream, B.dpsz[0].as<int64_t>() + p0, n_ptr, (const int32_t*)scratch, scratch + 257, B.order.as<int32_t>(), d_range, d_cnt);
     if (ke) (void)hipEventRecord(ke[0], c->stream);
@@ -182,7 +188,7 @@
         vmx_lowprio lp(c);
         hipLaunchKernelGGL(k_gapfill_fill_ns, dim3((unsigned)std::max<int64_t>(1, std::min<int64_t>(pn, (int64_t)c->num_cu * fill_waves))), dim3(64), 0, lp.stream(), B.tpool.as<uint8_t>(), B.qpool.as<uint8_t>(),
                            probs, (int)pn, sc.match, sc.mismatch, sc.o1, sc.e1, sc.o2, sc.e2, tb_base, B.bnd.as<int32_t>(), score, B.order.as<int32_t>(), d_range, d_cnt,
-                           redo_list, d_redo_cnt, ad_pct, d_redo_bytes, n_ptr, (unsigned long long)redo_cap, 1);
+                           redo_list, d_redo_cnt, ad_pct, d_redo_bytes, n_ptr, (unsigned long long)redo_cap, 1, (const uint8_t*)adw);
         lp.join();
     }
     hipLaunchKernelGGL(k_gapfill_redo, dim3((unsigned)std::max<int64_t>(1, std::min<int64_t>(pn, (int64_t)c->num_cu * 4))), dim3(64), 0, c->stream, B.tpool.as<uint8_t>(), B.qpool.as<uint8_t>(),
@@ -526,18 +532,19 @@
     const bool ad_pinned = getenv("VMX_AD_PCT") != nullptr || getenv("VMX_AD_PCT_MIN") != nullptr;
     const int ad_pct = ad_pinned ? vmx_ad_pct_env(prm->mode) : (ad_cur | (std::max(20, ad_cur - 25) << 16));
     static const int64_t tb_chunk = [] { const char* e = getenv("VMX_TB_CHUNK_GB"); const double v = e ? atof(e) : 0.0; return v > 0.5 ? (int64_t)(v * (double)(1 << 30)) : (int64_t)VMX_TB_CHUNK; }();
+    static const bool ad_cert = [] { const char* e = getenv("VMX_AD_CERT"); return !(e && atoi(e) == 0); }();
     int gf_chunks[2] = {0, 0}; int64_t gf_redo_cap = 0;
     auto gf_chunk = [&](int pass, int q, int p0, int64_t pn, const int32_t* n_ptr, int64_t tb_off0) {
         int32_t* ctl = B.gfctl.as<int32_t>() + (size_t)(pass * (VMX_MAX_CHUNKS + 1) + q) * VMX_GF_SLOT;
         hipEvent_t* ke = q < 8 ? c->gev + (pass ? 24 : 0) + 3 * q : nullptr;
-        vmx_gapfill_chunk(c, B, gf_score, ad_pct, prm->eqx, p0, pn, n_ptr, tb_off0, ctl, B.order.as<int32_t>() + round_cap + 32, gf_redo_cap, ke);
+        vmx_gapfill_chunk(c, B, gf_score, ad_pct, prm->eqx, p0, pn, n_ptr, tb_off0, ctl, B.order.as<int32_t>() + round_cap + 32, gf_redo_cap, ke, ke ? c->wev + (pass ? 16 : 0) + 2 * q : nullptr, ad_cert);
         if (ke) c->n_gev[pass] = q + 1;
         gf_chunks[pass] = q + 1;
     };
     auto gapfill = [&](int redo_only) -> int {
         for (int i = 0; i < 4; ++i) { VMX_TRY(B.dpsz[i].reserve(8 * (size_t)(round_cap + 2))); VMX_TRY(B.dpoff[i].reserve(8 * (size_t)(round_cap + 2))); }
         VMX_TRY(B.dptab.reserve(sizeof(vmx_dp_prob) * (size_t)(round_cap + 1))); VMX_TRY(B.ciglen.reserve(4 * (size_t)(round_cap + 1))); VMX_TRY(B.cigq.reserve(4 * (size_t)(round_cap + 1))); VMX_TRY(B.dpscore.reserve(4 * (size_t)(round_cap + 1)));
-        VMX_TRY(B.order.reserve(4 * (size_t)(2 * round_cap + 64)));
+        VMX_TRY(B.order.reserve(4 * (size_t)(2 * round_cap + 64))); VMX_TRY(B.adw.reserve((size_t)round_cap + 64));
         if (!redo_only) {
             gf_redo_cap = std::max<int64_t>((int64_t)((double)c->redo_need_max * 1.3), std::min<int64_t>((int64_t)512 << 20, std::max<int64_t>(tb_chunk / 8, 1 << 20)));
             if (const char* e = getenv("VMX_TEST_REDO_POOL_BYTES")) { const long long v = atoll(e); if (v > 0 && c->redo_need_max == 0) gf_redo_cap = v; }
@@ -670,7 +677,7 @@
             for (int q = 0; q < gf_chunks[pass]; ++q) {
                 const int32_t* ctl = h_ctl.data() + (size_t)(pass * (VMX_MAX_CHUNKS + 1) + q) * VMX_GF_SLOT;
                 unsigned long long rb = 0; memcpy(&rb, ctl + 16, 8);
-                st.n_dp_redo += ctl[12]; st.n_dp_redo_wide += ctl[18]; st.n_dp_redo_full += ctl[19]; st.dp_redo_tb_bytes += (int64_t)rb; st.dp_cells += (int64_t)rb; ad_failed += ctl[15];
+                st.n_dp_redo += ctl[12]; st.n_dp_redo_wide += ctl[18]; st.n_dp_redo_full += ctl[19]; st.n_dp_cert += ctl[20]; st.n_dp_cert_narrower += ctl[21]; st.n_dp_cert_unproven += ctl[22]; st.dp_redo_tb_bytes += (int64_t)rb; st.dp_cells += (int64_t)rb; ad_failed += ctl[15];
                 need_max = std::max<int64_t>(need_max, (int64_t)rb);
             }
         c->redo_need_max = std::max<long long>(c->redo_need_max, need_max);
@@ -726,6 +733,7 @@
             hipEvent_t* ke = c->gev + 24 * pass + 3 * q;
             if (hipEventElapsedTime(&ms, ke[0], ke[1]) == hipSuccess) st.ms_gapfill_fill += ms;
             if (hipEventElapsedTime(&ms, ke[1], ke[2]) == hipSuccess) st.ms_gapfill_trace += ms;
+            if (hipEventElapsedTime(&ms, c->wev[16 * pass + 2 * q], c->wev[16 * pass + 2 * q + 1]) == hipSuccess) st.ms_gapfill_width += ms;
             st.n_gapfill_launches++;
         }
     if (stats) *stats = st;
@@ -782,7 +790,7 @@
             tot.ms_total += st.ms_total; for (int i = 0; i < 16; ++i) tot.ms_stage[i] += st.ms_stage[i];
             tot.ms_gapfill_fill += st.ms_gapfill_fill; tot.ms_gapfill_trace += st.ms_gapfill_trace; tot.n_gapfill_launches += st.n_gapfill_launches;
             tot.n_ed_full += st.n_ed_full; tot.n_ed_tier2 += st.n_ed_tier2; tot.n_ed_tier1 += st.n_ed_tier1;
-            tot.n_dp_redo += st.n_dp_redo; tot.n_dp_redo_wide += st.n_dp_redo_wide; tot.n_dp_redo_full += st.n_dp_redo_full; tot.dp_redo_tb_bytes += st.dp_redo_tb_bytes; tot.ms_local_seed += st.ms_local_seed; tot.ms_cluster += st.ms_cluster; tot.n_host_syncs += st.n_host_syncs; tot.n_local_general += st.n_local_general; tot.n_ext_retries += st.n_ext_retries; tot.n_batch_retries += st.n_batch_retries;
+            tot.n_dp_redo += st.n_dp_redo; tot.n_dp_redo_wide += st.n_dp_redo_wide; tot.n_dp_redo_full += st.n_dp_redo_full; tot.n_dp_cert += st.n_dp_cert; tot.n_dp_cert_narrower += st.n_dp_cert_narrower; tot.n_dp_cert_unproven += st.n_dp_cert_unproven; tot.ms_gapfill_width += st.ms_gapfill_width; tot.dp_redo_tb_bytes += st.dp_redo_tb_bytes; tot.ms_local_seed += st.ms_local_seed; tot.ms_cluster += st.ms_cluster; tot.n_host_syncs += st.n_host_syncs; tot.n_local_general += st.n_local_general; tot.n_ext_retries += st.n_ext_retries; tot.n_batch_retries += st.n_batch_retries;
         }
     }
     *recs = (vm_record*)malloc(sizeof(vm_record) * std::max<size_t>(all.size(), 1)); *cigar_blob = (char*)malloc(std::max<size_t>(blob.size(), 1));
diff --git a/vacmap_amd/csrc/vmx_capi.hip b/vacmap_amd/csrc/vmx_capi.hip
--- a/vacmap_amd/csrc/vmx_capi.hip
+++ b/vacmap_amd/csrc/vmx_capi.hip
@@ -253,6 +253,7 @@
     else c->low = nullptr;
     for (int i = 0; i < 24; ++i) (void)hipEventCreate(&c->ev[i]);
     for (int i = 0; i < 48; ++i) (void)hipEventCreate(&c->gev[i]);
+    for (int i = 0; i < 32; ++i) (void)hipEventCreate(&c->wev[i]);
     for (int i = 0; i < 4; ++i) (void)hipEventCreate(&c->kev[i]);
     for (int i = 0; i < 4; ++i) { if (prio) (void)hipStreamCreateWithPriority(&c->aux[i], hipStreamDefault, prio_greatest); else (void)hipStreamCreate(&c->aux[i]); (void)hipEventCreate(&c->join_ev[i]); }
     (void)hipEventCreate(&c->fork_ev);
@@ -304,6 +305,7 @@
     vmx::devbuf_retired().flush();
     for (int i = 0; i < 24; ++i) (void)hipEventDestroy(c->ev[i]);
     for (int i = 0; i < 48; ++i) (void)hipEventDestroy(c->gev[i]);
+    for (int i = 0; i < 32; ++i) (void)hipEventDestroy(c->wev[i]);
     for (int i = 0; i < 4; ++i) (void)hipEventDestroy(c->kev[i]);
     for (int i = 0; i < 4; ++i) { (void)hipStreamSynchronize(c->aux[i]); (void)hipStreamDestroy(c->aux[i]); (void)hipEventDestroy(c->join_ev[i]); }
     (void)hipEventDestroy(c->fork_ev);
@@ -510,8 +512,8 @@
     return VM_OK;
 }
 
-int vm_k_cigar_batch_banded(vm_ctx* c, const vm_score* sc, int eqx, int64_t n, const char* t, const int64_t* t_off, const char* q,
-                            const int64_t* q_off, char** cigars, int64_t** cigar_off, int32_t** band_flag, int64_t* stats) {
+static int cigar_batch_banded(vm_ctx* c, const vm_score* sc, int eqx, int64_t n, const char* t, const int64_t* t_off, const char* q,
+                              const int64_t* q_off, char** cigars, int64_t** cigar_off, int32_t** band_flag, int64_t* stats, bool cert) {
     if (!c) { set_error("no context"); return VM_ERR_NO_CTX; }
     if (n > 0x7fffffff) { set_error("too many problems"); return VM_ERR_ARG; }
     VMX_HIP(hipSetDevice(c->device));
@@ -538,9 +540,9 @@
     VMX_TRY(B.tb.reserve((size_t)tb + 64)); VMX_TRY(B.tbredo.reserve((size_t)redo + 64)); VMX_TRY(B.bnd.reserve(sizeof(int32_t) * (size_t)(bnd + 4)));
     VMX_TRY(B.run.reserve(sizeof(uint32_t) * (size_t)(run + 4))); VMX_TRY(B.cig.reserve((size_t)cig + 16));
     VMX_TRY(B.ciglen.reserve(4 * (size_t)(n + 1))); VMX_TRY(B.cigq.reserve(4 * (size_t)(n + 1))); VMX_TRY(B.dpscore.reserve(4 * (size_t)(n + 1)));
-    VMX_TRY(B.order.reserve(4 * (size_t)(2 * n + 64)));
+    VMX_TRY(B.order.reserve(4 * (size_t)(2 * n + 64))); VMX_TRY(B.adw.reserve((size_t)n + 64));
     VMX_TRY(B.gfctl.reserve(4 * VMX_GF_SLOT)); VMX_HIP(hipMemsetAsync(B.gfctl.p, 0, 4 * VMX_GF_SLOT, c->stream));
-    if (n) vmx_gapfill_chunk(c, B, *sc, ad_pct, eqx, 0, n, B.chunkn.as<int32_t>(), 0, B.gfctl.as<int32_t>(), B.order.as<int32_t>() + n + 32, redo, nullptr);
+    if (n) vmx_gapfill_chunk(c, B, *sc, ad_pct, eqx, 0, n, B.chunkn.as<int32_t>(), 0, B.gfctl.as<int32_t>(), B.order.as<int32_t>() + n + 32, redo, nullptr, nullptr, cert);
     std::vector<char> hc((size_t)cig + 16); std::vector<int32_t> hl((size_t)n), flag((size_t)n), ctl(32);
     VMX_TRY(download(hc.data(), B.cig.p, (size_t)cig, c->stream));
     VMX_TRY(download(hl.data(), B.ciglen.p, (size_t)n, c->stream));
@@ -555,11 +557,27 @@
         small += sm; nb += sm && flag[i] > VMX_AD_FLAG;
         eligible += sm && vmx_ad_ns(probs[i].tl, probs[i].ql, sc->match, sc->o1, sc->e1, sc->o2, sc->e2, ad_pct & 0xffff, (ad_pct >> 16) & 0xffff) > 0;
     }
-    if (stats) { stats[0] = eligible; stats[1] = nb; stats[2] = ctl[12]; stats[3] = n - small; stats[4] = ctl[18]; stats[5] = ctl[19]; }
+    if (stats) { stats[0] = eligible; stats[1] = nb; stats[2] = ctl[12]; stats[3] = n - small; stats[4] = ctl[18]; stats[5] = ctl[19]; if (cert) { stats[6] = ctl[20]; stats[7] = ctl[21]; stats[8] = ctl[22]; stats[9] = ctl[15]; } }
     if (band_flag) { *band_flag = host_alloc<int32_t>((size_t)n); memcpy(*band_flag, flag.data(), sizeof(int32_t) * (size_t)n); }
     cigar_strings(n, probs.data(), hc.data(), hl.data(), cigars, cigar_off);
     return VM_OK;
 }
+
+int vm_k_cigar_batch_banded(vm_ctx* c, const vm_score* sc, int eqx, int64_t n, const char* t, const int64_t* t_off, const char* q,
+                            const int64_t* q_off, char** cigars, int64_t** cigar_off, int32_t** band_flag, int64_t* stats) {
+    return cigar_batch_banded(c, sc, eqx, n, t, t_off, q, q_off, cigars, cigar_off, band_flag, stats, false);
+}
+int vm_k_cigar_batch_banded_cert(vm_ctx* c, const vm_score* sc, int eqx, int64_t n, const char* t, const int64_t* t_off, const char* q,
+                                 const int64_t* q_off, char** cigars, int64_t** cigar_off, int32_t** band_flag, int64_t* stats) {
+    return cigar_batch_banded(c, sc, eqx, n, t, t_off, q, q_off, cigars, cigar_off, band_flag, stats, true);
+}
+
+void vm_ad_cert(const vm_score* sc, int tl, int ql, int64_t ed_ub, int64_t* out) {
+    out[0] = vmx_ad_cert_C(sc->match, sc->mismatch, sc->o1, sc->e1, sc->o2, sc->e2);
+    out[1] = vmx_ad_ns_cert(tl, ql, ed_ub, sc->match, sc->mismatch, sc->o1, sc->e1, sc->o2, sc->e2);
+}
+int64_t vm_ad_width_key(int ns, int tl, int ql) { return vmx_ad_width_key(ns, tl, ql); }
+int64_t vm_ad_ed_ub(const uint8_t* tcodes, int tl, const uint8_t* qcodes, int ql) { return vmx_ad_ed_ub(tcodes, tl, qcodes, ql); }
 
 int vm_k_cigar(vm_ctx* c, const char* t, int64_t tl, const char* q, int64_t ql, const vm_score* sc, int bw, int zdrop, int eqx, vm_cigar_out* out) {
     memset(out, 0, sizeof(*out));
diff --git a/vacmap_amd/csrc/vmx_host.h b/vacmap_amd/csrc/vmx_host.h
--- a/vacmap_amd/csrc/vmx_host.h
+++ b/vacmap_amd/csrc/vmx_host.h
@@ -125,6 +125,7 @@
     vmx_mailbox mb;
     hipEvent_t ev[24];
     hipEvent_t gev[48];
+    hipEvent_t wev[32];
     int n_gev[2] = {0, 0};
     hipEvent_t kev[4] = {nullptr, nullptr, nullptr, nullptr};
     int kev_set = 0;
@@ -270,7 +271,9 @@
 __global__ void k_gapfill_fill_ns(const uint8_t* tcodes, const uint8_t* qcodes, vmx_dp_prob* probs, int n_prob, int match,
                                   int mismatch, int o1, int e1, int o2, int e2, uint8_t* tb_pool, int32_t* bnd_pool, int32_t* out_score,
                                   const int32_t* order, const int32_t* range, int32_t* counter, int32_t* redo_list, int32_t* redo_cnt, int ad_pct,
-                                  unsigned long long* redo_bytes, const int32_t* n_ptr = nullptr, unsigned long long redo_cap = ~0ULL, int tb_by_ns = 0);
+                                  unsigned long long* redo_bytes, const int32_t* n_ptr = nullptr, unsigned long long redo_cap = ~0ULL, int tb_by_ns = 0, const uint8_t* adw = nullptr);
+__global__ void k_gapfill_width(const uint8_t* tcodes, const uint8_t* qcodes, const vmx_dp_prob* probs, int n_prob, const int32_t* n_ptr, int match, int mismatch, int o1, int e1,
+                                int o2, int e2, int ad_pct, uint8_t* adw, int64_t* key, int32_t* cnt);
 __global__ void k_gapfill_redo(const uint8_t* tcodes, const uint8_t* qcodes, const vmx_dp_prob* probs, int match, int mismatch, int o1, int e1, int o2, int e2,
                                uint8_t* tb_pool, int32_t* bnd_pool, int32_t* out_score, int32_t* redo_list, int32_t* redo_cnt, uint8_t* redo_pool);
 static inline int vmx_ad_pct_env(int mode = 0) {
diff --git a/vacmap_amd/csrc/vmx_kernels.h b/vacmap_amd/csrc/vmx_kernels.h
--- a/vacmap_amd/csrc/vmx_kernels.h
+++ b/vacmap_amd/csrc/vmx_kernels.h
@@ -162,6 +162,83 @@
 __host__ __device__ static inline int vmx_ad_ns(int tl, int ql, int match, int o1, int e1, int o2, int e2, int pct, int pct_min) {
     return vmx_ad_ns_nd(tl, ql, match, o1, e1, o2, e2, pct, pct_min, 32, 1, VMX_AD_NS_MAX);
 }
+__host__ __device__ static inline long long vmx_ad_cert_C(int match, int mismatch, int o1, int e1, int o2, int e2) {
+    const long long c1 = (long long)o1 + e1 < (long long)o2 + e2 ? (long long)o1 + e1 : (long long)o2 + e2;
+    const long long a = (long long)match - mismatch, b = (match + 1) / 2 + c1;
+    return a > b ? a : b;
+}
+__host__ __device__ static inline int vmx_ad_ns_cert(int tl, int ql, long long ed_ub, int match, int mismatch, int o1, int e1, int o2, int e2) {
+    if (tl <= 0 || ql <= 0 || ed_ub < 0) return 0;
+    const int mn = tl < ql ? tl : ql;
+    const long long need = vmx_ad_cert_C(match, mismatch, o1, e1, o2, e2) * ed_ub;
+    for (int ns = 1; ns <= VMX_AD_NS_MAX; ++ns) {
+        int dlo;
+        const int g = vmx_ad_geom(tl, ql, ns, &dlo);
+        if (g >= 1 && (g > mn || vmx_ad_margin(g, match, o1, e1, o2, e2) > need)) return ns;
+    }
+    return 0;
+}
+__host__ __device__ static inline unsigned long long vmx_ad_ld8(const uint8_t* p, int n) {
+    unsigned long long w = 0x0404040404040404ULL;
+    if (n <= 0) return w;
+#if defined(__HIP_DEVICE_COMPILE__)
+    unsigned long long v;
+    __builtin_memcpy(&v, p, 8);
+    if (n < 8) { const unsigned long long m = ~0ULL >> (64 - 8 * n); v = (v & m) | (w & ~m); }
+    return v;
+#else
+    for (int k = 0; k < 8 && k < n; ++k) w = (w & ~(0xffULL << (8 * k))) | ((unsigned long long)p[k] << (8 * k));
+    return w;
+#endif
+}
+__host__ __device__ static inline int vmx_ad_ed_ub(const uint8_t* T, int tl, const uint8_t* Q, int ql) {
+    int dlo = 0;
+    if (tl <= 0 || ql <= 0 || vmx_ad_geom_nd(tl, ql, 64, &dlo) < 1) return -1;
+    const int z = dlo + 63;
+    unsigned long long b0 = 0, b1 = 0, bv = 0;
+#define VMX_AD_PUSH(c) do { b0 = (b0 >> 1) | ((unsigned long long)((c) & 1u) << 63); b1 = (b1 >> 1) | ((unsigned long long)(((c) >> 1) & 1u) << 63); \
+                            bv = (bv >> 1) | ((unsigned long long)((c) < 4u) << 63); } while (0)
+    for (int r0 = 0; r0 < -dlo; r0 += 8) {
+        unsigned long long w = vmx_ad_ld8(T + r0, tl - r0);
+        for (int k = 0; k < 8 && r0 + k < -dlo; ++k) { const unsigned c = (unsigned)(w & 0xffu); w >>= 8; VMX_AD_PUSH(c); }
+    }
+    unsigned long long Mv = z ? ~0ULL >> (64 - z) : 0ULL, Pv = ~Mv;
+    int top = z;
+    for (int j0 = 1; j0 <= ql; j0 += 8) {
+        unsigned long long wt = vmx_ad_ld8(T + (j0 - 1 - dlo), tl - (j0 - 1 - dlo)), wq = vmx_ad_ld8(Q + (j0 - 1), ql - (j0 - 1));
+#pragma unroll
+        for (int k = 0; k < 8; ++k) {
+            if (j0 + k > ql) break;
+            const unsigned c = (unsigned)(wt >> (8 * k)) & 0xffu, q = (unsigned)(wq >> (8 * k)) & 0xffu;
+            VMX_AD_PUSH(c);
+            const unsigned long long m0 = 0ULL - (unsigned long long)(q & 1u), m1 = 0ULL - (unsigned long long)((q >> 1) & 1u);
+            const unsigned long long Eq = q < 4u ? bv & ~((b0 ^ m0) | (b1 ^ m1)) : 0ULL;
+            const unsigned long long D0 = ((((Eq & Pv) + Pv) ^ Pv) | Eq | Mv);
+            const unsigned long long Ph = Mv | ~(D0 | Pv), Mh = Pv & D0;
+            top += 1 - (int)(D0 & 1ULL);
+            const unsigned long long X = D0 >> 1;
+            Pv = Mh | ~(X | Ph); Mv = Ph & X;
+        }
+    }
+#undef VMX_AD_PUSH
+    const int ne = tl - ql + z;
+    const unsigned long long mask = ne ? ~0ULL >> (64 - ne) : 0ULL;
+    return top + __builtin_popcountll(Pv & mask) - __builtin_popcountll(Mv & mask);
+}
+__host__ __device__ static inline long long vmx_ad_width_key(int ns, int tl, int ql) {
+    int r = 0;
+    if (ns > 0) {
+        int bin = (tl + ql - 1) >> 5;
+        const int lo = ns == 3 ? 1 : (ns >= 4 ? 2 : 0);
+        bin = bin > 31 ? 31 : (bin < lo ? lo : bin);
+        r = ns == 1 ? 1 + bin : (ns == 2 ? 33 + bin : (ns == 3 ? 64 + bin : 94 + bin));
+    }
+    const int cls = r < 3 ? (r == 0 ? 0 : 2 * r + 2) : r + 5, e = cls >> 2, m = cls & 3;
+    return e >= 2 ? (long long)(4 | m) << (e - 2) : (long long)((4 | m) >> (2 - e));
+}
+#define VMX_ADW_NS(b) ((int)(b) & 7)
+#define VMX_ADW_CERT 16
+#define VMX_ADW_SIZED(b) ((int)(b) >> 5)
 #define VMX_AD_PCT_DEFAULT 100
 #define VMX_AD_PCT_MIN_DEFAULT 65
 #ifdef VMX_EMU
diff --git a/vacmap_amd/csrc/vmx_stage.h b/vacmap_amd/csrc/vmx_stage.h
--- a/vacmap_amd/csrc/vmx_stage.h
+++ b/vacmap_amd/csrc/vmx_stage.h
@@ -30,7 +30,7 @@
     vmx::DevBuf nanc64, aoff, rows, lens, keys, koff, sorted, flip, S, P, SA, cov, gmax, opc, rl, gap, scr, soff, res, plen, prow, ocodes;
     vmx::DevBuf er, coff3, soff2, segA, st, en, segA_s, st_s, en_s, segprob, dup, desc[2], rcount, oflow, probread, tl, ql, toff, qoff, tpool, qpool;
     vmx::DevBuf edout, carry, ext3, dpsz[4], dpoff[4], dptab, tb, tbredo, bnd, run, cig, ciglen, dpscore, rec, blob, bloboff, reccoff, recclen, dupd, totals;
-    vmx::DevBuf raw, codes, off, order, qrange, scanpart, scanoff, si, tg, cntp, fp, pp, chunkn, sellist, cigq, statblk, szh, side_codes, side_off, roundpart, gfctl, geotot;
+    vmx::DevBuf raw, codes, off, order, qrange, scanpart, scanoff, si, tg, cntp, fp, pp, chunkn, sellist, cigq, statblk, szh, side_codes, side_off, roundpart, gfctl, geotot, adw;
     void release() { vmx::DevBuf* p = (vmx::DevBuf*)this; for (size_t i = 0; i < sizeof(*this) / sizeof(vmx::DevBuf); ++i) p[i].release(); }
 };
 vmx_batch_bufs* vmx_ctx_batch_bufs(vm_ctx* c);
@@ -43,7 +43,7 @@
 
 #define VMX_GF_SLOT (32 + 544)
 void vmx_gapfill_chunk(vm_ctx* c, vmx_batch_bufs& B, const vm_score& sc, int ad_pct, int eqx, int p0, int64_t pn, const int32_t* n_ptr, int64_t tb_off0,
-                       int32_t* ctl, int32_t* redo_list, int64_t redo_cap, hipEvent_t* ke);
+                       int32_t* ctl, int32_t* redo_list, int64_t redo_cap, hipEvent_t* ke, hipEvent_t* we = nullptr, bool cert = true);
 
 extern "C" int vmx_seed_stage(vm_ctx* c, const vm_index* mi, int check_num, int mid_occ, int64_t n, const uint8_t* d_codes, const int64_t* d_roff, int64_t total_bases,
                    vmx::DevBuf* B, std::vector<int64_t>& h_koff, std::vector<int64_t>& h_nhits, vmx::DevBuf* arena = nullptr, int64_t** rows_out = nullptr);
diff --git a/vacmap_amd/lib.py b/vacmap_amd/lib.py
--- a/vacmap_amd/lib.py
+++ b/vacmap_amd/lib.py
@@ -69,7 +69,8 @@
                [('ms_total', C.c_double), ('ms_stage', C.c_double * 16), ('ms_gapfill_fill', C.c_double), ('ms_gapfill_trace', C.c_double),
                 ('n_gapfill_launches', C.c_int64), ('n_ed_full', C.c_int64), ('n_ed_tier2', C.c_int64), ('n_ed_tier1', C.c_int64),
                 ('n_dp_redo', C.c_int64), ('dp_redo_tb_bytes', C.c_int64), ('ms_local_seed', C.c_double), ('ms_cluster', C.c_double), ('n_host_syncs', C.c_int64), ('n_local_general', C.c_int64), ('n_ext_retries', C.c_int64), ('n_batch_retries', C.c_int64),
-                ('n_dp_redo_wide', C.c_int64), ('n_dp_redo_full', C.c_int64)]
+                ('n_dp_redo_wide', C.c_int64), ('n_dp_redo_full', C.c_int64),
+                ('n_dp_cert', C.c_int64), ('n_dp_cert_narrower', C.c_int64), ('n_dp_cert_unproven', C.c_int64), ('ms_gapfill_width', C.c_double)]
 
 
 def _b(s):
@@ -129,7 +130,11 @@
         L.vm_k_extend_batch.argtypes = [vp] + [C.c_int] * 6 + [i64, cp, vp, cp, vp, P(P(i32)), P(P(i32)), P(P(i32))]
         L.vm_k_cigar_batch.argtypes = [vp, P(Score), C.c_int, i64, cp, vp, cp, vp, P(vp), P(P(i64)), P(P(i32))]
         L.vm_k_cigar.argtypes = [vp, cp, i64, cp, i64, P(Score), C.c_int, C.c_int, C.c_int, P(CigarOut)]
+        L.vm_ad_cert.argtypes = [P(Score), C.c_int, C.c_int, i64, vp]; L.vm_ad_cert.restype = None
+        L.vm_ad_width_key.argtypes = [C.c_int, C.c_int, C.c_int]; L.vm_ad_width_key.restype = i64
+        L.vm_ad_ed_ub.argtypes = [vp, C.c_int, vp, C.c_int]; L.vm_ad_ed_ub.restype = i64
         L.vm_k_cigar_batch_banded.argtypes = [vp, P(Score), C.c_int, i64, cp, vp, cp, vp, P(vp), P(P(i64)), P(P(i32)), vp]
+        L.vm_k_cigar_batch_banded_cert.argtypes = L.vm_k_cigar_batch_banded.argtypes
         L.vm_chain_global_batch.argtypes = [vp, P(Params), C.c_int, i64, vp, vp, vp, C.c_int, P(ChainsOut)]
         L.vm_chain_linked.argtypes = [vp, C.c_int, C.c_int, C.c_double, C.c_int, C.c_int, i64, vp, i64, vp, vp, C.c_double, i64, i64, P(LinkedOut)]
         L.vm_linked_out_free.argtypes = [P(LinkedOut)]
@@ -303,19 +308,21 @@
         cigars = [blob[off[i]:off[i + 1] - 1].decode() for i in range(n)]
         return cigars, self._take(ss, n, np.int32)
 
-    def k_cigar_batch_banded(self, targets, queries, match=2, mismatch=-4, o1=4, e1=2, o2=24, e2=1, eqx=False):
+    def k_cigar_batch_banded(self, targets, queries, match=2, mismatch=-4, o1=4, e1=2, o2=24, e2=1, eqx=False, cert=False):
         t, to = _cat(targets); q, qo = _cat(queries)
         n = len(targets)
         sc = Score(match, mismatch, o1, e1, o2, e2)
-        cg = C.c_void_p(); co = C.POINTER(C.c_int64)(); fl = C.POINTER(C.c_int32)(); st = (C.c_int64 * 6)()
-        self.lib.check(self.lib.L.vm_k_cigar_batch_banded(self.h, C.byref(sc), int(eqx), n, t, to.ctypes.data, q, qo.ctypes.data,
-                                                          C.byref(cg), C.byref(co), C.byref(fl), st))
+        cg = C.c_void_p(); co = C.POINTER(C.c_int64)(); fl = C.POINTER(C.c_int32)(); st = (C.c_int64 * 10)()
+        entry = self.lib.L.vm_k_cigar_batch_banded_cert if cert else self.lib.L.vm_k_cigar_batch_banded
+        self.lib.check(entry(self.h, C.byref(sc), int(eqx), n, t, to.ctypes.data, q, qo.ctypes.data, C.byref(cg), C.byref(co), C.byref(fl), st))
         off = self._take(co, n + 1, np.int64)
         blob = C.string_at(cg.value, int(off[-1])) if off[-1] else b''
         self.lib.L.vm_free(cg)
         cigars = [blob[off[i]:off[i + 1] - 1].decode() for i in range(n)]
-        return cigars, self._take(fl, n, np.int32), {'eligible': st[0], 'proven': st[1], 'redo': st[2], 'not_eligible': st[3],
-                                                          'redo_wide': st[4], 'redo_full': st[5]}
+        out = {'eligible': st[0], 'proven': st[1], 'redo': st[2], 'not_eligible': st[3], 'redo_wide': st[4], 'redo_full': st[5]}
+        if cert:
+            out.update({'cert': st[6], 'cert_narrower': st[7], 'cert_unproven': st[8], 'band_failed': st[9]})
+        return cigars, self._take(fl, n, np.int32), out
 
     def k_cigar(self, target, query, match=2, mismatch=-4, gap_open_1=4, gap_extend_1=2, gap_open_2=24, gap_extend_2=1,
                 bw=-1, zdropvalue=-1, eqx=False):
```

Result: slower. 3.005 (-14.5%).
